# davelailai/DS-GCN

Hardware: AMD Instinct MI355X
Metric: clips/sec fwd+bwd, DS-STGCN NTU-60 3x64x25x2 (higher is better)
Workload: dtype f32; 1 GPU; DS-STGCN configs/dsstgcn/ntu60_xsub_3dkp/j.py (DSSTGCN_model.py kwargs), 64 clips/GPU of 3x64x25x2, 60 classes, train-mode BN, CE loss, fwd+bwd+grad all-reduce+SGD-nesterov per step; clips_per_gpu=64, global_batch=64, parallelism=dp1

## Files before the change

ds-gcn_amd/csrc/bwd64.hip:

```cpp
#include "common.h"

namespace {

constexpr int BF_NT = 256, BF_KC = 64, BF_LS = BF_KC + 2, BF_Q = BF_KC / 4, BF_J = 64 * BF_Q / BF_NT;
constexpr int BF_OOB = 0x7ffffff0;

struct BfArgs {
  const float* x1; const float* s1; const float* h1;
  const float* x2; const float* s2; const float* h2; int relu;
  const float* w;
  const float* z; const float* gz; const float* A0; const float* B0;
  float* dx; float* dx2; float* dwp; float* dbp; float* ipart;
  int pstride, n, Ci, Co, L, cpn, total_chunks, cps;
};

typedef float bf_f2 __attribute__((ext_vector_type(2)));

__device__ __forceinline__ __amdgpu_buffer_rsrc_t bf_rsrc(const void* p, int bytes) {
  return __builtin_amdgcn_make_buffer_rsrc(const_cast<void*>(p), (short)0, bytes, 0x00020000);
}
__device__ __forceinline__ f32x4 bf_load(__amdgpu_buffer_rsrc_t r, int voff) {
  return __builtin_bit_cast(f32x4, __builtin_amdgcn_raw_buffer_load_b128(r, voff, 0, 0));
}
__device__ __forceinline__ int bf_row32(int r, int half) { return (r & 3) + 8 * (r >> 2) + 4 * half; }

#ifdef DSGCN_LAB
__device__ long long g_bf_stamp[64];
#define BF_STAMP() do { if (blockIdx.x == 0 && threadIdx.x == 0 && nst < 62) g_bf_stamp[nst++] = wall_clock64(); } while (0)
#else
#define BF_STAMP() do {} while (0)
#endif

template <bool HASC, bool AFF, bool HAS2>
__global__ __launch_bounds__(BF_NT, 2) void k_bwd64(BfArgs a) {
  extern __shared__ __attribute__((aligned(16))) float lds[];
#ifdef DSGCN_LAB
  int nst = 0;
#endif
  BF_STAMP();
  float* Ds = lds;
  float* Xs = lds + 64 * BF_LS;
  float* Os = lds + 128 * BF_LS;
  float* Ws = lds + 192 * BF_LS;
  bf_f2* Cs = reinterpret_cast<bf_f2*>(Ws + 64 * 65);
  f32x4* Ps = reinterpret_cast<f32x4*>(Cs + 64);
  const int tid = threadIdx.x, lane = tid & 63;
  const int wave = __builtin_amdgcn_readfirstlane(tid >> 6);
  const int half = lane >> 5, l31 = lane & 31;
  const int Ci = a.Ci, Co = a.Co, L = a.L, L4 = L * 4;
  const int split = blockIdx.x;
  const int ch0 = split * a.cps, ch1 = min(a.total_chunks, ch0 + a.cps);

  for (int i = tid; i < 64 * 65; i += BF_NT) {
    const int co = i / 65, ci = i - co * 65;
    Ws[i] = (co < Co && ci < Ci) ? a.w[(size_t)co * Ci + ci] : 0.f;
  }
  if (tid < 64) {
    Cs[tid] = (HASC && tid < Co) ? bf_f2{a.A0[tid], a.B0[tid]} : bf_f2{0.f, 0.f};
    f32x4 p = {1.f, 0.f, 1.f, 0.f};
    if (AFF && tid < Ci) {
      if (a.s1) { p.x = a.s1[tid]; p.y = a.h1[tid]; }
      if (HAS2 && a.s2) { p.z = a.s2[tid]; p.w = a.h2[tid]; }
    }
    Ps[tid] = p;
  }
  const float lo = a.relu ? 0.f : -__builtin_inff();

  const int col = (tid % BF_Q) * 4, row0 = tid / BF_Q;
  f32x4 gr[BF_J], zr[HASC ? BF_J : 1], xr[BF_J], yr[HAS2 ? BF_J : 1];
  f32x4 xk[AFF ? BF_J : 1], yk[HAS2 ? BF_J : 1];
  float dsum[BF_J], r0[BF_J], r1[BF_J], r2[BF_J];
#pragma unroll
  for (int j = 0; j < BF_J; ++j) { dsum[j] = 0.f; r0[j] = 0.f; r1[j] = 0.f; r2[j] = 0.f; }
  auto issue = [&](int ch) {
    const int n = ch / a.cpn, c0 = (ch - n * a.cpn) * BF_KC;
    const bool pv = c0 + col < L;
    const __amdgpu_buffer_rsrc_t rg = bf_rsrc(a.gz + (size_t)n * Co * L, Co * L4);
    const __amdgpu_buffer_rsrc_t rz = bf_rsrc((HASC ? a.z : a.gz) + (size_t)n * Co * L, HASC ? Co * L4 : 0);
    const __amdgpu_buffer_rsrc_t rx = bf_rsrc(a.x1 + (size_t)n * Ci * L, Ci * L4);
    const __amdgpu_buffer_rsrc_t ry = bf_rsrc((HAS2 ? a.x2 : a.x1) + (size_t)n * Ci * L, HAS2 ? Ci * L4 : 0);
#pragma unroll
    for (int j = 0; j < BF_J; ++j) {
      const int row = row0 + 16 * j;
      const int vd = (pv && row < Co) ? (row * L + c0 + col) * 4 : BF_OOB;
      const int vx = (pv && row < Ci) ? (row * L + c0 + col) * 4 : BF_OOB;
      gr[j] = bf_load(rg, vd);
      if constexpr (HASC) zr[j] = bf_load(rz, vd);
      xr[j] = bf_load(rx, vx);
      if constexpr (HAS2) yr[j] = bf_load(ry, vx);
    }
  };
  auto commit = [&](int ch) {
    const int n = ch / a.cpn, c0 = (ch - n * a.cpn) * BF_KC;
    const bool pv = c0 + col < L;
#pragma unroll
    for (int j = 0; j < BF_J; ++j) {
      const int row = row0 + 16 * j;
      f32x4 d = gr[j];
      if constexpr (HASC) {
        const bf_f2 c = Cs[row];
#pragma unroll
        for (int e = 0; e < 4; ++e) d[e] += fmaf(c.y, zr[j][e], c.x);
      }
      if (!(pv && row < Co)) d = f32x4{0.f, 0.f, 0.f, 0.f};
      dsum[j] += (d.x + d.y) + (d.z + d.w);
      bf_f2* dd = reinterpret_cast<bf_f2*>(Ds + row * BF_LS + col);
      dd[0] = bf_f2{d.x, d.y};
      dd[1] = bf_f2{d.z, d.w};
      f32x4 v = xr[j];
      if constexpr (AFF) {
        const f32x4 p = Ps[row];
        xk[j] = xr[j];
        if constexpr (HAS2) yk[j] = yr[j];
#pragma unroll
        for (int e = 0; e < 4; ++e) {
          float t = fmaf(xr[j][e], p.x, p.y);
          if constexpr (HAS2) t += fmaf(yr[j][e], p.z, p.w);
          v[e] = fmaxf(t, lo);
        }
      }
      if (!(pv && row < Ci)) v = f32x4{0.f, 0.f, 0.f, 0.f};
      bf_f2* dxs = reinterpret_cast<bf_f2*>(Xs + row * BF_LS + col);
      dxs[0] = bf_f2{v.x, v.y};
      dxs[1] = bf_f2{v.z, v.w};
    }
  };

  f32x16 accw, accw2, accd, accd2;
#pragma unroll
  for (int i = 0; i < 16; ++i) { accw[i] = 0.f; accw2[i] = 0.f; }
  const bool narrow_i = Ci <= 32;
  const int mt = narrow_i ? (wave & 1) : (wave >> 1), nt = narrow_i ? 0 : (wave & 1);
  const int cit = narrow_i ? 0 : (wave >> 1), pt = wave & 1;
  const float* Ap = Ds + (32 * mt + l31) * BF_LS + 2 * half;
  const float* Bp = Xs + (32 * nt + l31) * BF_LS + 2 * half;
  const int KSd = (Co + 1) >> 1;
  const bool wg_on = 32 * mt < Co && 32 * nt < Ci && !(narrow_i && wave >= 2);
  const bool dg_on = 32 * cit < Ci && !(narrow_i && wave < 2);

  __syncthreads();
  BF_STAMP();
  if (ch0 < ch1) issue(ch0);
  for (int ch = ch0; ch < ch1; ++ch) {
    commit(ch);
    asm volatile("s_waitcnt lgkmcnt(0)" ::: "memory");
    __builtin_amdgcn_s_barrier();
    BF_STAMP();
    if (ch + 1 < ch1) issue(ch + 1);
    if (wg_on) {
      bf_f2 av0 = *reinterpret_cast<const bf_f2*>(Ap), bv0 = *reinterpret_cast<const bf_f2*>(Bp);
      bf_f2 av1 = *reinterpret_cast<const bf_f2*>(Ap + 4), bv1 = *reinterpret_cast<const bf_f2*>(Bp + 4);
#pragma unroll
      for (int w = 0; w < BF_Q; w += 2) {
        bf_f2 an0 = av0, bn0 = bv0, an1 = av1, bn1 = bv1;
        if (w + 2 < BF_Q) {
          an0 = *reinterpret_cast<const bf_f2*>(Ap + 4 * (w + 2)); bn0 = *reinterpret_cast<const bf_f2*>(Bp + 4 * (w + 2));
          an1 = *reinterpret_cast<const bf_f2*>(Ap + 4 * (w + 3)); bn1 = *reinterpret_cast<const bf_f2*>(Bp + 4 * (w + 3));
        }
        __builtin_amdgcn_sched_barrier(0);
        accw = __builtin_amdgcn_mfma_f32_32x32x2f32(av0.x, bv0.x, accw, 0, 0, 0);
        accw2 = __builtin_amdgcn_mfma_f32_32x32x2f32(av0.y, bv0.y, accw2, 0, 0, 0);
        accw = __builtin_amdgcn_mfma_f32_32x32x2f32(av1.x, bv1.x, accw, 0, 0, 0);
        accw2 = __builtin_amdgcn_mfma_f32_32x32x2f32(av1.y, bv1.y, accw2, 0, 0, 0);
        __builtin_amdgcn_sched_barrier(0);
        av0 = an0; bv0 = bn0; av1 = an1; bv1 = bn1;
      }
    }
    if (dg_on) {
#pragma unroll
      for (int i = 0; i < 16; ++i) { accd[i] = 0.f; accd2[i] = 0.f; }
      const float* Wa = Ws + half * 65 + 32 * cit + l31;
      const float* Db = Ds + half * BF_LS + 32 * pt + l31;
      const int KS4 = (KSd + 3) & ~3;
      float wa[4], db[4];
#pragma unroll
      for (int i = 0; i < 4; ++i) { wa[i] = Wa[2 * i * 65]; db[i] = Db[2 * i * BF_LS]; }
      for (int ks = 0; ks < KS4; ks += 4) {
        float wn[4], dn[4];
        const int kn = ks + 4 < 32 ? ks + 4 : 28;
#pragma unroll
        for (int i = 0; i < 4; ++i) { wn[i] = Wa[2 * (kn + i) * 65]; dn[i] = Db[2 * (kn + i) * BF_LS]; }
        __builtin_amdgcn_sched_barrier(0);
        accd = __builtin_amdgcn_mfma_f32_32x32x2f32(wa[0], db[0], accd, 0, 0, 0);
        accd2 = __builtin_amdgcn_mfma_f32_32x32x2f32(wa[1], db[1], accd2, 0, 0, 0);
        accd = __builtin_amdgcn_mfma_f32_32x32x2f32(wa[2], db[2], accd, 0, 0, 0);
        accd2 = __builtin_amdgcn_mfma_f32_32x32x2f32(wa[3], db[3], accd2, 0, 0, 0);
        __builtin_amdgcn_sched_barrier(0);
#pragma unroll
        for (int i = 0; i < 4; ++i) { wa[i] = wn[i]; db[i] = dn[i]; }
      }
#pragma unroll
      for (int r = 0; r < 16; ++r)
        Os[(32 * cit + bf_row32(r, half)) * BF_LS + 32 * pt + l31] = accd[r] + accd2[r];
    }
    asm volatile("s_waitcnt lgkmcnt(0)" ::: "memory");
    __builtin_amdgcn_s_barrier();
    BF_STAMP();
    {
      const int n = ch / a.cpn, c0 = (ch - n * a.cpn) * BF_KC;
      if (c0 + col < L) {
#pragma unroll
        for (int j = 0; j < BF_J; ++j) {
          const int row = row0 + 16 * j;
          if (row < Ci) {
            const bf_f2* o = reinterpret_cast<const bf_f2*>(Os + row * BF_LS + col);
            const bf_f2 lo2 = o[0], hi2 = o[1];
            f32x4 dv = {lo2.x, lo2.y, hi2.x, hi2.y};
            f32x4 p = {1.f, 0.f, 1.f, 0.f};
            if constexpr (AFF) {
              p = Ps[row];
#pragma unroll
              for (int e = 0; e < 4; ++e) {
                float t = fmaf(xk[j][e], p.x, p.y);
                if constexpr (HAS2) t += fmaf(yk[j][e], p.z, p.w);
                if (a.relu && !(t > 0.f)) dv[e] = 0.f;
                r0[j] = fmaf(dv[e], xk[j][e], r0[j]);
                r1[j] += dv[e];
                if constexpr (HAS2) r2[j] = fmaf(dv[e], yk[j][e], r2[j]);
              }
            }
            const size_t go = ((size_t)n * Ci + row) * L + c0 + col;
            __builtin_nontemporal_store(f32x4{dv.x * p.x, dv.y * p.x, dv.z * p.x, dv.w * p.x}, reinterpret_cast<f32x4*>(a.dx + go));
            if constexpr (HAS2) __builtin_nontemporal_store(f32x4{dv.x * p.z, dv.y * p.z, dv.z * p.z, dv.w * p.z}, reinterpret_cast<f32x4*>(a.dx2 + go));
          }
        }
      }
    }
  }

  BF_STAMP();
  float* dw = a.dwp + (size_t)split * a.pstride;
  {
    const int ci = 32 * nt + l31;
#pragma unroll
    for (int r = 0; r < 16; ++r) {
      const int co = 32 * mt + bf_row32(r, half);
      if (wg_on && co < Co && ci < Ci) dw[(size_t)co * Ci + ci] = accw[r] + accw2[r];
    }
  }
#pragma unroll
  for (int j = 0; j < BF_J; ++j) {
    float s = dsum[j], s0 = r0[j], s1 = r1[j], s2 = r2[j];
#pragma unroll
    for (int off = 1; off < BF_Q; off <<= 1) {
      s += __shfl_xor(s, off, 64);
      if (AFF) { s0 += __shfl_xor(s0, off, 64); s1 += __shfl_xor(s1, off, 64); }
      if (HAS2) s2 += __shfl_xor(s2, off, 64);
    }
    const int row = row0 + 16 * j;
    if ((tid % BF_Q) == 0) {
      if (row < Co) a.dbp[(size_t)split * a.pstride + row] = s;
      if (AFF && a.ipart && row < Ci) {
        float* o = a.ipart + ((size_t)split * Ci + row) * 3;
        o[0] = s0; o[1] = s1; o[2] = s2;
      }
    }
  }
#ifdef DSGCN_LAB
  BF_STAMP();
  if (blockIdx.x == 0 && threadIdx.x == 0) g_bf_stamp[63] = nst;
#endif
}

constexpr int BB_RB = 80, BB_RT = 144, BB_OS = 36;
constexpr int BB_DK = 0, BB_XK = 3 * 64 * BB_RB, BB_DT = 2 * 3 * 64 * BB_RB, BB_WT = BB_DT + 3 * 32 * BB_RT,
              BB_OSO = BB_WT + 3 * 64 * BB_RT, BB_LDS = BB_OSO + 64 * BB_OS * 4;

template <bool HASC, bool AFF>
__global__ __launch_bounds__(BF_NT, 2) void k_bwd64b(BfArgs a) {
  extern __shared__ __attribute__((aligned(16))) char ldsb[];
#ifdef DSGCN_LAB
  int nst = 0;
#endif
  BF_STAMP();
  char* Dk = ldsb + BB_DK;
  char* Xk = ldsb + BB_XK;
  char* Dt = ldsb + BB_DT;
  char* Wt = ldsb + BB_WT;
  float* Os = reinterpret_cast<float*>(ldsb + BB_OSO);
  const int tid = threadIdx.x, lane = tid & 63;
  const int wave = __builtin_amdgcn_readfirstlane(tid >> 6);
  const int half = lane >> 5, l31 = lane & 31;
  const int Ci = a.Ci, Co = a.Co, L = a.L, L4 = L * 4;
  const int split = blockIdx.x;
  const int ch0 = split * a.cps, ch1 = min(a.total_chunks, ch0 + a.cps);
  const int row = tid >> 2, q = tid & 3;
  const bool rd = row < Co, rx = row < Ci;
  const float A0v = (HASC && rd) ? a.A0[row] : 0.f, B0v = (HASC && rd) ? a.B0[row] : 0.f;
  float s1v = 1.f, h1v = 0.f;
  if (AFF && rx && a.s1) { s1v = a.s1[row]; h1v = a.h1[row]; }
  const float lo = a.relu ? 0.f : -__builtin_inff();
  for (int i = tid; i < 64 * 32; i += BF_NT) {
    const int ci = i >> 5, co = 2 * (i & 31);
    const float w0 = (ci < Ci && co < Co) ? a.w[(size_t)co * Ci + ci] : 0.f;
    const float w1 = (ci < Ci && co + 1 < Co) ? a.w[(size_t)(co + 1) * Ci + ci] : 0.f;
    unsigned p0, p1, p2;
    b3_split(w0, w1, p0, p1, p2);
    char* base = Wt + ci * BB_RT + co * 2;
    *reinterpret_cast<unsigned*>(base) = p0;
    *reinterpret_cast<unsigned*>(base + 64 * BB_RT) = p1;
    *reinterpret_cast<unsigned*>(base + 2 * 64 * BB_RT) = p2;
  }

  struct Raw { f32x4 g[2], z[HASC ? 2 : 1], x[2]; };
  Raw ra, rb;
  f32x4 xk[AFF ? 2 : 1];
  float dsum = 0.f, r0 = 0.f, r1 = 0.f;
  auto issue = [&](int ch, Raw& R) {
    const int n = ch / a.cpn, c0 = (ch - n * a.cpn) * 32;
    const __amdgpu_buffer_rsrc_t rg = bf_rsrc(a.gz + (size_t)n * Co * L, Co * L4);
    const __amdgpu_buffer_rsrc_t rz = bf_rsrc((HASC ? a.z : a.gz) + (size_t)n * Co * L, HASC ? Co * L4 : 0);
    const __amdgpu_buffer_rsrc_t r1_ = bf_rsrc(a.x1 + (size_t)n * Ci * L, Ci * L4);
#pragma unroll
    for (int h = 0; h < 2; ++h) {
      const int p = c0 + 8 * q + 4 * h;
      const int vd = (rd && p < L) ? (row * L + p) * 4 : BF_OOB;
      const int vx = (rx && p < L) ? (row * L + p) * 4 : BF_OOB;
      R.g[h] = bf_load(rg, vd);
      if constexpr (HASC) R.z[h] = bf_load(rz, vd);
      R.x[h] = bf_load(r1_, vx);
    }
  };
  auto commit = [&](int ch, const Raw& R) {
    const int n = ch / a.cpn, c0 = (ch - n * a.cpn) * 32;
    float d[8], v[8];
#pragma unroll
    for (int h = 0; h < 2; ++h) {
      const bool in = c0 + 8 * q + 4 * h < L;
#pragma unroll
      for (int e = 0; e < 4; ++e) {
        float x = R.g[h][e];
        if constexpr (HASC) x += fmaf(B0v, R.z[h][e], A0v);
        d[4 * h + e] = (rd && in) ? x : 0.f;
        float t = R.x[h][e];
        if constexpr (AFF) {
          t = fmaf(t, s1v, h1v);
          t = fmaxf(t, lo);
        }
        v[4 * h + e] = (rx && in) ? t : 0.f;
      }
      if constexpr (AFF) xk[h] = R.x[h];
    }
    dsum += ((d[0] + d[1]) + (d[2] + d[3])) + ((d[4] + d[5]) + (d[6] + d[7]));
    unsigned t0[4], t1[4], t2[4];
#pragma unroll
    for (int j = 0; j < 4; ++j) b3_split(d[2 * j], d[2 * j + 1], t0[j], t1[j], t2[j]);
    {
      char* base = Dk + row * BB_RB + q * 16;
      *reinterpret_cast<u32x4v*>(base) = u32x4v{t0[0], t0[1], t0[2], t0[3]};
      *reinterpret_cast<u32x4v*>(base + 64 * BB_RB) = u32x4v{t1[0], t1[1], t1[2], t1[3]};
      *reinterpret_cast<u32x4v*>(base + 2 * 64 * BB_RB) = u32x4v{t2[0], t2[1], t2[2], t2[3]};
    }
    {
      const int odd = row & 1;
      char* base = Dt + (8 * q + odd) * BB_RT + (row & ~1) * 2;
      const unsigned sel = odd ? 0x07060302u : 0x01000504u;
      unsigned o0[4], o1[4], o2[4];
#pragma unroll
      for (int j = 0; j < 4; ++j) {
        o0[j] = __shfl_xor(t0[j], 4, 64); o1[j] = __shfl_xor(t1[j], 4, 64); o2[j] = __shfl_xor(t2[j], 4, 64);
      }
#pragma unroll
      for (int j = 0; j < 4; ++j) {
        const unsigned w0 = __builtin_amdgcn_perm(t0[j], o0[j], sel);
        const unsigned w1 = __builtin_amdgcn_perm(t1[j], o1[j], sel);
        const unsigned w2 = __builtin_amdgcn_perm(t2[j], o2[j], sel);
        char* pj = base + 2 * j * BB_RT;
        *reinterpret_cast<unsigned*>(pj) = w0;
        *reinterpret_cast<unsigned*>(pj + 32 * BB_RT) = w1;
        *reinterpret_cast<unsigned*>(pj + 2 * 32 * BB_RT) = w2;
      }
    }
#pragma unroll
    for (int j = 0; j < 4; ++j) b3_split(v[2 * j], v[2 * j + 1], t0[j], t1[j], t2[j]);
    {
      char* base = Xk + row * BB_RB + q * 16;
      *reinterpret_cast<u32x4v*>(base) = u32x4v{t0[0], t0[1], t0[2], t0[3]};
      *reinterpret_cast<u32x4v*>(base + 64 * BB_RB) = u32x4v{t1[0], t1[1], t1[2], t1[3]};
      *reinterpret_cast<u32x4v*>(base + 2 * 64 * BB_RB) = u32x4v{t2[0], t2[1], t2[2], t2[3]};
    }
    (void)n;
  };

  const bool wgw = wave < 2;
  const int mt = wave & 1, cit = wave & 1;
  const bool wg0 = wgw && 32 * mt < Co, wg1 = wg0 && Ci > 32;
  const bool dg_on = !wgw && 32 * cit < Ci;
  const int KSD = (Co + 15) >> 4;
  f32x16 accw, accw1;
#pragma unroll
  for (int i = 0; i < 16; ++i) { accw[i] = 0.f; accw1[i] = 0.f; }
  const char* Af = Dk + (32 * mt + l31) * BB_RB + 16 * half;
  const char* Bf = Xk + l31 * BB_RB + 16 * half;
  const char* Wf = Wt + (32 * cit + l31) * BB_RT + 16 * half;
  const char* Df = Dt + l31 * BB_RT + 16 * half;
  auto six = [&](f32x16 c, const char* pa, int sa, const char* pb, int sb) {
    const bf16x8 a0 = __builtin_bit_cast(bf16x8, *reinterpret_cast<const u32x4v*>(pa)),
                 a1 = __builtin_bit_cast(bf16x8, *reinterpret_cast<const u32x4v*>(pa + sa)),
                 a2 = __builtin_bit_cast(bf16x8, *reinterpret_cast<const u32x4v*>(pa + 2 * sa));
    const bf16x8 b0 = __builtin_bit_cast(bf16x8, *reinterpret_cast<const u32x4v*>(pb)),
                 b1 = __builtin_bit_cast(bf16x8, *reinterpret_cast<const u32x4v*>(pb + sb)),
                 b2 = __builtin_bit_cast(bf16x8, *reinterpret_cast<const u32x4v*>(pb + 2 * sb));
    c = __builtin_amdgcn_mfma_f32_32x32x16_bf16(a2, b0, c, 0, 0, 0);
    c = __builtin_amdgcn_mfma_f32_32x32x16_bf16(a1, b1, c, 0, 0, 0);
    c = __builtin_amdgcn_mfma_f32_32x32x16_bf16(a0, b2, c, 0, 0, 0);
    c = __builtin_amdgcn_mfma_f32_32x32x16_bf16(a1, b0, c, 0, 0, 0);
    c = __builtin_amdgcn_mfma_f32_32x32x16_bf16(a0, b1, c, 0, 0, 0);
    c = __builtin_amdgcn_mfma_f32_32x32x16_bf16(a0, b0, c, 0, 0, 0);
    return c;
  };

  __syncthreads();
  BF_STAMP();
  auto unit = [&](int ch, Raw& R) {
    commit(ch, R);
    if (ch + 2 < ch1) issue(ch + 2, R);
    asm volatile("s_waitcnt lgkmcnt(0)" ::: "memory");
    __builtin_amdgcn_s_barrier();
    BF_STAMP();
    if (wg0) {
      accw = six(accw, Af, 64 * BB_RB, Bf, 64 * BB_RB);
      accw = six(accw, Af + 32, 64 * BB_RB, Bf + 32, 64 * BB_RB);
      if (wg1) {
        accw1 = six(accw1, Af, 64 * BB_RB, Bf + 32 * BB_RB, 64 * BB_RB);
        accw1 = six(accw1, Af + 32, 64 * BB_RB, Bf + 32 * BB_RB + 32, 64 * BB_RB);
      }
    }
    if (dg_on) {
      f32x16 accd;
#pragma unroll
      for (int i = 0; i < 16; ++i) accd[i] = 0.f;
#pragma unroll
      for (int ks = 0; ks < 4; ++ks)
        if (ks < KSD) accd = six(accd, Wf + 32 * ks, 64 * BB_RT, Df + 32 * ks, 32 * BB_RT);
#pragma unroll
      for (int r = 0; r < 16; ++r) Os[(32 * cit + bf_row32(r, half)) * BB_OS + l31] = accd[r];
    }
    asm volatile("s_waitcnt lgkmcnt(0)" ::: "memory");
    __builtin_amdgcn_s_barrier();
    BF_STAMP();
    {
      const int n = ch / a.cpn, c0 = (ch - n * a.cpn) * 32;
      f32x4* o = reinterpret_cast<f32x4*>(Os + row * BB_OS + 8 * q);
#pragma unroll
      for (int h = 0; h < 2; ++h) {
        f32x4 dv = o[h];
        if (rx && c0 + 8 * q + 4 * h < L) {
          float sx = 1.f;
          if constexpr (AFF) {
            sx = s1v;
#pragma unroll
            for (int e = 0; e < 4; ++e) {
              const float t = fmaf(xk[h][e], s1v, h1v);
              if (a.relu && !(t > 0.f)) dv[e] = 0.f;
              r0 = fmaf(dv[e], xk[h][e], r0);
              r1 += dv[e];
            }
          }
          const size_t go = ((size_t)n * Ci + row) * L + c0 + 8 * q + 4 * h;
          __builtin_nontemporal_store(f32x4{dv.x * sx, dv.y * sx, dv.z * sx, dv.w * sx}, reinterpret_cast<f32x4*>(a.dx + go));
        }
      }
    }
  };
  if (ch0 < ch1) issue(ch0, ra);
  if (ch0 + 1 < ch1) issue(ch0 + 1, rb);
  for (int ch = ch0; ch < ch1; ch += 2) {
    unit(ch, ra);
    if (ch + 1 < ch1) unit(ch + 1, rb);
  }

  BF_STAMP();
  float* dw = a.dwp + (size_t)split * a.pstride;
#pragma unroll
  for (int r = 0; r < 16; ++r) {
    const int co = 32 * mt + bf_row32(r, half);
    if (wg0 && co < Co && l31 < Ci) dw[(size_t)co * Ci + l31] = accw[r];
    if (wg1 && co < Co && 32 + l31 < Ci) dw[(size_t)co * Ci + 32 + l31] = accw1[r];
  }
  {
    float s = dsum, s0 = r0, s1 = r1;
#pragma unroll
    for (int off = 1; off < 4; off <<= 1) {
      s += __shfl_xor(s, off, 64);
      if (AFF) { s0 += __shfl_xor(s0, off, 64); s1 += __shfl_xor(s1, off, 64); }
    }
    if (q == 0) {
      if (rd) a.dbp[(size_t)split * a.pstride + row] = s;
      if (AFF && a.ipart && rx) {
        float* o = a.ipart + ((size_t)split * Ci + row) * 3;
        o[0] = s0; o[1] = s1; o[2] = 0.f;
      }
    }
  }
#ifdef DSGCN_LAB
  BF_STAMP();
  if (blockIdx.x == 0 && threadIdx.x == 0) g_bf_stamp[63] = nst;
#endif
}

struct BfPlan { int cpn, chunks, splits, cps; };

int g_bf_b3 = 1;

bool bf_plan(int n, int Ci, int Co, int L, BfPlan* p) {
  if (Ci <= 0 || Co <= 0 || Ci > 64 || Co > 64 || L % 4) return false;
  if ((long)64 * L * 4 >= (1L << 31) - 64) return false;
  p->cpn = (L + BF_KC - 1) / BF_KC;
  p->chunks = n * p->cpn;
  int target = 512;
  if (target > p->chunks) target = p->chunks;
  p->cps = (p->chunks + target - 1) / target;
  p->splits = (p->chunks + p->cps - 1) / p->cps;
  return true;
}

}

__attribute__((visibility("hidden"))) int dsgcn_bwd64_splits(int n, int Ci, int Co, int L) {
  BfPlan p;
  return bf_plan(n, Ci, Co, L, &p) ? p.splits : 0;
}

__attribute__((visibility("hidden"))) int dsgcn_bwd64(const float* x1, const float* s1, const float* h1, const float* x2,
                                                       const float* s2, const float* h2, int relu, const float* w,
                                                       const float* z, const float* gz, const float* A0, const float* B0,
                                                       float* dx, float* dx2, float* dwp, float* dbp, int pstride,
                                                       float* ipart, int n, int Ci, int Co, int L, hipStream_t st) {
  BfPlan p;
  if (!bf_plan(n, Ci, Co, L, &p)) return 0;
  BfArgs a = {};
  a.x1 = x1; a.s1 = s1; a.h1 = h1; a.x2 = x2; a.s2 = s2; a.h2 = h2; a.relu = relu; a.w = w; a.z = z; a.gz = gz;
  a.A0 = A0; a.B0 = B0; a.dx = dx; a.dx2 = dx2; a.dwp = dwp; a.dbp = dbp; a.ipart = ipart; a.pstride = pstride;
  a.n = n; a.Ci = Ci; a.Co = Co; a.L = L; a.cpn = p.cpn; a.total_chunks = p.chunks; a.cps = p.cps;
  const bool b3 = g_bf_b3 && x2 == nullptr && Ci >= 16;
  if (b3) {
    a.cpn = (L + 31) / 32;
    a.total_chunks = n * a.cpn;
    a.cps = (a.total_chunks + p.splits - 1) / p.splits;
  }
  const size_t lds = b3 ? (size_t)BB_LDS : (size_t)(192 * BF_LS + 64 * 65 + 2 * 64 + 4 * 64) * sizeof(float);
  const dim3 grid((unsigned)p.splits), blk(BF_NT);
  const bool hasc = A0 != nullptr, has2 = x2 != nullptr, aff = s1 != nullptr || s2 != nullptr || relu != 0 || has2;
  if (b3) {
#define BB_LAUNCH(HC, AF)                                                                                               \
  {                                                                                                                   \
    static bool raised = false;                                                                                       \
    if (!raised) {                                                                                                    \
      hipError_t e = hipFuncSetAttribute((const void*)k_bwd64b<HC, AF>, hipFuncAttributeMaxDynamicSharedMemorySize, \
                                         (int)lds);                                                                   \
      if (e != hipSuccess) return (int)e;                                                                             \
      raised = true;                                                                                                  \
    }                                                                                                                 \
    hipLaunchKernelGGL((k_bwd64b<HC, AF>), grid, blk, lds, st, a);                                                \
  }
    if (hasc) {
      if (aff) BB_LAUNCH(true, true) else BB_LAUNCH(true, false)
    } else {
      if (aff) BB_LAUNCH(false, true) else BB_LAUNCH(false, false)
    }
#undef BB_LAUNCH
    DSGCN_LAUNCH_CHECK();
    return 1;
  }
#define BF_LAUNCH(HC, AF, H2)                                                                                          \
  {                                                                                                                   \
    static bool raised = false;                                                                                       \
    if (!raised) {                                                                                                    \
      hipError_t e = hipFuncSetAttribute((const void*)k_bwd64<HC, AF, H2>, hipFuncAttributeMaxDynamicSharedMemorySize, \
                                         (int)lds);                                                                   \
      if (e != hipSuccess) return (int)e;                                                                             \
      raised = true;                                                                                                  \
    }                                                                                                                 \
    hipLaunchKernelGGL((k_bwd64<HC, AF, H2>), grid, blk, lds, st, a);                                                 \
  }
  if (has2) {
    if (hasc) BF_LAUNCH(true, true, true) else BF_LAUNCH(false, true, true)
  } else if (hasc) {
    if (aff) BF_LAUNCH(true, true, false) else BF_LAUNCH(true, false, false)
  } else {
    if (aff) BF_LAUNCH(false, true, false) else BF_LAUNCH(false, false, false)
  }
#undef BF_LAUNCH
  DSGCN_LAUNCH_CHECK();
  return 1;
}

__attribute__((visibility("hidden"))) int dsgcn_bwd64_tuning(int value) { g_bf_b3 = value; return 0; }

#ifdef DSGCN_LAB
extern "C" int dsgcn_bwd64_phases(long long* out) {
  return (int)hipMemcpyFromSymbol(out, HIP_SYMBOL(g_bf_stamp), sizeof(long long) * 64);
}
#endif
```

ds-gcn_amd/csrc/fuseout.hip:

```cpp
#include "common.h"
#include "dropout.h"
#include "dsgcn_jobs.h"

namespace {

__global__ __launch_bounds__(64) void k_fuse_out_fwd(const float* __restrict__ x1, const float* __restrict__ s1,
                                                     const float* __restrict__ h1, const float* __restrict__ x2,
                                                     const float* __restrict__ s2, const float* __restrict__ h2,
                                                     int relu, float* __restrict__ out, float* __restrict__ xbar, int C,
                                                     int T, int V, int vec, int ld, float* __restrict__ out_s2,
                                                     float* __restrict__ pmean, DropArgs dr) {
  extern __shared__ __attribute__((aligned(16))) float lds[];
  const int lane = threadIdx.x;
  const long plane = blockIdx.x;
  const int c = (int)(plane % C);
  const int L = T * V;
  const bool drop = dr.thresh != 0;
  const unsigned long long dstep = (drop && dr.step) ? (unsigned long long)*dr.step : 0ull;
  const float a1 = s1 ? s1[c] : 1.f, b1 = s1 ? h1[c] : 0.f;
  const float a2 = s2 ? s2[c] : 1.f, b2 = s2 ? h2[c] : 0.f;
  const float* p1 = x1 + (size_t)plane * L;
  const float* p2 = x2 ? x2 + (size_t)plane * L : nullptr;
  float* po = out ? out + (size_t)plane * L : nullptr;
  float psum = 0.f;
  if (vec) {
    const int L4 = L >> 2;
    const f32x4* q1 = reinterpret_cast<const f32x4*>(p1);
    const f32x4* q2 = reinterpret_cast<const f32x4*>(p2);
    f32x4* qo = reinterpret_cast<f32x4*>(po);
    f32x4* ql = reinterpret_cast<f32x4*>(lds);
#pragma unroll 4
    for (int i = lane; i < L4; i += 64) {
      f32x4 v = q1[i];
      v.x = fmaf(v.x, a1, b1); v.y = fmaf(v.y, a1, b1); v.z = fmaf(v.z, a1, b1); v.w = fmaf(v.w, a1, b1);
      if (relu & 2) { v.x = fmaxf(v.x, 0.f); v.y = fmaxf(v.y, 0.f); v.z = fmaxf(v.z, 0.f); v.w = fmaxf(v.w, 0.f); }
      if (drop) {
        unsigned rw[4];
        drop_words(dr, dstep, (unsigned long long)plane * L4 + i, rw);
        v.x *= rw[0] >= dr.thresh ? dr.inv : 0.f; v.y *= rw[1] >= dr.thresh ? dr.inv : 0.f;
        v.z *= rw[2] >= dr.thresh ? dr.inv : 0.f; v.w *= rw[3] >= dr.thresh ? dr.inv : 0.f;
      }
      if (p2) {
        const f32x4 r = q2[i];
        v.x += fmaf(r.x, a2, b2); v.y += fmaf(r.y, a2, b2); v.z += fmaf(r.z, a2, b2); v.w += fmaf(r.w, a2, b2);
      }
      if (relu & 1) { v.x = fmaxf(v.x, 0.f); v.y = fmaxf(v.y, 0.f); v.z = fmaxf(v.z, 0.f); v.w = fmaxf(v.w, 0.f); }
      if (po) qo[i] = v;
      psum += (v.x + v.y) + (v.z + v.w);
      if (xbar || out_s2) ql[i] = v;
    }
  } else {
    for (int i = lane; i < L; i += 64) {
      float v = fmaf(p1[i], a1, b1);
      if (relu & 2) v = fmaxf(v, 0.f);
      if (drop) v *= drop_mult(dr, dstep, (unsigned long long)plane * L + i);
      if (p2) v += fmaf(p2[i], a2, b2);
      if (relu & 1) v = fmaxf(v, 0.f);
      if (po) po[i] = v;
      psum += v;
      if (xbar || out_s2) lds[i] = v;
    }
  }
  if (pmean) {
    psum = wave_sum(psum);
    if (lane == 0) pmean[plane] = psum / (float)L;
  }
  if (xbar || out_s2) wave_lds_sync();
  if (out_s2) {
    const int T2 = (T + 1) >> 1, L2 = T2 * V;
    float* ps = out_s2 + (size_t)plane * L2;
    const float invV = 1.f / (float)V;
    if ((L2 & 3) == 0) {
      f32x4* q4 = reinterpret_cast<f32x4*>(ps);
      for (int i = lane; i < (L2 >> 2); i += 64) {
        int t, v;
        divmod_small(4 * i, V, invV, t, v);
        float r[4];
#pragma unroll
        for (int k = 0; k < 4; ++k) {
          r[k] = lds[2 * t * V + v];
          if (++v == V) { v = 0; ++t; }
        }
        q4[i] = f32x4{r[0], r[1], r[2], r[3]};
      }
    } else {
      for (int i = lane; i < L2; i += 64) {
        int t, v;
        divmod_small(i, V, invV, t, v);
        ps[i] = lds[2 * t * V + v];
      }
    }
  }
  if (xbar) {
    if (lane < ld) {
      float s = 0.f;
      if (lane < V)
        for (int t = 0; t < T; ++t) s += lds[t * V + lane];
      xbar[(size_t)plane * ld + lane] = s / (float)T;
    }
  }
}

__global__ __launch_bounds__(64) void k_fuse_out_bwd(const float* __restrict__ x1, const float* __restrict__ s1,
                                                     const float* __restrict__ h1, const float* __restrict__ x2,
                                                     const float* __restrict__ s2, const float* __restrict__ h2,
                                                     int relu, const float* __restrict__ dout,
                                                     const float* __restrict__ dout2, const float* __restrict__ dout3,
                                                     const float* __restrict__ dxbar, float* __restrict__ dx1,
                                                     float* __restrict__ dx2, float* __restrict__ part, int C, int T,
                                                     int V, int ld, int s3, DropArgs dr) {
  __shared__ float dxb[32];
  const int lane = threadIdx.x;
  const long plane = blockIdx.x;
  const int c = (int)(plane % C);
  const int L = T * V;
  const bool drop = dr.thresh != 0;
  const unsigned long long dstep = (drop && dr.step) ? (unsigned long long)*dr.step : 0ull;
  const float a1 = s1 ? s1[c] : 1.f, b1 = s1 ? h1[c] : 0.f;
  const float a2 = s2 ? s2[c] : 1.f, b2 = s2 ? h2[c] : 0.f;
  if (lane < V) dxb[lane] = dxbar ? dxbar[(size_t)plane * ld + lane] / (float)T : 0.f;
  wave_lds_sync();
  const float* __restrict__ p1 = x1 + (size_t)plane * L;
  const float* __restrict__ p2 = x2 ? x2 + (size_t)plane * L : nullptr;
  const float* __restrict__ pg = (dout && s3 != 3) ? dout + (size_t)plane * L : nullptr;
  const float gpl = s3 == 3 ? dout[plane] / (float)L : 0.f;
  const float* __restrict__ pg2 = dout2 ? dout2 + (size_t)plane * L : nullptr;
  const float* __restrict__ pg3 = dout3 ? dout3 + (size_t)plane * (s3 == 2 ? ((T + 1) >> 1) * V : L) : nullptr;
  float* __restrict__ o1 = dx1 + (size_t)plane * L;
  float* __restrict__ o2 = dx2 ? dx2 + (size_t)plane * L : nullptr;
  float u0 = 0.f, u1 = 0.f, u2 = 0.f, u3 = 0.f;
  int v = lane % V, t = lane / V;
  const int step = 64 % V, tstep = 64 / V;
#pragma unroll 5
  for (int i = lane; i < L; i += 64) {
    const float xa = p1[i];
    const float xb = p2 ? p2[i] : 0.f;
    const float pre1 = fmaf(xa, a1, b1);
    float pre = (relu & 2) ? fmaxf(pre1, 0.f) : pre1;
    const float dm = drop ? drop_mult(dr, dstep, (unsigned long long)plane * L + i) : 1.f;
    pre *= dm;
    if (p2) pre += fmaf(xb, a2, b2);
    float g = s3 == 3 ? gpl : (pg ? pg[i] : 0.f);
    if (pg2) g += pg2[i];
    if (pg3) {
      if (s3 == 2) { if (!(t & 1)) g += pg3[(t >> 1) * V + v]; }
      else g += pg3[i];
    }
    g += dxb[v];
    if ((relu & 1) && !(pre > 0.f)) g = 0.f;
    const float g1 = (((relu & 2) && !(pre1 > 0.f)) ? 0.f : g) * dm;
    o1[i] = g1 * a1;
    if (o2) o2[i] = g * a2;
    u0 = fmaf(g1, xa, u0);
    u1 += g;
    u2 = fmaf(g, xb, u2);
    u3 += g1;
    v += step;
    t += tstep;
    if (v >= V) { v -= V; ++t; }
  }
  if (part) {
    u0 = wave_sum(u0);
    u1 = wave_sum(u1);
    u2 = wave_sum(u2);
    u3 = wave_sum(u3);
    if (lane == 0) {
      part[(size_t)plane * 4 + 0] = u0;
      part[(size_t)plane * 4 + 1] = u1;
      part[(size_t)plane * 4 + 2] = u2;
      part[(size_t)plane * 4 + 3] = u3;
    }
  }
}

template <int NG, bool S3, bool X2>
__global__ __launch_bounds__(64) void k_fuse_out_bwd4(const float* __restrict__ x1, const float* __restrict__ s1,
                                                      const float* __restrict__ h1, const float* __restrict__ x2,
                                                      const float* __restrict__ s2, const float* __restrict__ h2,
                                                      int relu, const float* __restrict__ dout,
                                                      const float* __restrict__ dout2, const float* __restrict__ dout3,
                                                      const float* __restrict__ dxbar, float* __restrict__ dx1,
                                                      float* __restrict__ dx2, float* __restrict__ part, int C, int T,
                                                      int V, int ld, DropArgs dr) {
  __shared__ float dxb[32];
  const int lane = threadIdx.x;
  const long plane = blockIdx.x;
  const int c = (int)(plane % C);
  const int L = T * V, L4 = L >> 2;
  const bool drop = dr.thresh != 0;
  const unsigned long long dstep = (drop && dr.step) ? (unsigned long long)*dr.step : 0ull;
  const float a1 = s1 ? s1[c] : 1.f, b1 = s1 ? h1[c] : 0.f;
  const float a2 = s2 ? s2[c] : 1.f, b2 = s2 ? h2[c] : 0.f;
  if (lane < V) dxb[lane] = dxbar ? dxbar[(size_t)plane * ld + lane] / (float)T : 0.f;
  wave_lds_sync();
  const f32x4* __restrict__ p1 = reinterpret_cast<const f32x4*>(x1 + (size_t)plane * L);
  const f32x4* __restrict__ p2 = X2 ? reinterpret_cast<const f32x4*>(x2 + (size_t)plane * L) : nullptr;
  const f32x4* __restrict__ pg = NG >= 1 ? reinterpret_cast<const f32x4*>(dout + (size_t)plane * L) : nullptr;
  const float gplane = NG == 0 ? dout[plane] / (float)L : 0.f;
  const f32x4* __restrict__ pg2 = NG >= 2 ? reinterpret_cast<const f32x4*>(dout2 + (size_t)plane * L) : nullptr;
  const f32x4* __restrict__ pg3 = (NG >= 3 && !S3) ? reinterpret_cast<const f32x4*>(dout3 + (size_t)plane * L) : nullptr;
  const float* __restrict__ ps3 = S3 ? dout3 + (size_t)plane * (((T + 1) >> 1) * V) : nullptr;
  f32x4* __restrict__ o1 = reinterpret_cast<f32x4*>(dx1 + (size_t)plane * L);
  f32x4* __restrict__ o2 = X2 ? reinterpret_cast<f32x4*>(dx2 + (size_t)plane * L) : nullptr;
  const float invV = 1.f / (float)V;
  float u0 = 0.f, u1 = 0.f, u2 = 0.f, u3 = 0.f;
  for (int i = lane; i < L4; i += 64) {
    const f32x4 xa = p1[i];
    f32x4 xb = {0.f, 0.f, 0.f, 0.f}, g = {gplane, gplane, gplane, gplane};
    if constexpr (NG >= 1) g = pg[i];
    if constexpr (X2) xb = p2[i];
    if constexpr (NG >= 2) { const f32x4 w = pg2[i]; g.x += w.x; g.y += w.y; g.z += w.z; g.w += w.w; }
    if constexpr (NG >= 3 && !S3) { const f32x4 w = pg3[i]; g.x += w.x; g.y += w.y; g.z += w.z; g.w += w.w; }
    int t, v;
    divmod_small(4 * i, V, invV, t, v);
    f32x4 r1, r2;
    float dm[4] = {1.f, 1.f, 1.f, 1.f};
    if (drop) {
      unsigned rw[4];
      drop_words(dr, dstep, (unsigned long long)plane * L4 + i, rw);
#pragma unroll
      for (int k = 0; k < 4; ++k) dm[k] = rw[k] >= dr.thresh ? dr.inv : 0.f;
    }
#pragma unroll
    for (int k = 0; k < 4; ++k) {
      float gg = g[k];
      if constexpr (S3) { if (!(t & 1)) gg += ps3[(t >> 1) * V + v]; }
      gg += dxb[v];
      const float pre1 = fmaf(xa[k], a1, b1);
      float pre = ((relu & 2) ? fmaxf(pre1, 0.f) : pre1) * dm[k];
      if constexpr (X2) pre += fmaf(xb[k], a2, b2);
      if ((relu & 1) && !(pre > 0.f)) gg = 0.f;
      const float g1 = (((relu & 2) && !(pre1 > 0.f)) ? 0.f : gg) * dm[k];
      r1[k] = g1 * a1;
      r2[k] = gg * a2;
      u0 = fmaf(g1, xa[k], u0);
      u1 += gg;
      u2 = fmaf(gg, xb[k], u2);
      u3 += g1;
      if (++v == V) { v = 0; ++t; }
    }
    o1[i] = r1;
    if constexpr (X2) o2[i] = r2;
  }
  if (part) {
    u0 = wave_sum(u0);
    u1 = wave_sum(u1);
    u2 = wave_sum(u2);
    u3 = wave_sum(u3);
    if (lane == 0) {
      part[(size_t)plane * 4 + 0] = u0;
      part[(size_t)plane * 4 + 1] = u1;
      part[(size_t)plane * 4 + 2] = u2;
      part[(size_t)plane * 4 + 3] = u3;
    }
  }
}

int g_fo_vec = 1;

}

namespace {

DropArgs drop_args(const dsgcn_dropout* d) {
  DropArgs a = {};
  if (d && d->p > 0.f) {
    a.step = d->step; a.seed = d->seed; a.call = d->call;
    double t = (double)d->p * 4294967296.0;
    a.thresh = t >= 4294967295.0 ? 4294967295u : (t < 1.0 ? 1u : (unsigned)t);
    a.inv = 1.f / (1.f - d->p);
  }
  return a;
}

__global__ __launch_bounds__(256) void k_dropout_mask(float* __restrict__ mask, long numel, DropArgs dr) {
  const unsigned long long step = dr.step ? (unsigned long long)*dr.step : 0ull;
  for (long e = (long)blockIdx.x * 256 + threadIdx.x; e < numel; e += (long)gridDim.x * 256)
    mask[e] = dr.thresh ? drop_mult(dr, step, (unsigned long long)e) : 1.f;
}

}

extern "C" {

int dsgcn_fuse_out_fwd_drop(const float* x1, const float* s1, const float* h1, const float* x2, const float* s2,
                            const float* h2, int relu, float* out, float* out_s2, float* xbar, float* pmean, int n, int C,
                            int T, int V, int xbar_ld, const dsgcn_dropout* d, void* stream) {
  if (!x1 || (!out && !pmean) || n <= 0 || C <= 0 || T <= 0 || V <= 0 || V > 32 || (s1 && !h1) || (s2 && !h2)) return DSGCN_EINVAL;
  if ((out_s2 || xbar) && !out) return DSGCN_EINVAL;
  if (xbar && (xbar_ld < V || xbar_ld > 64)) return DSGCN_EINVAL;
  if (d && !(d->p >= 0.f && d->p < 1.f)) return DSGCN_EINVAL;
  const int vec = ((T * V) % 4 == 0) ? 1 : 0;
  const size_t lds = (xbar || out_s2) ? (size_t)T * V * sizeof(float) : 0;
  if (lds > 64 * 1024) return DSGCN_EUNSUPPORTED;
  hipLaunchKernelGGL(k_fuse_out_fwd, dim3((unsigned)((long)n * C)), dim3(64), lds, (hipStream_t)stream, x1, s1, h1, x2,
                     s2, h2, relu, out, xbar, C, T, V, vec, xbar ? xbar_ld : V, out_s2, pmean, drop_args(d));
  DSGCN_LAUNCH_CHECK();
  return 0;
}

int dsgcn_fuse_out_fwd(const float* x1, const float* s1, const float* h1, const float* x2, const float* s2,
                       const float* h2, int relu, float* out, float* xbar, int n, int C, int T, int V, int xbar_ld,
                       void* stream) {
  if (!out) return DSGCN_EINVAL;
  return dsgcn_fuse_out_fwd_drop(x1, s1, h1, x2, s2, h2, relu, out, nullptr, xbar, nullptr, n, C, T, V, xbar_ld, nullptr, stream);
}

int dsgcn_fuse_out_fwd2(const float* x1, const float* s1, const float* h1, const float* x2, const float* s2,
                        const float* h2, int relu, float* out, float* out_s2, float* xbar, int n, int C, int T, int V,
                        int xbar_ld, void* stream) {
  if (!out) return DSGCN_EINVAL;
  return dsgcn_fuse_out_fwd_drop(x1, s1, h1, x2, s2, h2, relu, out, out_s2, xbar, nullptr, n, C, T, V, xbar_ld, nullptr, stream);
}

int dsgcn_fuse_out_pool_fwd(const float* x1, const float* s1, const float* h1, const float* x2, const float* s2,
                            const float* h2, int relu, float* pmean, int n, int C, int T, int V, void* stream) {
  if (!pmean) return DSGCN_EINVAL;
  return dsgcn_fuse_out_fwd_drop(x1, s1, h1, x2, s2, h2, relu, nullptr, nullptr, nullptr, pmean, n, C, T, V, V, nullptr, stream);
}

int dsgcn_fuse_out_bwd_drop(const float* x1, const float* s1, const float* h1, const float* x2, const float* s2,
                            const float* h2, int relu, const float* dout, const float* dout2, const float* dout3,
                            int stride3, const float* dxbar, float* dx1, float* dx2, float* part, int n, int C, int T, int V,
                            int xbar_ld, const dsgcn_dropout* d, void* stream) {
  if (!x1 || !dx1 || n <= 0 || C <= 0 || T <= 0 || V <= 0 || V > 32 || (x2 && !dx2)) return DSGCN_EINVAL;
  if (dxbar && xbar_ld < V) return DSGCN_EINVAL;
  if ((dout2 || dout3) && !dout) return DSGCN_EINVAL;
  if (stride3 < 1 || stride3 > 3 || (stride3 == 3 && (!dout || dout2 || dout3 || dxbar))) return DSGCN_EINVAL;
  if (d && !(d->p >= 0.f && d->p < 1.f)) return DSGCN_EINVAL;
  const DropArgs dr = drop_args(d);
  const dim3 grid((unsigned)((long)n * C)), blk(64);
  hipStream_t st = (hipStream_t)stream;
  if (stride3 == 3) {
    if ((T * V) % 4 == 0) {
      if (x2)
        hipLaunchKernelGGL((k_fuse_out_bwd4<0, false, true>), grid, blk, 0, st, x1, s1, h1, x2, s2, h2, relu, dout,
                           (const float*)nullptr, (const float*)nullptr, (const float*)nullptr, dx1, dx2, part, C, T, V, V, dr);
      else
        hipLaunchKernelGGL((k_fuse_out_bwd4<0, false, false>), grid, blk, 0, st, x1, s1, h1, x2, s2, h2, relu, dout,
                           (const float*)nullptr, (const float*)nullptr, (const float*)nullptr, dx1, dx2, part, C, T, V, V, dr);
    } else {
      hipLaunchKernelGGL(k_fuse_out_bwd, grid, blk, 0, st, x1, s1, h1, x2, s2, h2, relu, dout, (const float*)nullptr,
                         (const float*)nullptr, (const float*)nullptr, dx1, dx2, part, C, T, V, V, 3, dr);
    }
    DSGCN_LAUNCH_CHECK();
    return 0;
  }
  if (g_fo_vec && dout && (T * V) % 4 == 0 && !(dout3 && !dout2 && stride3 == 1)) {
    const int ng = dout3 && stride3 == 1 ? 3 : (dout2 ? 2 : 1);
    const bool s3 = dout3 && stride3 == 2;
#define FO4(NGV, S3V, X2V) hipLaunchKernelGGL((k_fuse_out_bwd4<NGV, S3V, X2V>), grid, blk, 0, st, x1, s1, h1, x2, s2, h2, relu, \
                                              dout, dout2, dout3, dxbar, dx1, dx2, part, C, T, V, xbar_ld, dr)
    if (x2) {
      if (s3) { if (ng == 2) FO4(2, true, true); else FO4(1, true, true); }
      else if (ng == 3) FO4(3, false, true);
      else if (ng == 2) FO4(2, false, true);
      else FO4(1, false, true);
    } else {
      if (s3) { if (ng == 2) FO4(2, true, false); else FO4(1, true, false); }
      else if (ng == 3) FO4(3, false, false);
      else if (ng == 2) FO4(2, false, false);
      else FO4(1, false, false);
    }
#undef FO4
    DSGCN_LAUNCH_CHECK();
    return 0;
  }
  hipLaunchKernelGGL(k_fuse_out_bwd, grid, blk, 0, st, x1, s1, h1, x2, s2, h2, relu, dout, dout2, dout3, dxbar, dx1, dx2,
                     part, C, T, V, xbar_ld, stride3, dr);
  DSGCN_LAUNCH_CHECK();
  return 0;
}

int dsgcn_fuse_out_pool_bwd(const float* x1, const float* s1, const float* h1, const float* x2, const float* s2,
                            const float* h2, int relu, const float* dpmean, float* dx1, float* dx2, float* part, int n,
                            int C, int T, int V, void* stream) {
  if (!dpmean) return DSGCN_EINVAL;
  return dsgcn_fuse_out_bwd_drop(x1, s1, h1, x2, s2, h2, relu, dpmean, nullptr, nullptr, 3, nullptr, dx1, dx2, part, n, C, T, V,
                                 V, nullptr, stream);
}

int dsgcn_fuse_out_bwd3(const float* x1, const float* s1, const float* h1, const float* x2, const float* s2,
                        const float* h2, int relu, const float* dout, const float* dout2, const float* dout3,
                        const float* dxbar, float* dx1, float* dx2, float* part, int n, int C, int T, int V, int xbar_ld,
                        void* stream) {
  return dsgcn_fuse_out_bwd_drop(x1, s1, h1, x2, s2, h2, relu, dout, dout2, dout3, 1, dxbar, dx1, dx2, part, n, C, T, V,
                                 xbar_ld, nullptr, stream);
}

int dsgcn_fuse_out_bwd3s(const float* x1, const float* s1, const float* h1, const float* x2, const float* s2,
                         const float* h2, int relu, const float* dout, const float* dout2, const float* dout3, int stride3,
                         const float* dxbar, float* dx1, float* dx2, float* part, int n, int C, int T, int V, int xbar_ld,
                         void* stream) {
  if (stride3 != 1 && stride3 != 2) return DSGCN_EINVAL;
  return dsgcn_fuse_out_bwd_drop(x1, s1, h1, x2, s2, h2, relu, dout, dout2, dout3, stride3, dxbar, dx1, dx2, part, n, C, T, V,
                                 xbar_ld, nullptr, stream);
}

int dsgcn_dropout_mask(float* mask, long numel, const dsgcn_dropout* d, void* stream) {
  if (!mask || numel <= 0 || (d && !(d->p >= 0.f && d->p < 1.f))) return DSGCN_EINVAL;
  const long blocks = (numel + 255) / 256;
  hipLaunchKernelGGL(k_dropout_mask, dim3((unsigned)(blocks > 4096 ? 4096 : blocks)), dim3(256), 0, (hipStream_t)stream, mask,
                     numel, drop_args(d));
  DSGCN_LAUNCH_CHECK();
  return 0;
}

#ifdef DSGCN_LAB
int dsgcn_fuse_out_tuning(int key, int value) {
  if (key != 0) return DSGCN_EINVAL;
  g_fo_vec = value;
  return 0;
}
#endif

int dsgcn_fuse_out_bwd(const float* x1, const float* s1, const float* h1, const float* x2, const float* s2,
                       const float* h2, int relu, const float* dout, const float* dxbar, float* dx1, float* dx2,
                       float* part, int n, int C, int T, int V, int xbar_ld, void* stream) {
  return dsgcn_fuse_out_bwd3(x1, s1, h1, x2, s2, h2, relu, dout, nullptr, nullptr, dxbar, dx1, dx2, part, n, C, T, V,
                             xbar_ld, stream);
}

}

namespace {
__global__ __launch_bounds__(256) void k_pack(const float* const* __restrict__ src, const long* __restrict__ off,
                                              const int* __restrict__ numel, float* __restrict__ dst) {
  const int i = blockIdx.x;
  const float* __restrict__ s = src[i];
  float* __restrict__ d = dst + off[i];
  const int n = numel[i];
  for (int j = blockIdx.y * 256 + threadIdx.x; j < n; j += gridDim.y * 256) d[j] = s[j];
}
}

namespace {
__global__ __launch_bounds__(256) void k_pack_fill(const float* const* __restrict__ src, const long* __restrict__ off,
                                                   const long* __restrict__ numel, float* __restrict__ dst) {
  const int i = blockIdx.x;
  const float* __restrict__ s = src[i];
  float* __restrict__ d = dst + off[i];
  const long n = numel[i];
  if (s) {
    for (long j = blockIdx.y * 256 + threadIdx.x; j < n; j += gridDim.y * 256) d[j] = s[j];
  } else {
    for (long j = blockIdx.y * 256 + threadIdx.x; j < n; j += gridDim.y * 256) d[j] = 0.f;
  }
}
}

extern "C" int dsgcn_pack_fill(const float* const* src_table, const long* dst_offsets, const long* numels, int count,
                               float* dst, void* stream) {
  if (!src_table || !dst_offsets || !numels || !dst || count <= 0) return DSGCN_EINVAL;
  hipLaunchKernelGGL(k_pack_fill, dim3((unsigned)count, 8), dim3(256), 0, (hipStream_t)stream, src_table, dst_offsets,
                     numels, dst);
  DSGCN_LAUNCH_CHECK();
  return 0;
}

extern "C" int dsgcn_pack(const float* const* src_table, const long* dst_offsets, const int* numels, int count,
                          float* dst, void* stream) {
  if (!src_table || !dst_offsets || !numels || !dst || count <= 0) return DSGCN_EINVAL;
  hipLaunchKernelGGL(k_pack, dim3((unsigned)count, 8), dim3(256), 0, (hipStream_t)stream, src_table, dst_offsets, numels,
                     dst);
  DSGCN_LAUNCH_CHECK();
  return 0;
}

namespace {
__global__ __launch_bounds__(256) void k_add3(const f32x4* __restrict__ a, const f32x4* __restrict__ b,
                                              const f32x4* __restrict__ c, f32x4* __restrict__ out, long n4,
                                              const float* as, const float* bs, const float* cs, float* os, long n) {
  const long i = (long)blockIdx.x * 256 + threadIdx.x;
  if (i < n4) {
    f32x4 v = a[i];
    const f32x4 w = b[i];
    v.x += w.x; v.y += w.y; v.z += w.z; v.w += w.w;
    if (c) { const f32x4 u = c[i]; v.x += u.x; v.y += u.y; v.z += u.z; v.w += u.w; }
    out[i] = v;
  }
  if (blockIdx.x == 0) {
    const long j = n4 * 4 + threadIdx.x;
    if (j < n) os[j] = as[j] + bs[j] + (cs ? cs[j] : 0.f);
  }
}
}

extern "C" int dsgcn_add3(const float* a, const float* b, const float* c, float* out, long n, void* stream) {
  if (!a || !b || !out || n <= 0) return DSGCN_EINVAL;
  const long n4 = n / 4;
  const unsigned blocks = (unsigned)((n4 + 255) / 256);
  hipLaunchKernelGGL(k_add3, dim3(blocks ? blocks : 1), dim3(256), 0, (hipStream_t)stream,
                     reinterpret_cast<const f32x4*>(a), reinterpret_cast<const f32x4*>(b),
                     reinterpret_cast<const f32x4*>(c), reinterpret_cast<f32x4*>(out), n4, a, b, c, out, n);
  DSGCN_LAUNCH_CHECK();
  return 0;
}
```

ds-gcn_amd/csrc/pwconv.hip:

```cpp
#include "common.h"
#include "bn_jobs.h"

namespace {

constexpr int KCH = 16;
constexpr int WSTR = KCH + 1;
constexpr int NTW = 2;
constexpr int PW_NT = 256;
constexpr int XCH = KCH / 4;

struct PwArgs {
  const float* x1; const float* s1; const float* h1;
  const float* x2; const float* s2; const float* h2;
  int relu;
  const float* w; const float* bias;
  float* z; float* zaug; float* partial;
  int n, Ci, Co, T, V, Tout, stride, aug, TR, NPpad, vec, stats, roll, nbx, cc;
};

__device__ __forceinline__ int mfma_row32(int r, int half) { return (r & 3) + 8 * (r >> 2) + 4 * half; }

__device__ __forceinline__ float virt1(float a, float b, bool has2, float s1, float h1, float s2, float h2,
                                       int relu) {
  float v = fmaf(a, s1, h1);
// ... 920 lines not shown
          }
        }
      } else {
#pragma unroll
        for (int e = 0; e < 4; ++e) {
          const int pe = p + e;
          if (pe < nvalid) {
            if (co < Co) {
              if (has_g) gr[j][e] = a.gz[gzb + pe];
              if (has_c) zr[j][e] = a.z[gzb + pe];
            }
            if (ci < Ci) {
              const int rl = (int)(((float)pe + 0.5f) * invV);
              const size_t g = gxb + (size_t)rl * a.stride * V + (pe - rl * V);
              xr[j][e] = a.x1[g];
              if (HAS2) yr[HAS2 ? j : 0][e] = a.x2[g];
            }
          }
        }
      }
    }
  };

  auto commit = [&](int ch) {
    const int n = ch / a.nb_per_sample;
    const int r0 = (ch - n * a.nb_per_sample) * TR;
    const int nvalid = min(TR, a.Tout - r0) * V;
    float dsum = 0.f;
#pragma unroll
    for (int j = 0; j < WG_J; ++j) {
#pragma unroll
      for (int e = 0; e < 4; ++e) {
        const int pe = 16 * j + 4 * quarter + e;
        if (pe < KP) {
          float d = 0.f, x = 0.f;
          if (pe < nvalid) {
            if (co < Co) {
              d = has_g ? gr[j][e] : 0.f;
              if (has_c) d += fmaf(B0c, zr[j][e], A0c);
              if (a.aug) {
                const int rl = (int)(((float)pe + 0.5f) * invV);
                const size_t ga = (size_t)(n * Co + co) * a.Tout + r0 + rl;
                float ea = a.gzaug ? a.gzaug[ga] : 0.f;
                if (has_c) ea += fmaf(B0c, a.zaug[ga], A0c);
                d = fmaf(ea, invV, d);
              }
            }
            if (ci < Ci) x = virt1(xr[j][e], HAS2 ? yr[HAS2 ? j : 0][e] : 0.f, has2, s1, h1, s2, h2, a.relu);
          }
          Ds[row * LS + pe] = d;
          Xs[row * LS + pe] = x;
          dsum += d;
        }
      }
    }
    dsum += __shfl_xor(dsum, 1, 64);
    dsum += __shfl_xor(dsum, 2, 64);
    dbacc += dsum;
  };

  if (ch0 < ch1) issue(ch0);
  for (int ch = ch0; ch < ch1; ++ch) {
    commit(ch);
    __syncthreads();
    if (ch + 1 < ch1) issue(ch + 1);
    for (int kk = 0; kk < KP; kk += 2) {
      const float av = Ds[(32 * mt + l31) * LS + kk + half];
      const float bv = Xs[(32 * ntile + l31) * LS + kk + half];
      acc = __builtin_amdgcn_mfma_f32_32x32x2f32(av, bv, acc, 0, 0, 0);
    }
    __syncthreads();
  }
  const int cio = ciBase + 32 * ntile + l31;
  if (cio < Ci) {
#pragma unroll
    for (int r = 0; r < 16; ++r) {
      const int coo = coBase + 32 * mt + mfma_row32(r, half);
      if (coo < Co) a.dwp[(size_t)split * a.pstride + (size_t)coo * Ci + cio] = acc[r];
    }
  }
  if (byy == 0 && quarter == 0 && co < Co) a.dbp[(size_t)split * a.pstride + co] = dbacc;
}

__global__ __launch_bounds__(64) void k_bn_bwd_coef(const float* __restrict__ g_scale,
                                                    const float* __restrict__ g_shift,
                                                    const float* __restrict__ mean, const float* __restrict__ var,
                                                    const float* __restrict__ gamma, float eps, double count, int C,
                                                    int c_affine, float* __restrict__ dgamma,
                                                    float* __restrict__ dbeta, float* __restrict__ A0,
                                                    float* __restrict__ B0) {
  const int c = blockIdx.x * 64 + threadIdx.x;
  if (c >= C) return;
  if (c >= c_affine) { dgamma[c] = 0.f; dbeta[c] = 0.f; A0[c] = 0.f; B0[c] = 0.f; return; }
  const double gs = g_scale ? (double)g_scale[c] : 0.0, gh = g_shift ? (double)g_shift[c] : 0.0;
  const double mu = mean[c], r = 1.0 / sqrt((double)var[c] + (double)eps);
  const double g = gamma ? (double)gamma[c] : 1.0;
  const double t = gs - mu * gh;
  dgamma[c] = (float)(r * t);
  dbeta[c] = (float)gh;
  const double dmean = -gh * g * r;
  const double dvar = -0.5 * r * r * r * g * t;
  A0[c] = (float)((dmean - 2.0 * dvar * mu) / count);
  B0[c] = (float)(2.0 * dvar / count);
}

__global__ __launch_bounds__(1024) void k_bn_coef_rows(const float* __restrict__ part, int R, int C, int k, int ids, int idh,
                                                       const float* __restrict__ mean, const float* __restrict__ var,
                                                       const float* __restrict__ gamma, float eps, double count,
                                                       int c_affine, float* __restrict__ coef, int accumulate) {
  __shared__ double red[16][8][2];
  const BnCoefJob J = {part, mean, var, gamma, coef, count, eps, R, C, k, ids, idh, c_affine, accumulate};
  bn_coef_rows_block(J, blockIdx.x, red);
}

}

int g_pw_maxmt = 2;
int g_pw4 = 15;

__attribute__((visibility("hidden"))) int dsgcn_p4_tuning(int key, int value);
__attribute__((visibility("hidden"))) int dsgcn_p4_groups(int n, int K, int M, int L, int epi);
__attribute__((visibility("hidden"))) int dsgcn_wg2_tuning(int key, int value);
__attribute__((visibility("hidden"))) int dsgcn_p4_fwd(const float* x1, const float* s1, const float* h1,
                                                        const float* x2, const float* s2, const float* h2, int relu,
                                                        const float* w, const float* bias, float* z, float* partial,
                                                        int n, int Ci, int Co, int L, hipStream_t st, const void* ws);
__attribute__((visibility("hidden"))) size_t dsgcn_p4_ws_bytes(int n, int Ci, int Co, int L);
__attribute__((visibility("hidden"))) int dsgcn_bwd64_tuning(int value);
__attribute__((visibility("hidden"))) int dsgcn_p4_wsplit(const float* w, int Ci, int Co, void* out, hipStream_t st);
__attribute__((visibility("hidden"))) int dsgcn_p4_wsplit_multi(const float* const* w, void* const* out, const int* Ci,
                                                                const int* Co, int njobs, hipStream_t st);
__attribute__((visibility("hidden"))) int dsgcn_p4_dgrad(const float* x1, const float* s1, const float* h1,
                                                          const float* x2, const float* s2, const float* h2, int relu,
                                                          const float* w, const float* z, const float* gz,
                                                          const float* A0, const float* B0, float* dx1, float* dx2,
                                                          float* ipart, int n, int Ci, int Co, int L, hipStream_t st,
                                                          const void* ws);

__attribute__((visibility("hidden"))) int dsgcn_p4_group_ok(int n, int Ci, int Co, int L);
__attribute__((visibility("hidden"))) int dsgcn_p4_fwd_group(const float* const* x1, const float* const* s1,
                                                              const float* const* h1, int relu, const float* const* w,
                                                              float* const* z, int ng, int n, int Ci, int Co, int L,
                                                              hipStream_t st);
__attribute__((visibility("hidden"))) int dsgcn_p4_dgrad_group(const float* const* x1, const float* const* s1,
                                                                const float* const* h1, int relu, const float* const* w,
                                                                const float* const* gz, float* const* dx1, float* const* ipart,
                                                                int ng, int n, int Ci, int Co, int L, hipStream_t st);

__attribute__((visibility("hidden"))) int dsgcn_bwd64_splits(int n, int Ci, int Co, int L);
__attribute__((visibility("hidden"))) int dsgcn_bwd64(const float* x1, const float* s1, const float* h1, const float* x2,
                                                       const float* s2, const float* h2, int relu, const float* w,
                                                       const float* z, const float* gz, const float* A0, const float* B0,
                                                       float* dx, float* dx2, float* dwp, float* dbp, int pstride,
                                                       float* ipart, int n, int Ci, int Co, int L, hipStream_t st);

__attribute__((visibility("hidden"))) int dsgcn_wg2_splits(int n, int Ci, int Co, int L);
__attribute__((visibility("hidden"))) int dsgcn_wg2(const float* x1, const float* s1, const float* h1, const float* x2,
                                                     const float* s2, const float* h2, int relu, const float* z,
                                                     const float* gz, const float* A0, const float* B0, float* dwp,
                                                     float* dbp, int pstride, int n, int Ci, int Co, int L,
                                                     hipStream_t st, const BnCoefTable* jobs, int ngroup = 0,
                                                     const float* const* gx1 = nullptr, const float* const* gs1 = nullptr,
                                                     const float* const* gh1 = nullptr, const float* const* ggz = nullptr,
                                                     float* const* gdwp = nullptr, float* const* gdbp = nullptr);

static int pw_conv_rows(int n, int K, int M, int T, int V, int stride, int which) {
  const int Tout = (T + stride - 1) / stride;
  const int L = Tout * V;
  if (stride == 1 && (g_pw4 & which)) {
    const int g = dsgcn_p4_groups(n, K, M, L, which == 2 ? 1 : 0);
    if (g > 0) return g;
  }
  return n * ((L + 4 * 32 - 1) / (4 * 32));
}

extern "C" {

#ifdef DSGCN_LAB
int dsgcn_pwconv_tuning(int key, int value) {
  if (key == 1) { g_pw_maxmt = value; return 0; }
  if (key == 2) { g_pw_roll = value; return 0; }
  if (key == 3) { g_pw4 = value; return 0; }
  if (key >= 4 && key <= 6) return dsgcn_p4_tuning(key - 4, value);
  if (key >= 7 && key <= 9) return dsgcn_wg2_tuning(key - 7, value);
  if (key >= 10 && key <= 12) return dsgcn_p4_tuning(key - 7, value);
  if (key == 13) return dsgcn_wg2_tuning(3, value);
  if (key == 14) return dsgcn_p4_tuning(6, value);
  if (key >= 15 && key <= 17) return dsgcn_wg2_tuning(key - 11, value);
  if (key == 18) return dsgcn_bwd64_tuning(value);
  if (key == 19) return dsgcn_p4_tuning(7, value);
  if (key == 22) return dsgcn_p4_tuning(9, value);
  if (key == 20) return dsgcn_p4_tuning(8, value);
  return DSGCN_EINVAL;
}
#endif

int dsgcn_pwconv_plan(int Tout, int V, int aug, int* TR, int* NPpad, int* nblk_per_sample) {
  int tr = Tout >= 32 ? 8 : 4;
  if (tr > Tout) tr = Tout;
  int np = tr * (V + (aug ? 1 : 0));
  while (np > 256 && tr > 1) { tr >>= 1; np = tr * (V + (aug ? 1 : 0)); }
  if (np > 256) return DSGCN_EUNSUPPORTED;
  *TR = tr;
  *NPpad = (np + 31) & ~31;
  *nblk_per_sample = (Tout + tr - 1) / tr;
  return 0;
}

int dsgcn_pwconv_partial_rows(int n, int Ci, int Co, int T, int V, int stride, int aug) {
  int rows = pw_conv_rows(n, Ci, Co, T, V, stride, 1);
  if (aug) rows += n;
  return rows;
}

int dsgcn_pwconv_fwd_ws(const float* x1, const float* s1, const float* h1, const float* x2, const float* s2,
                        const float* h2, int relu, const float* w, const float* bias, float* z, float* zaug,
                        float* partial, int n, int Ci, int Co, int T, int V, int stride, int aug, int stats,
                        const void* ws, void* stream) {
  if (!x1 || !w || !z || n <= 0 || Ci <= 0 || Co <= 0 || T <= 0 || V <= 0 || stride <= 0) return DSGCN_EINVAL;
  if ((aug && !zaug) || (stats && !partial) || (s1 && !h1) || (s2 && !h2)) return DSGCN_EINVAL;
  const int Tout = (T + stride - 1) / stride;
  PwArgs a = {};
  a.x1 = x1; a.s1 = s1; a.h1 = h1; a.x2 = x2; a.s2 = s2; a.h2 = h2; a.relu = relu;
  a.w = w; a.bias = bias; a.z = z; a.zaug = zaug; a.partial = partial;
  a.n = n; a.Ci = Ci; a.Co = Co; a.T = T; a.V = V; a.Tout = Tout; a.stride = stride; a.aug = aug;
  a.stats = stats;
  a.roll = ((g_pw_roll & 1) && Ci % KW == 0) ? 1 : 0;
  hipStream_t st = (hipStream_t)stream;
  const int L = Tout * V;
  const int conv_rows = pw_conv_rows(n, Ci, Co, T, V, stride, 1);
  int fast = 0;
  if (stride == 1 && (g_pw4 & 1)) {
    fast = dsgcn_p4_fwd(x1, s1, h1, x2, s2, h2, relu, w, bias, z, stats ? partial : nullptr, n, Ci, Co, L, st, ws);
    if (fast != 0 && fast != 1) return fast;
  }
  if (!fast) {
  if ((long)n * Ci * T * V * 4 >= (1L << 31) - 64 || (long)n * Co * T * V * 4 >= (1L << 31) - 64) return DSGCN_EUNSUPPORTED;
  const int mtiles = (Co + 31) / 32;
  const int MT = mtiles >= g_pw_maxmt ? g_pw_maxmt : mtiles;
  const int NW = 1;
  const int nbx = (L + 4 * NW * 32 - 1) / (4 * NW * 32);
  a.nbx = nbx;
  a.cc = (mtiles + MT - 1) / MT;
  dim3 grid((unsigned)(((long)nbx * n + 7) / 8 * 8 * a.cc));
  size_t ldsf = (size_t)32 * MT * KWS + 4 + (size_t)4 * Ci;
  if (ldsf < (size_t)4 * 32 * 36 + 512) ldsf = (size_t)4 * 32 * 36 + 512;
  const size_t lds = ldsf * sizeof(float);
#define PW_FWD2(MTV)                                                                                  \
  if (a.roll) hipLaunchKernelGGL((k_pwconv_fwd2<MTV, 1, true>), grid, dim3(PW_NT), lds, st, a);       \
  else hipLaunchKernelGGL((k_pwconv_fwd2<MTV, 1, false>), grid, dim3(PW_NT), lds, st, a)
  switch (MT) {
    case 1: PW_FWD2(1); break;
    case 2: PW_FWD2(2); break;
    case 3: PW_FWD2(3); break;
    default: PW_FWD2(4); break;
  }
#undef PW_FWD2
  DSGCN_LAUNCH_CHECK();
  }
  if (aug) {
    const size_t l2 = (size_t)Tout * V * sizeof(float);
    if (l2 > 64 * 1024) return DSGCN_EUNSUPPORTED;
    hipLaunchKernelGGL(k_rowmean_stats, dim3((unsigned)((long)n * Co)), dim3(64), l2, st, z, zaug,
                       stats ? partial + (size_t)conv_rows * Co * 2 : (float*)nullptr, Co, Tout, V);
    DSGCN_LAUNCH_CHECK();
  }
  return 0;
}

int dsgcn_pwconv_fwd(const float* x1, const float* s1, const float* h1, const float* x2, const float* s2,
                     const float* h2, int relu, const float* w, const float* bias, float* z, float* zaug,
                     float* partial, int n, int Ci, int Co, int T, int V, int stride, int aug, int stats,
                     void* stream) {
  return dsgcn_pwconv_fwd_ws(x1, s1, h1, x2, s2, h2, relu, w, bias, z, zaug, partial, n, Ci, Co, T, V, stride, aug, stats,
                             nullptr, stream);
}

size_t dsgcn_pwconv_wsplit_bytes(int n, int Ci, int Co, int T, int V, int stride) {
  if (n <= 0 || Ci <= 0 || Co <= 0 || T <= 0 || V <= 0 || stride != 1 || (g_pw4 & 3) != 3) return 0;
  return dsgcn_p4_ws_bytes(n, Ci, Co, T * V);
}

int dsgcn_pwconv_wsplit(const float* w, int Ci, int Co, void* ws, void* stream) {
  if (!w || !ws || Ci <= 0 || Co <= 0) return DSGCN_EINVAL;
  return dsgcn_p4_wsplit(w, Ci, Co, ws, (hipStream_t)stream);
}

int dsgcn_pwconv_wsplit_multi(const float* const* w, void* const* ws, const int* Ci, const int* Co, int njobs,
                              void* stream) {
  if (!w || !ws || !Ci || !Co || njobs <= 0) return DSGCN_EINVAL;
  for (int j = 0; j < njobs; ++j)
    if (!w[j] || !ws[j] || Ci[j] <= 0 || Co[j] <= 0) return DSGCN_EINVAL;
  return dsgcn_p4_wsplit_multi(w, ws, Ci, Co, njobs, (hipStream_t)stream);
}

int dsgcn_bn_finalize(const float* partial, int nblk, int C, double count, const float* gamma, const float* beta,
                      float eps, float* mean_out, float* var_out, float* scale_out, float* shift_out, int c_affine,
                      void* stream) {
  if (!partial || !mean_out || !var_out || !scale_out || !shift_out || nblk <= 0 || C <= 0) return DSGCN_EINVAL;
  hipLaunchKernelGGL(k_bn_finalize, dim3((unsigned)((C + 7) / 8)), dim3(1024), 0, (hipStream_t)stream, partial, nblk,
                     C, count, gamma, beta, eps, mean_out, var_out, scale_out, shift_out, c_affine);
  DSGCN_LAUNCH_CHECK();
  return 0;
}

int dsgcn_pwconv_group_ok(int n, int Ci, int Co, int T, int V) {
  if (n <= 0 || Ci <= 0 || Co <= 0 || T <= 0 || V <= 0) return 0;
// ... 194 lines not shown
    case 1: DSGCN_DGRAD(1, 1); break;
    case 2: DSGCN_DGRAD(2, 1); break;
    case 3: DSGCN_DGRAD(3, 1); break;
    default: DSGCN_DGRAD(4, 1); break;
  }
#undef DSGCN_DGRAD
  DSGCN_LAUNCH_CHECK();
  return 0;
}

int dsgcn_pwconv_wgrad_splits(int n, int Ci, int Co, int T, int V, int stride) {
  const int Tout = (T + stride - 1) / stride;
  if (stride == 1 && (g_pw4 & 4)) {
    const int s = dsgcn_wg2_splits(n, Ci, Co, T * V);
    if (s > 0) return s;
  }
  const int TR = Tout >= WG_TR ? WG_TR : Tout;
  const int chunks = n * ((Tout + TR - 1) / TR);
  const int tiles = ((Co + 63) / 64) * ((Ci + 63) / 64);
  int splits = 512 / tiles;
  if (splits < 1) splits = 1;
  if (splits > chunks) splits = chunks;
  const int per = (chunks + splits - 1) / splits;
  return (chunks + per - 1) / per;
}

int dsgcn_pwconv_wgrad_jobs(const float* x1, const float* s1, const float* h1, const float* x2, const float* s2,
                            const float* h2, int relu, const float* z, const float* zaug, const float* gz,
                            const float* gzaug, const float* A0, const float* B0, float* dwp, float* dbp, int pstride, int n,
                            int Ci, int Co, int T, int V, int stride, int aug, const dsgcn_bn_coef_job* jobs, int njobs,
                            void* stream) {
  if (!x1 || !dwp || !dbp || n <= 0 || Ci <= 0 || Co <= 0 || T <= 0 || V <= 0 || stride <= 0) return DSGCN_EINVAL;
  if ((A0 && (!B0 || !z)) || (aug && A0 && !zaug)) return DSGCN_EINVAL;
  if (njobs < 0 || njobs > BNJ_MAX || (njobs > 0 && !jobs)) return DSGCN_EINVAL;
  BnCoefTable jt = {};
  jt.n = njobs;
  for (int i = 0; i < njobs; ++i) {
    const dsgcn_bn_coef_job& q = jobs[i];
    jt.j[i] = BnCoefJob{q.part, q.mean, q.var, q.gamma, q.coef, q.count, q.eps, q.R, q.C, q.k, q.i_ds, q.i_dh, q.c_affine,
                        q.accumulate};
  }
  if (!bnj_coef_ok(jt)) return DSGCN_EINVAL;
  if (stride == 1 && !aug && (g_pw4 & 4)) {
    if (pstride < Co * Ci) return DSGCN_EINVAL;
    const int fast = dsgcn_wg2(x1, s1, h1, x2, s2, h2, relu, z, gz, A0, B0, dwp, dbp, pstride, n, Ci, Co, T * V,
                               (hipStream_t)stream, &jt);
    if (fast == 1) return 0;
    if (fast != 0) return fast;
  }
  if (njobs) {
    hipLaunchKernelGGL(k_bn_coef_rows_multi, dim3((unsigned)bnj_total_blocks(jt)), dim3(BNJ_NT), 0, (hipStream_t)stream, jt);
    DSGCN_LAUNCH_CHECK();
  }
  if ((long)n * Ci * T * V * 4 >= (1L << 31) - 64 || (long)n * Co * T * V * 4 >= (1L << 31) - 64) return DSGCN_EUNSUPPORTED;
  const int Tout = (T + stride - 1) / stride;
  const int TR = Tout >= WG_TR ? WG_TR : Tout;
  if (TR * V > 16 * WG_J) return DSGCN_EUNSUPPORTED;
  PwBwdArgs a = {};
  a.x1 = x1; a.s1 = s1; a.h1 = h1; a.x2 = x2; a.s2 = s2; a.h2 = h2; a.relu = relu;
  a.z = z; a.zaug = zaug; a.gz = gz; a.gzaug = gzaug; a.A0 = A0; a.B0 = B0; a.dwp = dwp; a.dbp = dbp;
  a.pstride = pstride;
  if (pstride < Co * Ci) return DSGCN_EINVAL;
  a.n = n; a.Ci = Ci; a.Co = Co; a.T = T; a.V = V; a.Tout = Tout; a.stride = stride; a.aug = aug; a.TR = TR;
  a.nb_per_sample = (Tout + TR - 1) / TR;
  a.total_chunks = n * a.nb_per_sample;
  a.vec = (stride == 1 && (T * V) % 4 == 0 && (Tout * V) % 4 == 0 && (TR * V) % 4 == 0 &&
           ((Tout % TR) * V) % 4 == 0) ? 1 : 0;
  const int splits = dsgcn_pwconv_wgrad_splits(n, Ci, Co, T, V, stride);
  a.chunks_per_split = (a.total_chunks + splits - 1) / splits;
  const int KP = (TR * V + 1) & ~1;
  const int LS = KP | 1;
  const size_t lds = (size_t)2 * 64 * LS * sizeof(float);
  dim3 grid((unsigned)((Co + 63) / 64), (unsigned)((Ci + 63) / 64), (unsigned)splits);
  a.nbx = a.cc = 0;
  if (grid.x * grid.y > 1 && splits % 8 == 0 && (g_pw_roll & 8)) {
    a.nbx = (int)grid.x; a.cc = (int)grid.y;
    grid = dim3(grid.x * grid.y * (unsigned)splits);
  }
  hipStream_t st = (hipStream_t)stream;
  if (a.vec && x2) hipLaunchKernelGGL((k_pwconv_wgrad<true, true>), grid, dim3(PW_NT), lds, st, a);
  else if (a.vec) hipLaunchKernelGGL((k_pwconv_wgrad<true, false>), grid, dim3(PW_NT), lds, st, a);
  else if (x2) hipLaunchKernelGGL((k_pwconv_wgrad<false, true>), grid, dim3(PW_NT), lds, st, a);
  else hipLaunchKernelGGL((k_pwconv_wgrad<false, false>), grid, dim3(PW_NT), lds, st, a);
  DSGCN_LAUNCH_CHECK();
  return 0;
}

int dsgcn_pwconv_wgrad(const float* x1, const float* s1, const float* h1, const float* x2, const float* s2,
                       const float* h2, int relu, const float* z, const float* zaug, const float* gz,
                       const float* gzaug, const float* A0, const float* B0, float* dwp, float* dbp, int pstride, int n,
                       int Ci, int Co, int T, int V, int stride, int aug, void* stream) {
  return dsgcn_pwconv_wgrad_jobs(x1, s1, h1, x2, s2, h2, relu, z, zaug, gz, gzaug, A0, B0, dwp, dbp, pstride, n, Ci, Co, T, V,
                                 stride, aug, nullptr, 0, stream);
}

int dsgcn_dz_eff_aug(const float* gz, const float* z, const float* gzaug, const float* zaug, const float* A0,
                     const float* B0, float* out, int n, int C, int T, int V, void* stream) {
  if (!z || !zaug || !out || n <= 0 || C <= 0 || T <= 0 || V <= 0) return DSGCN_EINVAL;
  if ((T * V) % 4 == 0 && T <= 8192) {
    hipLaunchKernelGGL(k_dz_eff_aug4, dim3((unsigned)((long)n * C)), dim3(64), (size_t)T * 4, (hipStream_t)stream, gz, z,
                       gzaug, zaug, A0, B0, out, C, T, V);
    DSGCN_LAUNCH_CHECK();
    return 0;
  }
  hipLaunchKernelGGL(k_dz_eff_aug, dim3((unsigned)((long)n * C)), dim3(64), 0, (hipStream_t)stream, gz, z, gzaug, zaug,
                     A0, B0, out, C, T, V);
  DSGCN_LAUNCH_CHECK();
  return 0;
}

int dsgcn_bn_bwd_coef(const float* g_scale, const float* g_shift, const float* mean, const float* var,
                      const float* gamma, float eps, double count, int C, int c_affine, float* dgamma, float* dbeta,
                      float* A0, float* B0, void* stream) {
  if (!mean || !var || !dgamma || !dbeta || !A0 || !B0 || C <= 0) return DSGCN_EINVAL;
  hipLaunchKernelGGL(k_bn_bwd_coef, dim3((unsigned)((C + 63) / 64)), dim3(64), 0, (hipStream_t)stream, g_scale,
                     g_shift, mean, var, gamma, eps, count, C, c_affine, dgamma, dbeta, A0, B0);
  DSGCN_LAUNCH_CHECK();
  return 0;
}

int dsgcn_bn_coef_rows(const float* part, int R, int C, int k, int i_ds, int i_dh, const float* mean, const float* var,
                       const float* gamma, float eps, double count, int c_affine, float* coef, int accumulate,
                       void* stream) {
  if (!part || !mean || !var || !coef || R <= 0 || C <= 0 || k <= 0 || i_ds < 0 || i_ds >= k || i_dh < 0 || i_dh >= k)
    return DSGCN_EINVAL;
  hipLaunchKernelGGL(k_bn_coef_rows, dim3((unsigned)((C + 7) / 8)), dim3(1024), 0, (hipStream_t)stream, part, R, C, k, i_ds,
                     i_dh, mean, var, gamma, eps, count, c_affine, coef, accumulate);
  DSGCN_LAUNCH_CHECK();
  return 0;
}

}


extern "C" {

int dsgcn_pwconv_bwd_rows(int n, int Ci, int Co, int T, int V, int stride) {
  if (stride != 1 || !(g_pw4 & 8) || n <= 0 || T <= 0 || V <= 0) return 0;
  return dsgcn_bwd64_splits(n, Ci, Co, T * V);
}

int dsgcn_pwconv_bwd(const float* x1, const float* s1, const float* h1, const float* x2, const float* s2, const float* h2,
                     int relu, const float* w, const float* z, const float* gz, const float* A0, const float* B0,
                     float* dx1, float* dx2, float* ipart, float* dwp, float* dbp, int pstride, int n, int Ci, int Co,
                     int T, int V, void* stream) {
  if (!x1 || !w || !gz || !dx1 || !dwp || !dbp || n <= 0 || Ci <= 0 || Co <= 0 || T <= 0 || V <= 0) return DSGCN_EINVAL;
  if ((A0 && (!B0 || !z)) || (s1 && !h1) || (s2 && !h2) || (x2 && !dx2) || pstride < Co * Ci) return DSGCN_EINVAL;
  const int rc = dsgcn_bwd64(x1, s1, h1, x2, s2, h2, relu, w, z, gz, A0, B0, dx1, dx2, dwp, dbp, pstride, ipart, n, Ci, Co,
                             T * V, (hipStream_t)stream);
  if (rc == 1) return 0;
  return rc == 0 ? DSGCN_EUNSUPPORTED : rc;
}

}
```

ds-gcn_amd/kernels.py:

```python
import contextlib
import sys

_active = None


def ops():
    return _active if _active is not None else sys.modules[__name__]


@contextlib.contextmanager
def use_ops(namespace):
    global _active
    prev = _active
    _active = namespace
    try:
        yield namespace
    finally:
        _active = prev


NAME = 'hip'

import torch

# ... 254 lines not shown
        job = jobs.get(key)
        if job is None:
            if len(jobs) > self.limit:
                for k in [k for k, j in jobs.items() if not j['pinned']]:
                    del jobs[k]
            job = jobs[key] = dict(stamp=None, used=0, pinned=False, **alloc())
        job['src'] = src
        if capturing:
            job['pinned'] = True
        stamp = (ws['epoch'], self._versions(src))
        job['used'] = ws['epoch']
        if job['stamp'] == stamp:
            return job
        if self.batched != ws['epoch'] and job['stamp'] is not None:
            self.batched = ws['epoch']
            for k in [k for k, j in jobs.items() if j['used'] < ws['epoch'] - 1 and j is not job and not j['pinned']]:
                del jobs[k]
            todo = [j for k, j in jobs.items() if k[2] == dev and j['stamp'] is not None]
            self.launch(todo)
            for j in todo:
                j['stamp'] = (ws['epoch'], self._versions(j['src']))
                if capturing:
                    j['pinned'] = True
            if job['stamp'] == stamp:
                return job
        self.launch([job])
        job['stamp'] = stamp
        return job


class deferred_param_sums:

    def __init__(self, flat=None):
        self.flat = flat

    def __enter__(self):
        global _deferred
        if self.flat is not None:
            if not self.flat.gather:
                raise RuntimeError('deferred_param_sums needs FlatParams(gather=True): with gradient views autograd '
                                   'accumulates in place, before the deferred sums are filled')
            if any(p.grad is not None for p in self.flat.params):
                raise RuntimeError('deferred_param_sums: a parameter already holds a .grad — call zero_grad() first '
                                   '(gradient accumulation over several backward passes is not supported here)')
        self.prev = _deferred
        _deferred = []
        return self

    def __exit__(self, *exc):
        global _deferred
        try:
            if exc[0] is None:
                flush_param_sums()
        finally:
            _deferred = self.prev
            _leaf_uses.clear()
            _post_flush.clear()
            _ctr_fin_queue.clear()
        return False


_post_flush = []


def flush_param_sums():
    global _deferred
    queued = _deferred
    if queued:
        _deferred = [] if _deferred is not None else None
        for level in sorted({j[4] for j in queued}):
            _flush_jobs([j[:4] for j in queued if j[4] == level])
    hooks = list(_post_flush)
    _post_flush.clear()
    for h in hooks:
        h()


def _flush_jobs(jobs):
    import numpy as _np
    k = len(jobs)
    tab = _np.empty((k, 4), dtype=_np.int64)
    blk = 0
    nblocks = native.lib().dsgcn_colsum_blocks
    for i, (src, R, C, out) in enumerate(jobs):
        tab[i] = (src.data_ptr(), out.data_ptr(), (R << 32) | C, blk)
        blk += nblocks(src.data_ptr(), C)
    native.check(native.lib().dsgcn_colsum_multi_host(tab.ctypes.data, k, _stream()), 'dsgcn_colsum_multi_host')


def param_colsum(t, defer_ok=True, level=0):
    if _deferred is None or not defer_ok or not t.is_cuda:
        return colsum(t)
    R = t.shape[0]
    shape = t.shape[1:]
    C = t.numel() // max(R, 1)
    g = _fold(R, C)
    out = torch.empty(C, device=t.device, dtype=torch.float32)
    if g > 1:
        mid = torch.empty(g * C, device=t.device, dtype=torch.float32)
        _deferred.append((t, R // g, g * C, mid, level))
        _deferred.append((mid, g, C, out, level + 1))
    else:
        _deferred.append((t, R, C, out, level))
    return out.view(shape)


class _CatRows(torch.autograd.Function):

    @staticmethod
    def forward(ctx, *ts):
        ctx.rows = [t.shape[0] for t in ts]
        t0 = ts[0]
        adjacent = all(t.is_contiguous() and t.dtype == t0.dtype and t.device == t0.device and
                       t.shape[1:] == t0.shape[1:] for t in ts)
        if adjacent:
            esz = t0.element_size()
            base = t0.untyped_storage().data_ptr()
            for a, b in zip(ts[:-1], ts[1:]):
                if b.untyped_storage().data_ptr() != base or a.data_ptr() + a.numel() * esz != b.data_ptr():
                    adjacent = False
                    break
        if not adjacent:
            return torch.cat(ts, 0)
        size = (sum(ctx.rows),) + tuple(t0.shape[1:])
        stride = []
        acc = 1
        for d in reversed(size):
            stride.append(acc)
            acc *= d
        return torch.as_strided(t0.detach(), size, tuple(reversed(stride)))

    @staticmethod
    def backward(ctx, g):
        return tuple(g.split(ctx.rows, 0))


def cat_rows(tensors):
    tensors = list(tensors)
    return tensors[0] if len(tensors) == 1 else _CatRows.apply(*tensors)


def _f32c(t):
    if t is None:
        return None
    if t.dtype != torch.float32:
        raise TypeError(f'dsgcn kernels compute in fp32, got {t.dtype}')
    return t if t.is_contiguous() else t.contiguous()


BN_FEED = _os.environ.get('DSGCN_BN_FEED', '1') != '0'


class BNCtx:
    __slots__ = ('mean', 'var', 'gamma', 'eps', 'count', 'C', 'n_affine', 'coef', 'host', 'queued')

    def __init__(self):
        self.coef = None
        self.host = False
        self.queued = None


def _bn_attach(scale, bn, mean, var, gamma, eps, count, n_affine):
    if bn is None or scale is None or not BN_FEED:
        return
    bn.mean, bn.var, bn.gamma, bn.eps, bn.count = mean, var, gamma, float(eps), float(count)
    bn.C, bn.n_affine = int(scale.numel()), int(n_affine)
    scale._dsgcn_bn = bn


def _bn_of(scale):
    return getattr(scale, '_dsgcn_bn', None) if (scale is not None and BN_FEED) else None


BN_BATCH = _os.environ.get('DSGCN_BN_BATCH', '1') == '1'
_fin_queue = None
_coef_wait = []


def _fin_job(partial, rows, Co, count, gamma, beta, eps, mean, var, scale, shift, n_affine):
    j = native.BnFinJob(_ptr(partial), _ptr(gamma), _ptr(beta), _ptr(mean), _ptr(var), _ptr(scale), _ptr(shift), float(count),
                        float(eps), int(rows), int(Co), int(n_affine))
    j._keep = (partial, gamma, beta, mean, var, scale, shift)
    return j


def _launch_fin(jobs):
    lib = native.lib()
    for i in range(0, len(jobs), native.BN_JOBS_MAX):
        chunk = jobs[i:i + native.BN_JOBS_MAX]
        arr = (native.BnFinJob * len(chunk))(*chunk)
        native.check(lib.dsgcn_bn_finalize_multi(arr, len(chunk), _stream()), 'dsgcn_bn_finalize_multi')


def bn_finalize(partial, rows, Co, count, gamma, beta, eps, mean, var, scale, shift, n_affine):
    if _fin_queue is not None:
        _fin_queue.append(_fin_job(partial, rows, Co, count, gamma, beta, eps, mean, var, scale, shift, n_affine))
        return
    rc = native.lib().dsgcn_bn_finalize(_ptr(partial), rows, Co, count, _ptr(gamma), _ptr(beta), float(eps), _ptr(mean),
                                        _ptr(var), _ptr(scale), _ptr(shift), int(n_affine), _stream())
    native.check(rc, 'dsgcn_bn_finalize')


class bn_batch:

    def __init__(self):
        self.jobs = []
        self._stack = []

    def _enter(self, flush):
        global _fin_queue
        self._stack.append((_fin_queue, flush))
        if BN_BATCH:
            _fin_queue = self.jobs
        return self

    def __enter__(self):
        return self._enter(True)

    def hold(self):
        outer = self

        class _Hold:
            def __enter__(self):
                return outer._enter(False)

            def __exit__(self, *exc):
                return outer.__exit__(*exc)
        return _Hold()

    def take(self):
        jobs, self.jobs[:] = list(self.jobs), []
        return jobs

    def flush(self):
        jobs = self.take()
        if jobs:
            _launch_fin(jobs)

    def __exit__(self, *exc):
        global _fin_queue
        _fin_queue, flush = self._stack.pop()
        if exc[0] is not None:
            self.jobs[:] = []
        elif flush:
            self.flush()
        return False


def _coef_job(bn, part, k, i_ds, i_dh):
    C = bn.C
    R = part.numel() // (C * k)
    acc = bn.coef is not None
    if not acc:
        bn.coef = torch.empty((4, C), device=part.device, dtype=torch.float32)
    j = native.BnCoefJob(_ptr(part), _ptr(bn.mean), _ptr(bn.var), _ptr(bn.gamma), _ptr(bn.coef), float(bn.count),
                         float(bn.eps), int(R), int(C), int(k), int(i_ds), int(i_dh), int(bn.n_affine), int(acc))
    j._keep = (part, bn.mean, bn.var, bn.gamma, bn.coef)
    return j


def _launch_coef(jobs):
    lib = native.lib()
    for i in range(0, len(jobs), native.BN_JOBS_MAX):
        chunk = jobs[i:i + native.BN_JOBS_MAX]
        arr = (native.BnCoefJob * len(chunk))(*chunk)
        native.check(lib.dsgcn_bn_coef_rows_multi(arr, len(chunk), _stream()), 'dsgcn_bn_coef_rows_multi')


def _flush_coef_wait():
    if _coef_wait:
        jobs = [j for _, j in _coef_wait]
        for bn, _ in _coef_wait:
            bn.queued = None
        _coef_wait.clear()
        _launch_coef(jobs)


def _bn_feed(bn, part, k, i_ds, i_dh):
    _bn_feed_multi([(bn, part, k, i_ds, i_dh)])


def _job_array(jobs):
    return ((native.BnCoefJob * len(jobs))(*jobs) if jobs else None), len(jobs)


def _bn_feed_multi(feeds, launch=True):
    if not BN_BATCH:
        for bn, part, k, i_ds, i_dh in feeds:
            C = bn.C
            R = part.numel() // (C * k)
            acc = bn.coef is not None
            if not acc:
                bn.coef = torch.empty((4, C), device=part.device, dtype=torch.float32)
            rc = native.lib().dsgcn_bn_coef_rows(_ptr(part), R, C, k, i_ds, i_dh, _ptr(bn.mean), _ptr(bn.var), _ptr(bn.gamma),
                                                 bn.eps, bn.count, bn.n_affine, _ptr(bn.coef), int(acc), _stream())
            native.check(rc, 'dsgcn_bn_coef_rows')
        return []
    now = []
    for bn, part, k, i_ds, i_dh in feeds:
        if bn.queued is not None:
            _flush_coef_wait()
        job = _coef_job(bn, part, k, i_ds, i_dh)
        if bn.host:
            bn.queued = job
            _coef_wait.append((bn, job))
        else:
            now.append(job)
    if not launch and len(now) <= native.BN_JOBS_MAX:
        return now
    if now:
        _launch_coef(now)
    return []


def _bn_coef(bn, gscale, gshift, mean, var, gamma, eps, count, C, n_affine):
    coef = None
    if bn is not None:
        if bn.queued is not None:
            _flush_coef_wait()
        coef, bn.coef = bn.coef, None
    if gscale is not None or gshift is not None:
        c2 = torch.empty((4, C), device=mean.device, dtype=torch.float32)
        rc = native.lib().dsgcn_bn_bwd_coef(_ptr(gscale), _ptr(gshift), _ptr(mean), _ptr(var), _ptr(gamma), eps, count, C,
                                            n_affine, _ptr(c2[0]), _ptr(c2[1]), _ptr(c2[2]), _ptr(c2[3]), _stream())
# ... 97 lines not shown
                                       _ptr(edge_type), _ptr(dahat), _ptr(dd), _ptr(dproj), _ptr(ppar), pstride, n, mid, V,
                                       ld, P, E, arr, len(jobs), _stream())
        native.check(rc, 'dsgcn_dynadj_bwd_jobs')
        red = param_colsum(ppar, ctx.defer_ok)
        o = 3 * V * V
        dA, dalpha, dbeta = red[:o].view(3, V, V), red[o:o + 3], red[o + 3:o + 6]
        dwe = red[o + 6:o + 6 + E * mid * mid].view(E * mid, mid)
        dbe = red[o + 6 + E * mid * mid:o + 6 + E * mid * mid + E * mid]
        return dproj, dA, dalpha, dbeta, dwe, dbe, None, None, None, None


def _kb_projections(xbar, V, weights, biases):
    w_all = cat_rows(weights)
    b_all = cat_rows(biases)
    xpad = torch.nn.functional.pad(xbar, (0, 32 - V)) if xbar.shape[-1] < 32 else xbar
    proj = pwconv(xpad.unsqueeze(2), None, None, None, False, w_all, b_all, 1, False)[0]
    return proj.view(xbar.shape[0], w_all.shape[0], xpad.shape[-1])


def dynadj(xbar, A, alpha, beta, w1, b1, w2, b2, wse, bse, we, be, node_type, edge_type, single_use=True, host=None):
    proj = _kb_projections(xbar, A.shape[-1], [w1, w2, wse], [b1, b2, bse])
    return _DynAdj.apply(proj, A, alpha, beta, we, be, node_type, edge_type, bool(single_use), host)


class _TypedSelect(torch.autograd.Function):

    @staticmethod
    def forward(ctx, proj, node_type, KM, P, V):
        _require_cuda(proj)
        proj = _f32c(proj)
        n, _, ld = proj.shape
        x12 = torch.empty((n, KM, 2, 32), device=proj.device, dtype=torch.float32)
        native.check(native.lib().dsgcn_dyntyped_select_fwd(_ptr(proj), _ptr(node_type), _ptr(x12), n, KM, P, V, ld,
                                                            _stream()), 'dsgcn_dyntyped_select_fwd')
        ctx.save_for_backward(node_type)
        ctx.dims = (tuple(proj.shape), KM, P, V)
        return x12

    @staticmethod
    def backward(ctx, dx12):
        node_type, = ctx.saved_tensors
        shape, KM, P, V = ctx.dims
        dx12 = _f32c(dx12)
        dproj = torch.empty(shape, device=dx12.device, dtype=torch.float32)
        native.check(native.lib().dsgcn_dyntyped_select_bwd(_ptr(dx12), _ptr(node_type), _ptr(dproj), shape[0], KM, P, V,
                                                            shape[2], _stream()), 'dsgcn_dyntyped_select_bwd')
        return dproj, None, None, None, None


class _TypedAdj(torch.autograd.Function):

    @staticmethod
    def forward(ctx, x12, pq, be, A, alpha, beta, edge_type, flags, defer_ok):
        _require_cuda(x12, A)
        x12, pq, be, A, alpha, beta = [_f32c(t) for t in (x12, pq, be, A, alpha, beta)]
        n, KM = x12.shape[:2]
        mid, V = KM // 3, A.shape[-1]
        E = pq.shape[1] // KM if pq is not None else 0
        ahat = torch.empty((n, KM, V, V), device=x12.device, dtype=torch.float32)
        rc = native.lib().dsgcn_dyntyped_fwd(_ptr(x12), _ptr(pq), _ptr(be), _ptr(A), _ptr(alpha), _ptr(beta),
                                             _ptr(edge_type), _ptr(ahat), n, mid, V, E, flags, _stream())
        native.check(rc, 'dsgcn_dyntyped_fwd')
        ctx.save_for_backward(x12, pq, be, alpha, beta, edge_type)
        ctx.dims = (n, mid, V, E, flags)
        ctx.defer_ok = defer_ok
        return ahat

    @staticmethod
    def backward(ctx, dahat):
        x12, pq, be, alpha, beta, edge_type = ctx.saved_tensors
        n, mid, V, E, flags = ctx.dims
        dahat = _f32c(dahat)
        lib = native.lib()
        dd = torch.empty_like(dahat)
        dx12 = torch.empty_like(x12)
        dpq = torch.empty_like(pq) if pq is not None else None
        pstride = lib.dsgcn_dyntyped_partial_stride(mid, V, E, flags)
        ppar = torch.empty((n, pstride), device=x12.device, dtype=torch.float32)
        rc = lib.dsgcn_dyntyped_bwd(_ptr(x12), _ptr(pq), _ptr(be), _ptr(alpha), _ptr(beta), _ptr(edge_type), _ptr(dahat),
                                    _ptr(dd), _ptr(dx12), _ptr(dpq), _ptr(ppar), pstride, n, mid, V, E, flags, _stream())
        native.check(rc, 'dsgcn_dyntyped_bwd')
        red = param_colsum(ppar, bool(ctx.defer_ok))
        o = 3 * V * V
        dA, dalpha, dbeta = red[:o].view(3, V, V), red[o:o + 3], red[o + 3:o + 6]
        dbe = red[o + 6:o + 6 + E * 3 * mid] if pq is not None else None
        return dx12, dpq, dbe, dA, dalpha, dbeta, None, None, None


def dynadj_typed(xbar, A, alpha, beta, w1, b1, w2, b2, we, be, node_type, edge_type, P, add_type, single_use=True):
    V = A.shape[-1]
    proj = _kb_projections(xbar, V, [w1, w2], [b1, b2])
    x12 = _TypedSelect.apply(proj, node_type, w1.shape[0] // P, P, V)
    pq, flags = None, 0
    if we is not None:
        pq = pwconv(x12, None, None, None, False, we, None, 1, False)[0]
        flags = 1 | (2 if add_type else 0)
    defer_ok = bool(single_use) and _leafish(A, alpha, beta, be)
    return _TypedAdj.apply(x12, pq, be if we is not None else None, A, alpha, beta, edge_type, flags, defer_ok)



import ctypes as _ct


def _pw_plan(Tout, V, aug):
    tr, npad, nb = _ct.c_int(), _ct.c_int(), _ct.c_int()
    native.check(native.lib().dsgcn_pwconv_plan(Tout, V, int(aug), _ct.byref(tr), _ct.byref(npad), _ct.byref(nb)),
                 'dsgcn_pwconv_plan')
    return tr.value, npad.value, nb.value


class _PwConv(torch.autograd.Function):

    @staticmethod
    def forward(ctx, x1, s1, h1, x2, s2, h2, relu, weight, bias, stride, aug, gamma, beta, eps, n_affine, want_bn,
                bn=None, out=None):
        _require_cuda(x1, weight)
        ctx.bn, ctx.bn1, ctx.bn2 = bn, _bn_of(s1), _bn_of(s2)
        x1, s1, h1, x2, s2, h2, bias, gamma, beta = [_f32c(t) for t in (x1, s1, h1, x2, s2, h2, bias, gamma, beta)]
        w2 = _f32c(weight.reshape(weight.shape[0], -1))
        n, Ci, T, V = x1.shape
        Co = w2.shape[0]
        assert w2.shape[1] == Ci, (w2.shape, x1.shape)
        Tout = (T + stride - 1) // stride
        dev = x1.device
        if out is not None:
            z = out.t
            if (tuple(z.shape) != (n, Co, Tout, V) or z.dtype != torch.float32 or not z.is_contiguous() or z.device != dev
                    or z.requires_grad):
                raise ValueError(f'pwconv(out=): expected a contiguous fp32 {(n, Co, Tout, V)} slice without history')
        else:
            z = torch.empty((n, Co, Tout, V), device=dev, dtype=torch.float32)
        zaug = torch.empty((n, Co, Tout), device=dev, dtype=torch.float32) if aug else None
        lib = native.lib()
        partial = None
        if want_bn:
            rows = lib.dsgcn_pwconv_partial_rows(n, Ci, Co, T, V, stride, int(aug))
            partial = torch.empty((rows, Co, 2), device=dev, dtype=torch.float32)
        ws = None
        wsb = lib.dsgcn_pwconv_wsplit_bytes(n, Ci, Co, T, V, stride)
        if wsb:
            ws = _wsplit_image(w2, Ci, Co, wsb)
        rc = lib.dsgcn_pwconv_fwd_ws(_ptr(x1), _ptr(s1), _ptr(h1), _ptr(x2), _ptr(s2), _ptr(h2), int(relu), _ptr(w2),
                                     _ptr(bias), _ptr(z), _ptr(zaug), _ptr(partial), n, Ci, Co, T, V, stride, int(aug),
                                     int(want_bn), _ptr(ws), _stream())
        native.check(rc, 'dsgcn_pwconv_fwd_ws')
        scale = shift = mean = var = None
        count = float(n * Tout * (V + (1 if aug else 0)))
        if want_bn:
            stats = torch.empty((4, Co), device=dev, dtype=torch.float32)
            mean, var, scale, shift = stats[0], stats[1], stats[2], stats[3]
            bn_finalize(partial, partial.shape[0], Co, count, gamma, beta, eps, mean, var, scale, shift, n_affine)
            ctx.mark_non_differentiable(mean, var)
        ctx.set_materialize_grads(False)
        ctx.save_for_backward(x1, s1, h1, x2, s2, h2, w2, z, zaug, gamma, mean, var, ws)
        ctx.cfg = (int(relu), stride, int(aug), float(eps), int(n_affine), bool(want_bn), count, tuple(weight.shape),
                   bias is not None, beta is not None)
        ctx.defer_ok = _leafish(weight, bias)
        sink = getattr(weight, '_dsgcn_sink', None)
        if sink is not None and not (bias is None and s2 is None and (s1 is None or getattr(s1, '_dsgcn_sink', None) is sink)):
            sink = None
        ctx.sink = sink
        return z, zaug, scale, shift, mean, var

    @staticmethod
    def backward(ctx, gz, gzaug, gscale, gshift, _gm, _gv):
        x1, s1, h1, x2, s2, h2, w2, z, zaug, gamma, mean, var, ws = ctx.saved_tensors
        relu, stride, aug, eps, n_affine, want_bn, count, wshape, has_bias, has_beta = ctx.cfg
        n, Ci, T, V = x1.shape
        Co = w2.shape[0]
        dev = x1.device
        lib = native.lib()
        st = _stream()
        gz, gzaug, gscale, gshift = _f32c(gz), _f32c(gzaug), _f32c(gscale), _f32c(gshift)
        A0 = B0 = dgamma = dbeta = None
        if want_bn:
            dgamma, dbeta, A0, B0 = _bn_coef(ctx.bn, gscale, gshift, mean, var, gamma, eps, count, Co, n_affine)
        Tout = z.shape[2]
        if gz is None:
            gz = torch.zeros_like(z)
        if aug:
            dzeff = torch.empty_like(z)
            rc = lib.dsgcn_dz_eff_aug(_ptr(gz), _ptr(z), _ptr(gzaug), _ptr(zaug), _ptr(A0), _ptr(B0), _ptr(dzeff), n,
                                      Co, Tout, V, st)
            native.check(rc, 'dsgcn_dz_eff_aug')
            gz, gzaug, A0, B0, aug = dzeff, None, None, None, 0
        dx1 = torch.empty_like(x1)
        dx2 = torch.empty_like(x2) if x2 is not None else None
        pstride = Co * Ci + Co
        rows = lib.dsgcn_pwconv_bwd_rows(n, Ci, Co, T, V, stride) if (not aug and gz is not None) else 0
        if rows > 0:
            wpart = torch.empty((rows, pstride), device=dev, dtype=torch.float32)
            ipart = (torch.empty((rows, Ci, 3), device=dev, dtype=torch.float32)
                     if (s1 is not None or s2 is not None) else None)
            rc = lib.dsgcn_pwconv_bwd(_ptr(x1), _ptr(s1), _ptr(h1), _ptr(x2), _ptr(s2), _ptr(h2), relu, _ptr(w2), _ptr(z),
                                      _ptr(gz), _ptr(A0), _ptr(B0), _ptr(dx1), _ptr(dx2), _ptr(ipart), wpart.data_ptr(),
                                      wpart.data_ptr() + 4 * Co * Ci, pstride, n, Ci, Co, T, V, st)
            native.check(rc, 'dsgcn_pwconv_bwd')
            return _PwConv._finish(wpart, ipart, dx1, dx2, s1, s2, Co, Ci, wshape, has_bias, dgamma, dbeta, gamma,
                                   has_beta, n_affine, ctx.defer_ok, ctx.bn1, ctx.bn2, ctx.sink is not None and bool(ctx.sink))
        ipart = None
        if s1 is not None or s2 is not None:
            rows = lib.dsgcn_pwconv_ipart_rows(n, Ci, Co, T, V, stride)
            ipart = torch.empty((rows, Ci, 3), device=dev, dtype=torch.float32)
        rc = lib.dsgcn_pwconv_dgrad_ws(_ptr(x1), _ptr(s1), _ptr(h1), _ptr(x2), _ptr(s2), _ptr(h2), relu, _ptr(w2),
                                       _ptr(z), _ptr(zaug), _ptr(gz), _ptr(gzaug), _ptr(A0), _ptr(B0), _ptr(dx1),
                                       _ptr(dx2), _ptr(ipart), n, Ci, Co, T, V, stride, aug, _ptr(ws), st)
        native.check(rc, 'dsgcn_pwconv_dgrad_ws')
        splits = lib.dsgcn_pwconv_wgrad_splits(n, Ci, Co, T, V, stride)
        pstride = Co * Ci + Co
        wpart = torch.empty((splits, pstride), device=dev, dtype=torch.float32)
        sink = ctx.sink is not None and bool(ctx.sink)
        hosted, fed = [], False
        if (ipart is not None and not (sink and _deferred is not None) and (s1 is None or ctx.bn1 is not None) and
                (s2 is None or ctx.bn2 is not None)):
            hosted = _bn_feed_multi(([(ctx.bn1, ipart, 3, 0, 1)] if s1 is not None else []) +
                                    ([(ctx.bn2, ipart, 3, 2, 1)] if s2 is not None else []), launch=False)
            fed = True
        rc = lib.dsgcn_pwconv_wgrad_jobs(_ptr(x1), _ptr(s1), _ptr(h1), _ptr(x2), _ptr(s2), _ptr(h2), relu, _ptr(z),
                                         _ptr(zaug), _ptr(gz), _ptr(gzaug), _ptr(A0), _ptr(B0), wpart.data_ptr(),
                                         wpart.data_ptr() + 4 * Co * Ci, pstride, n, Ci, Co, T, V, stride, aug,
                                         *_job_array(hosted), st)
        native.check(rc, 'dsgcn_pwconv_wgrad_jobs')
        return _PwConv._finish(wpart, ipart, dx1, dx2, s1, s2, Co, Ci, wshape, has_bias, dgamma, dbeta, gamma, has_beta,
                               n_affine, ctx.defer_ok, ctx.bn1, ctx.bn2, sink, fed)

    @staticmethod
    def _finish(wpart, ipart, dx1, dx2, s1, s2, Co, Ci, wshape, has_bias, dgamma, dbeta, gamma, has_beta, n_affine,
                defer_ok=False, bn1=None, bn2=None, sink=False, already_fed=False):
        if sink and _deferred is not None:
            wsum = param_colsum(wpart, True)
            ds1 = dh1 = None
            if ipart is not None:
                red = param_colsum(ipart.view(ipart.shape[0], -1), True).view(Ci, 3)
                ds1, dh1 = red[:, 0], red[:, 1]
            return (dx1, ds1, dh1, dx2, None, None, None, wsum[:Co * Ci].view(wshape), None, None, None, None, None, None,
                    None, None, None, None)
        fed = ipart is not None and (s1 is None or bn1 is not None) and (s2 is None or bn2 is not None)
        if fed and already_fed:
            ipart = None
        elif fed:
            _bn_feed_multi(([(bn1, ipart, 3, 0, 1)] if s1 is not None else []) + ([(bn2, ipart, 3, 2, 1)] if s2 is not None else []))
            ipart = None
        if ipart is not None and (_deferred is None or not defer_ok):
            wsum, red = colsum_pair(wpart, ipart, split_last_b=True)
        elif ipart is not None:
            red = colsum(ipart, split_last=True)
            wsum = param_colsum(wpart, True)
        else:
            wsum = param_colsum(wpart, defer_ok)
        dw = wsum[:Co * Ci].view(wshape)
        db = wsum[Co * Ci:] if has_bias else None
        ds1 = dh1 = ds2 = dh2 = None
        if ipart is not None:
            if s1 is not None:
                ds1, dh1 = red[0], red[1]
            if s2 is not None:
                ds2, dh2 = red[2], red[1]
        if dgamma is not None:
            dgamma = dgamma[:n_affine] if gamma is not None else None
            dbeta = dbeta[:n_affine] if has_beta else None
        return (dx1, ds1, dh1, dx2, ds2, dh2, None, dw, db, None, None, dgamma, dbeta, None, None, None, None, None)


class _PwConvGroup(torch.autograd.Function):

    @staticmethod
    def forward(ctx, K, slots, *ts):
        xs, ss, hs, ws = ts[:K], ts[K:2 * K], ts[2 * K:3 * K], ts[3 * K:4 * K]
        _require_cuda(*xs, *ws)
        xs = [_f32c(t) for t in xs]
        ss = [_f32c(t) for t in ss]
        hs = [_f32c(t) for t in hs]
        w2 = [_f32c(w.reshape(w.shape[0], -1)) for w in ws]
        n, Ci, T, V = xs[0].shape
        Co = w2[0].shape[0]
        zs = [sl.t for sl in slots]
        for z in zs:
            if tuple(z.shape) != (n, Co, T, V) or z.dtype != torch.float32 or not z.is_contiguous() or z.requires_grad:
                raise ValueError(f'pwconv_group(out=): expected contiguous fp32 {(n, Co, T, V)} slices without history')
        rc = native.lib().dsgcn_pwconv_fwd_group(_ptr_array(xs), _ptr_array(ss), _ptr_array(hs), 0, _ptr_array(w2),
                                                 _ptr_array(zs), K, n, Ci, Co, T, V, _stream())
        native.check(rc, 'dsgcn_pwconv_fwd_group')
        ctx.save_for_backward(*xs, *ss, *hs, *w2)
        ctx.K = K
        ctx.wshapes = [tuple(w.shape) for w in ws]
        ctx.defer_ok = [_leafish(w) for w in ws]
        sinks = []
        for w, s1 in zip(ws, ss):
            sink = getattr(w, '_dsgcn_sink', None)
            if sink is not None and not (s1 is None or getattr(s1, '_dsgcn_sink', None) is sink):
                sink = None
            sinks.append(sink)
        ctx.sinks = sinks
        ctx.set_materialize_grads(False)
        return tuple(zs)

    @staticmethod
    def backward(ctx, *gzs):
        K = ctx.K
        sv = ctx.saved_tensors
        xs, ss, hs, w2 = sv[:K], sv[K:2 * K], sv[2 * K:3 * K], sv[3 * K:4 * K]
        n, Ci, T, V = xs[0].shape
        Co = w2[0].shape[0]
        dev = xs[0].device
        lib = native.lib()
        st = _stream()
        gzs = [_f32c(g) if g is not None else torch.zeros((n, Co, T, V), device=dev, dtype=torch.float32) for g in gzs]
        dxs = [torch.empty_like(x) for x in xs]
        has_s = ss[0] is not None
        rows = lib.dsgcn_pwconv_ipart_rows(n, Ci, Co, T, V, 1) if has_s else 0
        iparts = [torch.empty((rows, Ci, 3), device=dev, dtype=torch.float32) if has_s else None for _ in range(K)]
        rc = lib.dsgcn_pwconv_dgrad_group(_ptr_array(xs), _ptr_array(ss), _ptr_array(hs), 0, _ptr_array(w2), _ptr_array(gzs),
                                          _ptr_array(dxs), _ptr_array(iparts), K, n, Ci, Co, T, V, st)
        native.check(rc, 'dsgcn_pwconv_dgrad_group')
        splits = lib.dsgcn_pwconv_wgrad_splits(n, Ci, Co, T, V, 1)
        pstride = Co * Ci + Co
        out_x, out_s, out_h, out_w = [], [], [], []
        wparts = [torch.empty((splits, pstride), device=dev, dtype=torch.float32) for _ in range(K)]
        dwp = (_ct.c_void_p * K)(*[w.data_ptr() for w in wparts])
        dbp = (_ct.c_void_p * K)(*[w.data_ptr() + 4 * Co * Ci for w in wparts])
        rc = -2
        if GROUP_WGRAD:
            rc = lib.dsgcn_pwconv_wgrad_group(_ptr_array(xs), _ptr_array(ss), _ptr_array(hs), 0, _ptr_array(gzs), dwp, dbp,
                                              pstride, K, n, Ci, Co, T, V, st)
        if rc == -2:
            for k in range(K):
                rc = lib.dsgcn_pwconv_wgrad(_ptr(xs[k]), _ptr(ss[k]), _ptr(hs[k]), None, None, None, 0, None, None,
                                            _ptr(gzs[k]), None, None, None, wparts[k].data_ptr(),
                                            wparts[k].data_ptr() + 4 * Co * Ci, pstride, n, Ci, Co, T, V, 1, 0, st)
                native.check(rc, 'dsgcn_pwconv_wgrad')
        else:
            native.check(rc, 'dsgcn_pwconv_wgrad_group')
        for k in range(K):
            wpart = wparts[k]
            sink = ctx.sinks[k] is not None and bool(ctx.sinks[k])
            r = _PwConv._finish(wpart, iparts[k], dxs[k], None, ss[k], None, Co, Ci, ctx.wshapes[k], False, None, None, None,
                                False, 0, ctx.defer_ok[k], None, None, sink)
            out_x.append(r[0]); out_s.append(r[1]); out_h.append(r[2]); out_w.append(r[7])
        return (None, None, *out_x, *out_s, *out_h, *out_w)


def pwconv_group(xs, affs, ws, slots):
    K = len(xs)
    n, Ci, T, V = xs[0].shape
    Co = ws[0].shape[0]
    same = all(x.shape == xs[0].shape for x in xs) and all(w.shape == ws[0].shape for w in ws)
    if (GROUP_CONVS and 2 <= K <= 3 and same and xs[0].is_cuda and
            native.lib().dsgcn_pwconv_group_ok(n, Ci, Co, T, V) == 1):
        ss = [a[0] if a is not None else None for a in affs]
        hs = [a[1] if a is not None else None for a in affs]
        return list(_PwConvGroup.apply(K, list(slots), *xs, *ss, *hs, *ws))
    return [pwconv(x, a, None, None, False, w, None, 1, False, out=sl)[0] for x, a, w, sl in zip(xs, affs, ws, slots)]


GROUP_CONVS = _os.environ.get('DSGCN_GROUP_CONVS', '1') == '1'
GROUP_WGRAD = _os.environ.get('DSGCN_GROUP_WGRAD', '1') == '1'


class OutSlot:
    __slots__ = ('t',)

    def __init__(self, t):
        self.t = t


def pwconv(x1, a1, x2, a2, relu, weight, bias, stride=1, aug=False, gamma=None, beta=None, eps=1e-5, n_affine=None,
           want_bn=False, out=None):
    s1, h1 = a1 if a1 is not None else (None, None)
    s2, h2 = a2 if a2 is not None else (None, None)
    if n_affine is None:
        n_affine = weight.shape[0] if gamma is not None else 0
    bn = BNCtx() if want_bn else None
    out = _PwConv.apply(x1, s1, h1, x2, s2, h2, bool(relu), weight, bias, int(stride), bool(aug), gamma, beta,
                        float(eps), int(n_affine), bool(want_bn), bn, out)
    if want_bn:
        Tout = out[0].shape[2]
        count = float(x1.shape[0] * Tout * (x1.shape[3] + (1 if aug else 0)))
        _bn_attach(out[2], bn, out[4], out[5], gamma, eps, count, n_affine)
    return out



def tmean(x, ld=True):
    _require_cuda(x)
    return fuse_out(x, None, None, None, 0, ld)[1]


class _BranchAct(torch.autograd.Function):

    @staticmethod
    def forward(ctx, z, zaug, scale, shift, n_act):
        _require_cuda(z)
        z, zaug, scale, shift = [_f32c(t) for t in (z, zaug, scale, shift)]
        n, C, T, V = z.shape
        h = torch.empty((n, C, T, V + (1 if zaug is not None else 0)), device=z.device, dtype=torch.float32)
        rc = native.lib().dsgcn_branch_act_fwd(_ptr(z), _ptr(zaug), _ptr(scale), _ptr(shift), int(n_act), _ptr(h), n, C,
                                               T, V, _stream())
        native.check(rc, 'dsgcn_branch_act_fwd')
        ctx.save_for_backward(z, zaug, scale, shift)
        ctx.n_act = int(n_act)
        ctx.bn = _bn_of(scale)
        return h

    @staticmethod
    def backward(ctx, dh):
        z, zaug, scale, shift = ctx.saved_tensors
        n, C, T, V = z.shape
        dh = _f32c(dh)
        dz = torch.empty_like(z)
        dzaug = torch.empty_like(zaug) if zaug is not None else None
        part = torch.empty((n, C, 2), device=z.device, dtype=torch.float32)
        rc = native.lib().dsgcn_branch_act_bwd(_ptr(z), _ptr(zaug), _ptr(scale), _ptr(shift), ctx.n_act, _ptr(dh),
                                               _ptr(dz), _ptr(dzaug), _ptr(part), n, C, T, V, _stream())
        native.check(rc, 'dsgcn_branch_act_bwd')
        if ctx.bn is not None:
            _bn_feed(ctx.bn, part, 2, 0, 1)
            return dz, dzaug, None, None, None
        red = colsum(part, split_last=True)
        return dz, dzaug, red[0], red[1], None


class _TmsCombine(torch.autograd.Function):

    @staticmethod
    def forward(ctx, o, coeff, gamma, beta, eps, want_bn, bn=None):
        _require_cuda(o)
        ctx.bn = bn
        o, coeff, gamma, beta = [_f32c(t) for t in (o, coeff, gamma, beta)]
        n, C, T, V1 = o.shape
        V = V1 - 1
        dev = o.device
        f = torch.empty((n, C, T, V), device=dev, dtype=torch.float32)
        partial = torch.empty((n, C, 2), device=dev, dtype=torch.float32) if want_bn else None
        lib = native.lib()
        rc = lib.dsgcn_tms_combine_fwd(_ptr(o), _ptr(coeff), _ptr(f), _ptr(partial), n, C, T, V, _stream())
        native.check(rc, 'dsgcn_tms_combine_fwd')
        scale = shift = mean = var = None
        count = float(n * T * V)
        if want_bn:
            stats = torch.empty((4, C), device=dev, dtype=torch.float32)
            mean, var, scale, shift = stats[0], stats[1], stats[2], stats[3]
            rc = lib.dsgcn_bn_finalize(_ptr(partial), n, C, count, _ptr(gamma), _ptr(beta), float(eps), _ptr(mean),
                                       _ptr(var), _ptr(scale), _ptr(shift), C, _stream())
            native.check(rc, 'dsgcn_bn_finalize')
            ctx.mark_non_differentiable(mean, var)
        ctx.set_materialize_grads(False)
        ctx.save_for_backward(o, coeff, gamma, mean, var)
        ctx.cfg = (float(eps), bool(want_bn), count, beta is not None)
        ctx.defer_ok = _leafish(coeff)
        return f, scale, shift, mean, var

    @staticmethod
    def backward(ctx, gf, gscale, gshift, _gm, _gv):
        o, coeff, gamma, mean, var = ctx.saved_tensors
        eps, want_bn, count, has_beta = ctx.cfg
        n, C, T, V1 = o.shape
        V = V1 - 1
        dev = o.device
        lib = native.lib()
        gf, gscale, gshift = _f32c(gf), _f32c(gscale), _f32c(gshift)
        A0 = B0 = dgamma = dbeta = None
        if want_bn:
            dgamma, dbeta, A0, B0 = _bn_coef(ctx.bn, gscale, gshift, mean, var, gamma, eps, count, C, C)
        do = torch.empty_like(o)
        pcoef = torch.empty((n * C, V), device=dev, dtype=torch.float32)
        rc = lib.dsgcn_tms_combine_bwd(_ptr(o), _ptr(coeff), _ptr(gf), _ptr(A0), _ptr(B0), _ptr(do), _ptr(pcoef), n, C,
                                       T, V, _stream())
        native.check(rc, 'dsgcn_tms_combine_bwd')
        dcoeff = param_colsum(pcoef, ctx.defer_ok)
        if dgamma is not None:
            dgamma = dgamma if gamma is not None else None
            dbeta = dbeta if has_beta else None
        return do, dcoeff, dgamma, dbeta, None, None, None


def _int_array(vals):
    return (_ct.c_int * len(vals))(*vals)


def _ptr_array(tensors):
    return (_ct.c_void_p * len(tensors))(*[None if t is None else t.data_ptr() for t in tensors])


class _TapBranches(torch.autograd.Function):

    @staticmethod
    def forward(ctx, h, stride, KT, Cout, types, ci0s, co0s, cins, couts, dils, *wb):
        _require_cuda(h)
        h = _f32c(h)
        n, Cin, T, V1 = h.shape
        nbr = len(types)
        ws = [_f32c(t) for t in wb[:nbr]]
        bs = [_f32c(t) for t in wb[nbr:]]
        Tout = (T + stride - 1) // stride
        o = torch.empty((n, Cout, Tout, V1), device=h.device, dtype=torch.float32)
        rc = native.lib().dsgcn_tapconv_fwd(_ptr(h), _ptr(o), n, Cin, Cout, T, V1, stride, KT, nbr, _int_array(types),
                                            _int_array(ci0s), _int_array(co0s), _int_array(cins), _int_array(couts),
                                            _int_array(dils), _ptr_array(ws), _ptr_array(bs), _stream())
        native.check(rc, 'dsgcn_tapconv_fwd')
        ctx.save_for_backward(h, *[w for w in ws if w is not None])
        ctx.cfg = (stride, KT, Cout, tuple(types), tuple(ci0s), tuple(co0s), tuple(cins), tuple(couts), tuple(dils),
                   tuple(b is not None for b in bs))
        ctx.defer_ok = _leafish(*wb)
        return o

    @staticmethod
    def backward(ctx, go):
        h, *wsaved = ctx.saved_tensors
        stride, KT, Cout, types, ci0s, co0s, cins, couts, dils, has_b = ctx.cfg
        n, Cin, T, V1 = h.shape
        nbr = len(types)
        go = _f32c(go)
        lib = native.lib()
        it = iter(wsaved)
        ws = [next(it) if t == 0 else None for t in types]
        tabs = (_int_array(types), _int_array(ci0s), _int_array(co0s), _int_array(cins), _int_array(couts),
                _int_array(dils))
        dh = torch.empty_like(h)
        rc = lib.dsgcn_tapconv_dgrad(_ptr(h), _ptr(go), _ptr(dh), n, Cin, Cout, T, V1, stride, KT, nbr, *tabs,
                                     _ptr_array(ws), _stream())
        native.check(rc, 'dsgcn_tapconv_dgrad')
        Tout = go.shape[2]
        if 0 not in types:
            return (dh, None, None, None, None, None, None, None, None, None, *([None] * (2 * nbr)))
        offs, off = [], 0
# ... 1008 lines not shown

def ctr_topology(xbar, w1, b1, w2, b2, w4, b4, alpha, A, beta=None, edge=None, subset_major=False):
    n, Ci, V = xbar.shape
    K = A.shape[0]
    R = w1.shape[0] // K
    proj = pwconv(xbar.unsqueeze(2), None, None, None, False, cat_rows([w1, w2]), cat_rows([b1, b2]), 1,
                  False)[0].view(n, 2 * K * R, V)
    if subset_major and CTR_ONE_CONV and beta is None and not edge and alpha.numel() == 1 and K <= 4:
        d = _TanhDiffAug.apply(proj, A, K, R)
        use = _leafish(alpha, *w4, *b4)
        prep = _CtrWPrep.apply(use, alpha, *w4, *b4)
        for t in prep[:2 * K]:
            t._dsgcn_sink = use
        Co = w4[0].shape[0]
        buf = torch.empty((K, n, Co, V, V), device=xbar.device, dtype=torch.float32)
        parts = pwconv_group([d[k] for k in range(K)], [(prep[K + k], prep[2 * K + k]) for k in range(K)],
                             [prep[k] for k in range(K)], [OutSlot(buf[k]) for k in range(K)])
        return _JoinSlices.apply(OutSlot(buf), *parts)
    d = _TanhDiff.apply(proj, K, R)
    S = []
    for k in range(K):
        dk = d[k]
        if edge and k in edge:
            we, be, et = edge[k]
            dk = _EdgeSelect.apply(pwconv(dk, None, None, None, False, we, be, 1, False)[0], et, R)
        S.append(pwconv(dk, None, None, None, False, w4[k], b4[k], 1, False)[0])
    G = None
    if beta is not None:
        x1 = proj[:, :K * R].reshape(n * K, R, 1, V)
        x2 = proj[:, K * R:].reshape(n * K, R, 1, V)
        G = ops().gram(x1, x2).view(n, K, V, V)
    return _CtrAffine.apply(alpha, A, beta, G, *S)


class _Tee3(torch.autograd.Function):

    @staticmethod
    def forward(ctx, x):
        ctx.set_materialize_grads(False)
        return x.view_as(x), x.view_as(x), x.view_as(x)

    @staticmethod
    def backward(ctx, ga, gb, gc):
        gs = [_f32c(g) for g in (ga, gb, gc) if g is not None]
        if not gs:
            return None
        if len(gs) == 1:
            return gs[0]
        out = torch.empty_like(gs[0])
        rc = native.lib().dsgcn_add3(_ptr(gs[0]), _ptr(gs[1]), _ptr(gs[2]) if len(gs) > 2 else None, _ptr(out),
                                     out.numel(), _stream())
        native.check(rc, 'dsgcn_add3')
        return out


def tee3(x):
    _require_cuda(x)
    if not x.requires_grad:
        return x, x, x
    return _Tee3.apply(x)


class Prestrided:
    __slots__ = ('x', 'stride', 'frames')

    def __init__(self, x, stride, frames):
        if x.shape[2] != (frames + stride - 1) // stride:
            raise ValueError(f'Prestrided: {x.shape[2]} frames are not every {stride}-th of {frames}')
        self.x, self.stride, self.frames = x, int(stride), int(frames)


FUSE_OUT_LDS_BYTES = 64 * 1024


def prestrided_fits(T, V):
    return T * V * 4 <= FUSE_OUT_LDS_BYTES


_drop_state = {'call': 0, 'step': {}, 'used': False}


def _dropout_record(p, device):
    st = _drop_state
    if device not in st['step']:
        st['step'][device] = torch.zeros((), dtype=torch.int64, device=device)
    st['call'] = (st['call'] + 1) & 0x7fffffff
    st['used'] = True
    step = st['step'][device]
    return native.Dropout(step.data_ptr(), int(torch.initial_seed()) & 0xffffffffffffffff, st['call'], float(p)), step


def dropout_step_advance():
    if _drop_state['used']:
        for step in _drop_state['step'].values():
            step.add_(1)


def dropout_mask(numel, rec):
    dev = next(iter(_drop_state['step']))
    out = torch.empty(numel, device=dev, dtype=torch.float32)
    native.check(native.lib().dsgcn_dropout_mask(_ptr(out), numel, _ct.byref(rec), _stream()), 'dsgcn_dropout_mask')
    return out


class _FuseOut(torch.autograd.Function):

    @staticmethod
    def forward(ctx, x1, s1, h1, x2, s2, h2, relu, xbar_ld, tee, dropout=0.0):
        _require_cuda(x1)
        x1, s1, h1, x2, s2, h2 = [_f32c(t) for t in (x1, s1, h1, x2, s2, h2)]
        n, C, T, V = x1.shape
        if x2 is not None and x2.shape != x1.shape:
            raise ValueError(f'fuse_out: the two terms differ in shape: {tuple(x1.shape)} vs {tuple(x2.shape)}')
        out = torch.empty_like(x1)
        out_s2 = torch.empty((n, C, (T + 1) // 2, V), device=x1.device, dtype=torch.float32) if tee == 2 else None
        xbar = torch.empty((n, C, xbar_ld), device=x1.device, dtype=torch.float32) if xbar_ld else None
        ctx.drop = _dropout_record(dropout, x1.device) if dropout > 0 else None
        rc = native.lib().dsgcn_fuse_out_fwd_drop(_ptr(x1), _ptr(s1), _ptr(h1), _ptr(x2), _ptr(s2), _ptr(h2), int(relu),
                                                  _ptr(out), _ptr(out_s2), _ptr(xbar), None, n, C, T, V, int(xbar_ld),
                                                  _ct.byref(ctx.drop[0]) if ctx.drop else None, _stream())
        native.check(rc, 'dsgcn_fuse_out_fwd_drop')
        ctx.save_for_backward(x1, s1, h1, x2, s2, h2)
        ctx.relu = int(relu)
        ctx.xbar_ld = int(xbar_ld)
        ctx.tee = int(tee)
        ctx.bn1, ctx.bn2 = _bn_of(s1), _bn_of(s2)
        ctx.set_materialize_grads(False)
        if tee == 2:
            return out, out.view_as(out), out_s2, xbar
        if tee:
            return out, out.view_as(out), out.view_as(out), xbar
        return out, None, None, xbar

    @staticmethod
    def backward(ctx, dout, dout2, dout3, dxbar):
        x1, s1, h1, x2, s2, h2 = ctx.saved_tensors
        n, C, T, V = x1.shape
        stride3 = 1
        for g, frames in ((dout, T), (dout2, T), (dout3, (T + 1) // 2 if ctx.tee == 2 else T)):
            if g is not None and tuple(g.shape) != (n, C, frames, V):
                raise ValueError(f'fuse_out backward: gradient of shape {tuple(g.shape)}, expected {(n, C, frames, V)}')
        if ctx.tee == 2:
            d3 = _f32c(dout3)
            full = [_f32c(g) for g in (dout, dout2) if g is not None]
            if d3 is not None and not full:
                full = [torch.zeros_like(x1)]
            douts = full + [None] * (2 - len(full)) + [d3]
            stride3 = 2 if d3 is not None else 1
        else:
            douts = [_f32c(g) for g in (dout, dout2, dout3) if g is not None]
            douts += [None] * (3 - len(douts))
        dxbar = _f32c(dxbar)
        dx1 = torch.empty_like(x1)
        dx2 = torch.empty_like(x2) if x2 is not None else None
        need_part = s1 is not None or s2 is not None
        part = torch.empty((n, C, 4), device=x1.device, dtype=torch.float32) if need_part else None
        rc = native.lib().dsgcn_fuse_out_bwd_drop(_ptr(x1), _ptr(s1), _ptr(h1), _ptr(x2), _ptr(s2), _ptr(h2), ctx.relu,
                                                  _ptr(douts[0]), _ptr(douts[1]), _ptr(douts[2]), stride3, _ptr(dxbar),
                                                  _ptr(dx1), _ptr(dx2), _ptr(part), n, C, T, V, ctx.xbar_ld or V,
                                                  _ct.byref(ctx.drop[0]) if ctx.drop else None, _stream())
        native.check(rc, 'dsgcn_fuse_out_bwd_drop')
        ds1 = dh1 = ds2 = dh2 = None
        if need_part and (s1 is None or ctx.bn1 is not None) and (s2 is None or ctx.bn2 is not None):
            _bn_feed_multi(([(ctx.bn1, part, 4, 0, 3)] if s1 is not None else []) +
                           ([(ctx.bn2, part, 4, 2, 1)] if s2 is not None else []))
        elif need_part:
            red = colsum(part, split_last=True)
            if s1 is not None:
                ds1, dh1 = red[0], red[3]
            if s2 is not None:
                ds2, dh2 = red[2], red[1]
        return dx1, ds1, dh1, dx2, ds2, dh2, None, None, None, None


class _FuseOutPool(torch.autograd.Function):

    @staticmethod
    def forward(ctx, x1, s1, h1, x2, s2, h2, relu, dropout=0.0):
        _require_cuda(x1)
        x1, s1, h1, x2, s2, h2 = [_f32c(t) for t in (x1, s1, h1, x2, s2, h2)]
        n, C, T, V = x1.shape
        if x2 is not None and x2.shape != x1.shape:
            raise ValueError(f'fuse_out_pool: the two terms differ in shape: {tuple(x1.shape)} vs {tuple(x2.shape)}')
        pm = torch.empty((n, C), device=x1.device, dtype=torch.float32)
        ctx.drop = _dropout_record(dropout, x1.device) if dropout > 0 else None
        rc = native.lib().dsgcn_fuse_out_fwd_drop(_ptr(x1), _ptr(s1), _ptr(h1), _ptr(x2), _ptr(s2), _ptr(h2), int(relu),
                                                  None, None, None, _ptr(pm), n, C, T, V, V,
                                                  _ct.byref(ctx.drop[0]) if ctx.drop else None, _stream())
        native.check(rc, 'dsgcn_fuse_out_fwd_drop')
        ctx.save_for_backward(x1, s1, h1, x2, s2, h2)
        ctx.relu = int(relu)
        ctx.bn1, ctx.bn2 = _bn_of(s1), _bn_of(s2)
        return pm

    @staticmethod
    def backward(ctx, dpm):
        x1, s1, h1, x2, s2, h2 = ctx.saved_tensors
        n, C, T, V = x1.shape
        dpm = _f32c(dpm)
        dx1 = torch.empty_like(x1)
        dx2 = torch.empty_like(x2) if x2 is not None else None
        need_part = s1 is not None or s2 is not None
        part = torch.empty((n, C, 4), device=x1.device, dtype=torch.float32) if need_part else None
        rc = native.lib().dsgcn_fuse_out_bwd_drop(_ptr(x1), _ptr(s1), _ptr(h1), _ptr(x2), _ptr(s2), _ptr(h2), ctx.relu,
                                                  _ptr(dpm), None, None, 3, None, _ptr(dx1), _ptr(dx2), _ptr(part), n, C, T, V,
                                                  V, _ct.byref(ctx.drop[0]) if ctx.drop else None, _stream())
        native.check(rc, 'dsgcn_fuse_out_bwd_drop')
        ds1 = dh1 = ds2 = dh2 = None
        if need_part and (s1 is None or ctx.bn1 is not None) and (s2 is None or ctx.bn2 is not None):
            _bn_feed_multi(([(ctx.bn1, part, 4, 0, 3)] if s1 is not None else []) +
                           ([(ctx.bn2, part, 4, 2, 1)] if s2 is not None else []))
        elif need_part:
            red = colsum(part, split_last=True)
            if s1 is not None:
                ds1, dh1 = red[0], red[3]
            if s2 is not None:
                ds2, dh2 = red[2], red[1]
        return dx1, ds1, dh1, dx2, ds2, dh2, None, None


DROPOUT_FUSED = _os.environ.get('DSGCN_DROPOUT_FUSED', '1') != '0'


def fuse_out_pool(x1, a1, x2, a2, relu, dropout=0.0):
    s1, h1 = a1 if a1 is not None else (None, None)
    s2, h2 = a2 if a2 is not None else (None, None)
    return _FuseOutPool.apply(x1, s1, h1, x2, s2, h2, int(relu), float(dropout))


def fuse_out(x1, a1, x2, a2, relu, want_tmean=False, tee=False, dropout=0.0):
    s1, h1 = a1 if a1 is not None else (None, None)
    s2, h2 = a2 if a2 is not None else (None, None)
    ld = 0 if not want_tmean else (x1.shape[-1] if want_tmean is True else int(want_tmean))
    o1, o2, o3, xbar = _FuseOut.apply(x1, s1, h1, x2, s2, h2, int(relu), ld, int(tee), float(dropout))
    if int(tee) == 2:
        o3 = Prestrided(o3, 2, x1.shape[2])
    return ((o1, o2, o3) if tee else o1), xbar


class _HeadLoss(torch.autograd.Function):

    @staticmethod
    def forward(ctx, feat, weight, bias, label, M, loss_weight):
        _require_cuda(feat, weight, label)
        feat, weight, bias = _f32c(feat), _f32c(weight), _f32c(bias)
        if label.dtype != torch.int64 or not label.is_contiguous():
            label = label.to(torch.int64).contiguous()
        R, C = feat.shape
        K = weight.shape[0]
        if R % M or weight.shape[1] != C or label.numel() * M != R:
            raise ValueError(f'head_loss: feat {tuple(feat.shape)}, weight {tuple(weight.shape)}, {label.numel()} labels, '
                             f'{M} persons do not fit together')
        N = R // M
        dev = feat.device
        pooled = torch.empty((N, C), device=dev, dtype=torch.float32)
        score = torch.empty((N, K), device=dev, dtype=torch.float32)
        prob = torch.empty((N, K), device=dev, dtype=torch.float32)
        clip = torch.empty((N, 3), device=dev, dtype=torch.float32)
        loss = torch.empty((), device=dev, dtype=torch.float32)
        acc = torch.empty(2, device=dev, dtype=torch.float64)
        rc = native.lib().dsgcn_head_loss_fwd(_ptr(feat), _ptr(weight), _ptr(bias), _ptr(label), N, M, C, K,
                                              float(loss_weight), _ptr(pooled), _ptr(score), _ptr(prob), _ptr(clip),
                                              _ptr(loss), _ptr(acc), _stream())
        native.check(rc, 'dsgcn_head_loss_fwd')
        ctx.save_for_backward(prob, pooled, weight, label)
        ctx.dims = (N, M, C, K, float(loss_weight), bias is not None)
        ctx.mark_non_differentiable(acc, score)
        ctx.set_materialize_grads(False)
        return loss, acc, score

    @staticmethod
    def backward(ctx, gloss, _gacc, _gscore):
        if gloss is None:
            return None, None, None, None, None, None
        prob, pooled, weight, label = ctx.saved_tensors
        N, M, C, K, lw, has_bias = ctx.dims
        dev = prob.device
        gloss = _f32c(gloss)
        dfeat = torch.empty((N * M, C), device=dev, dtype=torch.float32)
        dw = torch.empty((K, C), device=dev, dtype=torch.float32)
        db = torch.empty(K, device=dev, dtype=torch.float32)
        rc = native.lib().dsgcn_head_loss_bwd(_ptr(prob), _ptr(pooled), _ptr(weight), _ptr(label), _ptr(gloss), N, M, C, K,
                                              lw, _ptr(dfeat), _ptr(dw), _ptr(db), _stream())
        native.check(rc, 'dsgcn_head_loss_bwd')
        return dfeat, dw, (db if has_bias else None), None, None, None


def head_loss(feat, weight, bias, label, persons, loss_weight=1.0):
    return _HeadLoss.apply(feat, weight, bias, label, int(persons), float(loss_weight))


def bn_running_update(items):
    import ctypes as _c
    k = len(items)
    ptrs = lambda ts: (_c.c_void_p * k)(*[None if t is None else t.data_ptr() for t in ts])
    for bn, mean, var, _ in items:
        _require_cuda(bn.running_mean, mean, var)
        for t in (bn.running_mean, bn.running_var, mean, var):
            if t.dtype != torch.float32 or not t.is_contiguous() or t.numel() != bn.num_features:
                raise ValueError('bn_running_update: fp32 contiguous per-channel vectors expected')
    nbt = [bn.num_batches_tracked for bn, _, _, _ in items]
    rc = native.lib().dsgcn_bn_running_multi(
        ptrs([bn.running_mean for bn, _, _, _ in items]), ptrs([bn.running_var for bn, _, _, _ in items]),
        ptrs([m for _, m, _, _ in items]), ptrs([v for _, _, v, _ in items]), ptrs(nbt),
        _int_array([bn.num_features for bn, _, _, _ in items]),
        (_c.c_float * k)(*[c / max(c - 1.0, 1.0) for _, _, _, c in items]),
        (_c.c_float * k)(*[float(bn.momentum) for bn, _, _, _ in items]), k, _stream())
    native.check(rc, 'dsgcn_bn_running_multi')


class _DataBN(torch.autograd.Function):

    @staticmethod
    def forward(ctx, x, gamma, beta, bn, mvc, training):
# ... 57 lines not shown
```

ds-gcn_amd/native.py:

```python
import ctypes
import glob
import os
import subprocess

_HERE = os.path.dirname(os.path.abspath(__file__))
CSRC = os.path.join(_HERE, 'csrc')
LIB_DIR = os.path.join(_HERE, 'lib')
LIB_PATH = os.path.join(LIB_DIR, 'libdsgcn.so')
LAB_LIB_PATH = os.path.join(LIB_DIR, 'libdsgcn_lab.so')
INCLUDE = os.path.join(os.path.dirname(_HERE), 'include')

_lib = None
_lab = None

c_f = ctypes.c_void_p
c_i = ctypes.c_void_p
c_int = ctypes.c_int
c_st = ctypes.c_void_p

SIGNATURES = {
    'dsgcn_version': [],
    'dsgcn_aggregate_fwd': [c_f, c_f, c_f, c_int, c_f, c_f, c_int, c_int, c_int, c_int, c_st],
    'dsgcn_aggregate_bwd_partial_rows': [c_int, c_int, c_int],
    'dsgcn_aggregate_bwd': [c_f, c_f, c_f, c_int, c_f, c_f, c_f, c_f, c_f, c_int, c_int, c_int, c_int, c_st],
    'dsgcn_pwconv_plan': [c_int, c_int, c_int, ctypes.POINTER(ctypes.c_int), ctypes.POINTER(ctypes.c_int),
                          ctypes.POINTER(ctypes.c_int)],
    'dsgcn_pwconv_fwd': [c_f] * 6 + [c_int] + [c_f] * 5 + [c_int] * 8 + [c_st],
    'dsgcn_bn_coef_rows': [c_f, c_int, c_int, c_int, c_int, c_int, c_f, c_f, c_f, ctypes.c_float, ctypes.c_double, c_int, c_f, c_int, c_st],
    'dsgcn_pwconv_fwd_ws': [c_f] * 6 + [c_int] + [c_f] * 5 + [c_int] * 8 + [c_f, c_st],
    'dsgcn_pwconv_wsplit': [c_f, c_int, c_int, c_f, c_st],
    'dsgcn_pwconv_wsplit_multi': [ctypes.c_void_p, ctypes.c_void_p, ctypes.POINTER(ctypes.c_int),
                                  ctypes.POINTER(ctypes.c_int), c_int, c_st],
    'dsgcn_pwconv_wsplit_bytes': [c_int] * 6,
    'dsgcn_tconv_ws_bytes': [c_int] * 7,
    'dsgcn_tconv_wsplit': [c_f, c_int, c_int, c_int, c_f, c_st],
    'dsgcn_tconv_wsplit_multi': [ctypes.c_void_p, c_int, c_st],
    'dsgcn_tconv_rows': [c_int] * 8,
    'dsgcn_tconv_fwd': [c_f] * 6 + [c_int] + [c_f] * 4 + [c_int] * 7 + [c_st],
    'dsgcn_tconv_dgrad': [c_f] * 6 + [c_int] + [c_f] * 8 + [c_int] * 7 + [c_st],
    'dsgcn_tconv_wgrad_splits': [c_int] * 7,
    'dsgcn_tconv_wgrad': [c_f] * 6 + [c_int] + [c_f] * 4 + [ctypes.c_void_p] * 2 + [c_int] * 8 + [c_st],
    'dsgcn_bn_finalize': [c_f, c_int, c_int, ctypes.c_double, c_f, c_f, ctypes.c_float, c_f, c_f, c_f, c_f, c_int,
                          c_st],
    'dsgcn_pwconv_partial_rows': [c_int] * 7,
    'dsgcn_pwconv_ipart_rows': [c_int] * 6,
    'dsgcn_dz_eff_aug': [c_f] * 7 + [c_int] * 4 + [c_st],
    'dsgcn_colsum': [c_f, c_int, c_int, c_f, c_st],
    'dsgcn_colsum_t': [c_f, c_int, c_int, c_int, c_f, c_st],
    'dsgcn_colsum_blocks': [c_f, c_int],
    'dsgcn_colsum_multi': [c_f, c_int, c_int, c_st],
    'dsgcn_colsum2': [c_f, c_int, c_int, c_int, c_f, c_f, c_int, c_int, c_int, c_f, c_st],
    'dsgcn_pwconv_dgrad': [c_f] * 6 + [c_int] + [c_f] * 10 + [c_int] * 7 + [c_st],
    'dsgcn_pwconv_dgrad_ws': [c_f] * 6 + [c_int] + [c_f] * 10 + [c_int] * 7 + [c_f, c_st],
    'dsgcn_pwconv_wgrad_splits': [c_int] * 6,
    'dsgcn_pwconv_bwd_rows': [c_int] * 6,
    'dsgcn_pwconv_bwd': [c_f] * 6 + [c_int] + [c_f] * 10 + [c_int] * 6 + [c_st],
    'dsgcn_pwconv_wgrad': [c_f] * 6 + [c_int] + [c_f] * 8 + [c_int] * 8 + [c_st],
    'dsgcn_bn_bwd_coef': [c_f] * 5 + [ctypes.c_float, ctypes.c_double, c_int, c_int] + [c_f] * 4 + [c_st],
    'dsgcn_branch_act_fwd': [c_f] * 4 + [c_int] + [c_f] + [c_int] * 4 + [c_st],
    'dsgcn_branch_act_bwd': [c_f] * 4 + [c_int] + [c_f] * 4 + [c_int] * 4 + [c_st],
    'dsgcn_tms_combine_fwd': [c_f] * 4 + [c_int] * 4 + [c_st],
    'dsgcn_tms_combine_bwd': [c_f] * 7 + [c_int] * 4 + [c_st],
    'dsgcn_tapconv_fwd': [c_f, c_f] + [c_int] * 8 + [c_i] * 6 + [ctypes.c_void_p, ctypes.c_void_p, c_st],
    'dsgcn_tapconv_dgrad': [c_f, c_f, c_f] + [c_int] * 8 + [c_i] * 6 + [ctypes.c_void_p, c_st],
    'dsgcn_tapconv_wgrad_splits': [c_int] * 8 + [c_i] * 4,
    'dsgcn_tapconv_wgrad': [c_f, c_f] + [c_int] * 8 + [c_i] * 6 + [ctypes.c_void_p, ctypes.c_void_p, c_int, c_int, c_st],
    'dsgcn_tms_rows': [c_int] * 8 + [c_i] * 3 + [c_int],
    'dsgcn_tms_fwd': [c_f] * 4 + [c_int] + [c_f] * 4 + [c_int] * 7 + [c_i] * 4 + [ctypes.c_void_p, ctypes.c_void_p, c_st],
    'dsgcn_tms_dgrad': [c_f] * 4 + [c_int] + [c_f] * 10 + [c_int] * 7 + [c_i] * 4 + [ctypes.c_void_p, c_st],
    'dsgcn_tms_wgrad': [c_f] * 4 + [c_int] + [c_f] * 5 + [c_int] * 7 + [c_i] * 4 + [ctypes.c_void_p, ctypes.c_void_p, c_int, c_st],
    'dsgcn_tms_split_rows': [c_int] * 8 + [c_i] * 4,
    'dsgcn_tms_split_fwd': [c_f] * 4 + [c_int] + [c_f] * 4 + [c_int] * 6 + [c_i] * 4 + [ctypes.c_void_p, ctypes.c_void_p, c_st],
    'dsgcn_tms_split_prep': [c_f] * 9 + [c_int] * 4 + [c_st],
    'dsgcn_tms_split_dgrad': [c_f] * 4 + [c_int] + [c_f] * 5 + [c_int] * 6 + [c_i] * 4 + [ctypes.c_void_p, c_st],
    'dsgcn_tms_split_wgrad': [c_f] * 4 + [c_int] + [c_f] * 2 + [c_int] * 6 + [c_i] * 4 + [ctypes.c_void_p, ctypes.c_void_p, c_int, c_int, c_st],
    'dsgcn_aggsum_partial_rows': [c_int, c_int, c_int],
    'dsgcn_aggsum_bwd_piece_rows': [c_int] * 5,
    'dsgcn_aggsum_fwd': [c_f, c_f] + [ctypes.c_long] * 3 + [c_f, c_f] + [c_int] * 5 + [c_st],
    'dsgcn_aggsum_bwd': [c_f, c_f] + [ctypes.c_long] * 3 + [c_f] * 6 + [ctypes.c_long] * 3 + [c_int] * 5 + [c_st],
    'dsgcn_tanhdiff_fwd': [c_f, c_f] + [c_int] * 4 + [c_st],
    'dsgcn_tanhdiff_bwd': [c_f, c_f, c_f] + [c_int] * 4 + [c_st],
    'dsgcn_tanhdiff_bwd_k': [c_f, ctypes.c_void_p, c_f] + [c_int] * 4 + [c_st],
    'dsgcn_tanhdiff_aug_fwd': [c_f, c_f, c_f] + [c_int] * 4 + [c_st],
    'dsgcn_tanhdiff_aug_bwd': [c_f, ctypes.c_void_p, c_f, c_f] + [c_int] * 4 + [c_st],
    'dsgcn_ctr_wprep': [ctypes.c_void_p, ctypes.c_void_p, c_f, c_f, c_f] + [c_int] * 3 + [c_st],
    'dsgcn_ctr_wprep_multi': [ctypes.c_void_p, c_int, c_st],
    'dsgcn_ctr_wfin_multi': [ctypes.c_void_p, c_int, c_st],
    'dsgcn_ctr_wfin': [ctypes.c_void_p, ctypes.c_void_p, c_int, ctypes.c_void_p, c_f] + [c_int] * 3 + [c_st],
    'dsgcn_ctr_affine_fwd': [ctypes.c_void_p, c_f, c_int, c_f, c_f, c_f, c_f] + [c_int] * 4 + [c_st],
    'dsgcn_ctr_affine_bwd': [ctypes.c_void_p, c_f, c_int, c_f, ctypes.c_void_p, c_f] + [c_int] * 4 + [c_st],
    'dsgcn_edge_select_fwd': [c_f, c_i, c_f] + [c_int] * 4 + [c_st],
    'dsgcn_edge_select_bwd': [c_f, c_i, c_f] + [c_int] * 4 + [c_st],
    'dsgcn_plane_stats': [c_f, c_f, ctypes.c_long, c_int, c_st],
    'dsgcn_add3': [c_f, c_f, c_f, c_f, ctypes.c_long, c_st],
    'dsgcn_pack': [c_f, c_f, c_f, c_int, c_f, c_st],
    'dsgcn_pack_fill': [c_f, c_f, c_f, c_int, c_f, c_st],
    'dsgcn_colsum_multi_host': [ctypes.c_void_p, c_int, c_st],
    'dsgcn_fuse_out_fwd': [c_f] * 6 + [c_int] + [c_f] * 2 + [c_int] * 5 + [c_st],
    'dsgcn_fuse_out_bwd': [c_f] * 6 + [c_int] + [c_f] * 5 + [c_int] * 5 + [c_st],
    'dsgcn_fuse_out_bwd3': [c_f] * 6 + [c_int] + [c_f] * 7 + [c_int] * 5 + [c_st],
    'dsgcn_fuse_out_fwd2': [c_f] * 6 + [c_int] + [c_f] * 3 + [c_int] * 5 + [c_st],
    'dsgcn_fuse_out_bwd3s': [c_f] * 6 + [c_int] + [c_f] * 3 + [c_int] + [c_f] * 4 + [c_int] * 5 + [c_st],
    'dsgcn_fuse_out_pool_fwd': [c_f] * 6 + [c_int] + [c_f] + [c_int] * 4 + [c_st],
    'dsgcn_fuse_out_pool_bwd': [c_f] * 6 + [c_int] + [c_f] * 4 + [c_int] * 4 + [c_st],
    'dsgcn_dwcausal_fwd': [c_f, c_f, c_f, c_i, c_f] + [c_int] * 6 + [c_st],
    'dsgcn_dwcausal_bwd': [c_f, c_f, c_i, c_f, c_f, c_f] + [c_int] * 6 + [c_st],
    'dsgcn_gate_fwd': [c_f, c_f, c_int, c_f, c_f] + [c_int] * 5 + [c_st],
    'dsgcn_gate_bwd': [c_f, c_f, c_int, c_f, c_f, c_int, c_f, c_f] + [c_int] * 4 + [c_st],
    'dsgcn_skeleton_prep': [ctypes.c_void_p] * 11 + [c_int] * 10 + [c_st],
    'dsgcn_dynadj_partial_stride': [c_int, c_int, c_int],
    'dsgcn_dynadj_fwd': [c_f] * 6 + [c_i, c_i, c_f] + [c_int] * 6 + [c_st],
    'dsgcn_dynadj_bwd': [c_f] * 5 + [c_i, c_i] + [c_f] * 4 + [c_int] * 7 + [c_st],
    'dsgcn_pwconv_group_ok': [c_int] * 5,
    'dsgcn_pwconv_fwd_group': [ctypes.c_void_p] * 3 + [c_int] + [ctypes.c_void_p] * 2 + [c_int] * 6 + [c_st],
    'dsgcn_pwconv_dgrad_group': [ctypes.c_void_p] * 3 + [c_int] + [ctypes.c_void_p] * 4 + [c_int] * 6 + [c_st],
    'dsgcn_pwconv_wgrad_group': [ctypes.c_void_p] * 3 + [c_int] + [ctypes.c_void_p] * 3 + [c_int] * 7 + [c_st],
    'dsgcn_pwconv_wgrad_jobs': [c_f] * 6 + [c_int] + [c_f] * 8 + [c_int] * 8 + [ctypes.c_void_p, c_int, c_st],
    'dsgcn_tms_split_wgrad_jobs': [c_f] * 4 + [c_int] + [c_f] * 2 + [c_int] * 6 + [c_i] * 4 + [ctypes.c_void_p, ctypes.c_void_p, c_int, c_int, ctypes.c_void_p, c_int, c_st],
    'dsgcn_fuse_out_fwd_drop': [c_f] * 6 + [c_int] + [c_f] * 4 + [c_int] * 5 + [ctypes.c_void_p, c_st],
    'dsgcn_fuse_out_bwd_drop': [c_f] * 6 + [c_int] + [c_f] * 3 + [c_int] + [c_f] * 4 + [c_int] * 5 + [ctypes.c_void_p, c_st],
    'dsgcn_dropout_mask': [c_f, ctypes.c_long, ctypes.c_void_p, c_st],
    'dsgcn_bn_finalize_multi': [ctypes.c_void_p, c_int, c_st],
    'dsgcn_bn_coef_rows_multi': [ctypes.c_void_p, c_int, c_st],
    'dsgcn_dyntyped_select_fwd': [c_f, c_i, c_f] + [c_int] * 5 + [c_st],
    'dsgcn_dyntyped_select_bwd': [c_f, c_i, c_f] + [c_int] * 5 + [c_st],
    'dsgcn_dyntyped_partial_stride': [c_int] * 4,
    'dsgcn_dyntyped_fwd': [c_f] * 6 + [c_i, c_f] + [c_int] * 5 + [c_st],
    'dsgcn_dyntyped_bwd': [c_f] * 5 + [c_i] + [c_f] * 5 + [c_int] * 6 + [c_st],
    'dsgcn_dynflag_partial_stride': [c_int] * 4,
    'dsgcn_dynflag_fwd': [c_f] * 8 + [c_i, c_i, c_f] + [c_int] * 7 + [c_st],
    'dsgcn_dynflag_bwd': [c_f] * 7 + [c_i, c_i] + [c_f] * 5 + [c_int] * 8 + [c_st],
    'dsgcn_dynplain_partial_stride': [c_int] * 2,
    'dsgcn_dynplain_fwd': [c_f] * 5 + [c_int] * 5 + [c_st],
    'dsgcn_dynplain_bwd': [c_f] * 6 + [c_int] * 6 + [c_st],
    'dsgcn_dynadj_fwd_jobs': [c_f] * 6 + [c_i, c_i, c_f] + [c_int] * 6 + [ctypes.c_void_p, c_int, c_st],
    'dsgcn_dynadj_bwd_jobs': [c_f] * 5 + [c_i, c_i] + [c_f] * 4 + [c_int] * 7 + [ctypes.c_void_p, c_int, c_st],
    'dsgcn_head_loss_fwd': [c_f, c_f, c_f, c_i] + [c_int] * 4 + [ctypes.c_float] + [c_f] * 6 + [c_st],
    'dsgcn_head_loss_bwd': [c_f, c_f, c_f, c_i, c_f] + [c_int] * 4 + [ctypes.c_float] + [c_f] * 3 + [c_st],
    'dsgcn_head_test_fwd': [c_f, c_f, c_f] + [c_int] * 6 + [c_f, c_f, c_st],
    'dsgcn_data_bn_fwd': [c_f] * 10 + [c_int] * 7 + [ctypes.c_float, ctypes.c_float, c_st],
    'dsgcn_data_bn_bwd': [c_f] * 6 + [c_int] * 6 + [c_st],
    'dsgcn_sgd_step': [c_f, c_f, c_f, c_f, ctypes.c_float, ctypes.c_float, c_int, ctypes.c_longlong, c_st],
    'dsgcn_grad_norm_rows': [ctypes.c_longlong],
    'dsgcn_grad_norm_partials': [c_f, ctypes.c_longlong, c_int, ctypes.c_void_p, c_st],
    'dsgcn_sgd_step_clip': [c_f, c_f, c_f, c_f, ctypes.c_void_p, c_int, c_int, ctypes.c_float, c_f, ctypes.c_float,
                            ctypes.c_float, c_int, ctypes.c_longlong, c_st],
    'dsgcn_bn_running_multi': [ctypes.c_void_p] * 5 + [ctypes.POINTER(ctypes.c_int), ctypes.POINTER(ctypes.c_float),
                               ctypes.POINTER(ctypes.c_float), c_int, c_st],
}




class BnFinJob(ctypes.Structure):
    _fields_ = [('partial', ctypes.c_void_p), ('gamma', ctypes.c_void_p), ('beta', ctypes.c_void_p),
                ('mean', ctypes.c_void_p), ('var', ctypes.c_void_p), ('scale', ctypes.c_void_p), ('shift', ctypes.c_void_p),
                ('count', ctypes.c_double), ('eps', ctypes.c_float), ('nblk', ctypes.c_int), ('C', ctypes.c_int),
                ('c_affine', ctypes.c_int)]


class BnCoefJob(ctypes.Structure):
    _fields_ = [('part', ctypes.c_void_p), ('mean', ctypes.c_void_p), ('var', ctypes.c_void_p), ('gamma', ctypes.c_void_p),
                ('coef', ctypes.c_void_p), ('count', ctypes.c_double), ('eps', ctypes.c_float), ('R', ctypes.c_int),
                ('C', ctypes.c_int), ('k', ctypes.c_int), ('i_ds', ctypes.c_int), ('i_dh', ctypes.c_int),
                ('c_affine', ctypes.c_int), ('accumulate', ctypes.c_int)]


BN_JOBS_MAX = 4


class Dropout(ctypes.Structure):
    _fields_ = [('step', ctypes.c_void_p), ('seed', ctypes.c_ulonglong), ('call', ctypes.c_uint), ('p', ctypes.c_float)]


class CtrPrepJob(ctypes.Structure):
    _fields_ = [('w', ctypes.c_void_p * 4), ('b', ctypes.c_void_p * 4), ('alpha', ctypes.c_void_p), ('wout', ctypes.c_void_p),
                ('sh', ctypes.c_void_p), ('K', ctypes.c_int), ('Co', ctypes.c_int), ('R', ctypes.c_int),
                ('reserved', ctypes.c_int)]


class CtrFinJob(ctypes.Structure):
    _fields_ = [('dwp', ctypes.c_void_p * 4), ('ds', ctypes.c_void_p * 4), ('out', ctypes.c_void_p * 4),
                ('dalpha', ctypes.c_void_p), ('K', ctypes.c_int), ('Co', ctypes.c_int), ('R', ctypes.c_int),
                ('ds_stride', ctypes.c_int)]


class TsplitJob(ctypes.Structure):
    _fields_ = [('w', ctypes.c_void_p), ('ws', ctypes.c_void_p), ('Ci', ctypes.c_int), ('Co', ctypes.c_int),
                ('KT', ctypes.c_int), ('reserved', ctypes.c_int)]


SIZE_T_RESULTS = {'dsgcn_pwconv_wsplit_bytes', 'dsgcn_tconv_ws_bytes'}

LAB_SIGNATURES = {
    'dsgcn_aggregate_fwd_valu': [c_f, c_f, c_f, c_int, c_f, c_f, c_int, c_int, c_int, c_int, c_st],
    'dsgcn_aggregate_fwd_variant': [c_f, c_f, c_f, c_int, c_f, c_f, c_int, c_int, c_int, c_int, c_int, c_st],
    'dsgcn_set_tuning': [c_int, c_int],
    'dsgcn_pwconv_tuning': [c_int, c_int],
    'dsgcn_diag_mfma_probe': [c_f, c_int, c_int, c_int, c_st],
    'dsgcn_aggsum_tuning': [c_int, c_int],
    'dsgcn_tms_tuning': [c_int, c_int],
    'dsgcn_dynadj_phases': [ctypes.c_void_p],
    'dsgcn_pwg2_phases': [ctypes.c_void_p],
    'dsgcn_pwg2_phases_block': [c_int],
    'dsgcn_bwd64_phases': [ctypes.c_void_p],
    'dsgcn_tcw_phases': [ctypes.c_void_p],
    'dsgcn_tconv_tuning': [c_int, c_int],
    'dsgcn_tms_split_tuning': [c_int, c_int],
    'dsgcn_fuse_out_tuning': [c_int, c_int],
    'dsgcn_tms_split_phases': [c_int, ctypes.c_void_p],
}


def sources(lab=False):
    srcs = sorted(glob.glob(os.path.join(CSRC, '*.hip')))
    if lab:
        srcs += sorted(glob.glob(os.path.join(CSRC, 'lab', '*.hip')))
    return srcs


def _source_hash(lab=False):
    import hashlib
    h = hashlib.sha256()
    extra = sorted(glob.glob(os.path.join(CSRC, 'lab', '*.h'))) if lab else []
    for path in (sources(lab) + sorted(glob.glob(os.path.join(CSRC, '*.h'))) + extra +
                 sorted(glob.glob(os.path.join(INCLUDE, '*.h')))):
        with open(path, 'rb') as f:
            h.update(os.path.basename(path).encode())
            h.update(f.read())
    return h.hexdigest()


def _file_hash(paths):
    import hashlib
    h = hashlib.sha256()
    for path in paths:
        with open(path, 'rb') as f:
            h.update(os.path.basename(path).encode())
            h.update(f.read())
    return h.hexdigest()


def build(force=False, verbose=False, lab=False):
    from concurrent.futures import ThreadPoolExecutor
    srcs = sources(lab)
    lib_path = LAB_LIB_PATH if lab else LIB_PATH
    stamp = lib_path + '.srchash'
    digest = _source_hash(lab)
    if not force and os.path.exists(lib_path) and os.path.exists(stamp):
        with open(stamp) as f:
            if f.read().strip() == digest:
                return lib_path
    obj_dir = os.path.join(LIB_DIR, 'obj_lab' if lab else 'obj')
    os.makedirs(obj_dir, exist_ok=True)
    hipcc = os.environ.get('HIPCC', '/opt/rocm/bin/hipcc')
    headers = sorted(glob.glob(os.path.join(CSRC, '*.h'))) + sorted(glob.glob(os.path.join(INCLUDE, '*.h')))
    if lab:
        headers += sorted(glob.glob(os.path.join(CSRC, 'lab', '*.h')))
    flags = ['--offload-arch=gfx950', '-O3', '-std=c++17', '-fPIC', '-I', INCLUDE, '-I', CSRC]
    if lab:
        flags.append('-DDSGCN_LAB')
        flags += [f for f in os.environ.get('DSGCN_LAB_FLAGS', '').split() if f]
    jobs, objs = [], []
    for src in srcs:
        base = os.path.splitext(os.path.basename(src))[0]
        obj = os.path.join(obj_dir, f'{base}.{_file_hash([src] + headers)[:16]}.o')
        objs.append(obj)
        if force or not os.path.exists(obj):
            for old in glob.glob(os.path.join(obj_dir, base + '.*.o')):
                os.remove(old)
            jobs.append([hipcc] + flags + ['-c', src, '-o', obj])

# ... 53 lines not shown
```

include/dsgcn.h:

```cpp
#ifndef DSGCN_H_
#define DSGCN_H_

#include <stddef.h>
#include "dsgcn_jobs.h"
#ifdef __cplusplus
extern "C" {
#endif

#define DSGCN_EINVAL (-1)
#define DSGCN_EUNSUPPORTED (-2)

int dsgcn_version(void);

int dsgcn_aggregate_fwd(const float* zp, const float* scale, const float* shift, int relu, const float* ahat,
                        float* y, int n, int KC, int T, int V, void* stream);

int dsgcn_aggregate_bwd_partial_rows(int n, int T, int V);
int dsgcn_aggregate_bwd(const float* zp, const float* scale, const float* shift, int relu, const float* ahat,
                        const float* dy, float* dzp, float* dahat, float* partial, int n, int KC, int T, int V,
                        void* stream);

int dsgcn_dynadj_partial_stride(int mid, int V, int E);
int dsgcn_dynadj_fwd(const float* proj, const float* A, const float* alpha, const float* beta, const float* we,
                     const float* be, const int* node_type, const int* edge_type, float* ahat, int n, int mid, int V,
                     int ld, int P, int E, void* stream);
int dsgcn_dynadj_bwd(const float* proj, const float* alpha, const float* beta, const float* we, const float* be,
                     const int* node_type, const int* edge_type, const float* dahat, float* dd_ws, float* dproj,
                     float* ppar, int pstride, int n, int mid, int V, int ld, int P, int E, void* stream);
int dsgcn_dynadj_fwd_jobs(const float* proj, const float* A, const float* alpha, const float* beta, const float* we,
                          const float* be, const int* node_type, const int* edge_type, float* ahat, int n, int mid, int V,
                          int ld, int P, int E, const dsgcn_bn_fin_job* jobs, int njobs, void* stream);
int dsgcn_dynadj_bwd_jobs(const float* proj, const float* alpha, const float* beta, const float* we, const float* be,
                          const int* node_type, const int* edge_type, const float* dahat, float* dd_ws, float* dproj,
                          float* ppar, int pstride, int n, int mid, int V, int ld, int P, int E,
                          const dsgcn_bn_coef_job* jobs, int njobs, void* stream);

int dsgcn_dyntyped_select_fwd(const float* proj, const int* node_type, float* x12, int n, int KM, int P, int V, int ld,
                              void* stream);
int dsgcn_dyntyped_select_bwd(const float* dx12, const int* node_type, float* dproj, int n, int KM, int P, int V, int ld,
                              void* stream);
int dsgcn_dyntyped_partial_stride(int mid, int V, int E, int flags);
int dsgcn_dyntyped_fwd(const float* x12, const float* pq, const float* be, const float* A, const float* alpha,
                       const float* beta, const int* edge_type, float* ahat, int n, int mid, int V, int E, int flags,
                       void* stream);
int dsgcn_dyntyped_bwd(const float* x12, const float* pq, const float* be, const float* alpha, const float* beta,
                       const int* edge_type, const float* dahat, float* dd_ws, float* dx12, float* dpq, float* ppar,
                       int pstride, int n, int mid, int V, int E, int flags, void* stream);

int dsgcn_dynflag_partial_stride(int mid, int V, int E, int flags);
int dsgcn_dynflag_fwd(const float* proj, const float* pq, const float* be, const float* wa, const float* ba,
                      const float* A, const float* alpha, const float* beta, const int* node_type, const int* edge_type,
                      float* ahat, int n, int mid, int V, int ld, int P, int E, int flags, void* stream);
int dsgcn_dynflag_bwd(const float* proj, const float* pq, const float* be, const float* wa, const float* ba,
                      const float* alpha, const float* beta, const int* node_type, const int* edge_type,
                      const float* dahat, float* dd_ws, float* dproj, float* dpq, float* ppar, int pstride, int n,
                      int mid, int V, int ld, int P, int E, int flags, void* stream);

int dsgcn_dynplain_partial_stride(int K, int V);
int dsgcn_dynplain_fwd(const float* proj, const float* A, const float* alpha, const float* beta, float* ahat, int n, int K,
                       int mid, int V, int ld, void* stream);
int dsgcn_dynplain_bwd(const float* proj, const float* alpha, const float* beta, const float* dahat, float* dproj,
                       float* ppar, int pstride, int n, int K, int mid, int V, int ld, void* stream);

int dsgcn_fuse_out_fwd(const float* x1, const float* s1, const float* h1, const float* x2, const float* s2,
                       const float* h2, int relu, float* out, float* xbar, int n, int C, int T, int V, int xbar_ld,
                       void* stream);
int dsgcn_fuse_out_bwd(const float* x1, const float* s1, const float* h1, const float* x2, const float* s2,
                       const float* h2, int relu, const float* dout, const float* dxbar, float* dx1, float* dx2,
                       float* part, int n, int C, int T, int V, int xbar_ld, void* stream);
int dsgcn_fuse_out_bwd3(const float* x1, const float* s1, const float* h1, const float* x2, const float* s2,
                        const float* h2, int relu, const float* dout, const float* dout2, const float* dout3,
                        const float* dxbar, float* dx1, float* dx2, float* part, int n, int C, int T, int V, int xbar_ld,
                        void* stream);
int dsgcn_fuse_out_fwd2(const float* x1, const float* s1, const float* h1, const float* x2, const float* s2,
                        const float* h2, int relu, float* out, float* out_s2, float* xbar, int n, int C, int T, int V,
                        int xbar_ld, void* stream);
int dsgcn_fuse_out_bwd3s(const float* x1, const float* s1, const float* h1, const float* x2, const float* s2,
                         const float* h2, int relu, const float* dout, const float* dout2, const float* dout3, int stride3,
                         const float* dxbar, float* dx1, float* dx2, float* part, int n, int C, int T, int V, int xbar_ld,
                         void* stream);

int dsgcn_fuse_out_pool_fwd(const float* x1, const float* s1, const float* h1, const float* x2, const float* s2,
                            const float* h2, int relu, float* pmean, int n, int C, int T, int V, void* stream);
int dsgcn_fuse_out_pool_bwd(const float* x1, const float* s1, const float* h1, const float* x2, const float* s2,
                            const float* h2, int relu, const float* dpmean, float* dx1, float* dx2, float* part, int n,
                            int C, int T, int V, void* stream);
int dsgcn_fuse_out_fwd_drop(const float* x1, const float* s1, const float* h1, const float* x2, const float* s2,
                            const float* h2, int relu, float* out, float* out_s2, float* xbar, float* pmean, int n, int C,
                            int T, int V, int xbar_ld, const dsgcn_dropout* d, void* stream);
int dsgcn_fuse_out_bwd_drop(const float* x1, const float* s1, const float* h1, const float* x2, const float* s2,
                            const float* h2, int relu, const float* dout, const float* dout2, const float* dout3,
                            int stride3, const float* dxbar, float* dx1, float* dx2, float* part, int n, int C, int T, int V,
                            int xbar_ld, const dsgcn_dropout* d, void* stream);
int dsgcn_dropout_mask(float* mask, long numel, const dsgcn_dropout* d, void* stream);

size_t dsgcn_tconv_ws_bytes(int n, int Ci, int Co, int T, int V, int KT, int stride);
int dsgcn_tconv_wsplit(const float* w, int Ci, int Co, int KT, void* ws, void* stream);
int dsgcn_tconv_wsplit_multi(const dsgcn_tsplit_job* jobs, int njobs, void* stream);
int dsgcn_tconv_rows(int which, int n, int Ci, int Co, int T, int V, int KT, int stride);
int dsgcn_tconv_fwd(const float* x1, const float* s1, const float* h1, const float* x2, const float* s2, const float* h2,
                    int relu, const void* ws, const float* bias, float* z, float* partial, int n, int Ci, int Co, int T,
                    int V, int KT, int stride, void* stream);
int dsgcn_tconv_dgrad(const float* x1, const float* s1, const float* h1, const float* x2, const float* s2,
                      const float* h2, int relu, const void* ws, const float* z, const float* gz, const float* A0,
                      const float* B0, float* dx1, float* dx2, float* ipart, int n, int Ci, int Co, int T, int V, int KT,
                      int stride, void* stream);

int dsgcn_tconv_wgrad_splits(int n, int Ci, int Co, int T, int V, int KT, int stride);
int dsgcn_tconv_wgrad(const float* x1, const float* s1, const float* h1, const float* x2, const float* s2,
                      const float* h2, int relu, const float* z, const float* gz, const float* A0, const float* B0,
                      float* dwp, float* dbp, int pstride, int n, int Ci, int Co, int T, int V, int KT, int stride,
                      void* stream);

int dsgcn_branch_act_fwd(const float* z, const float* zaug, const float* scale, const float* shift, int n_act,
                         float* h, int n, int C, int T, int V, void* stream);
int dsgcn_branch_act_bwd(const float* z, const float* zaug, const float* scale, const float* shift, int n_act,
                         const float* dh, float* dz, float* dzaug, float* part, int n, int C, int T, int V,
                         void* stream);
int dsgcn_tapconv_fwd(const float* h, float* o, int n, int Cin, int Cout, int T, int V1, int stride, int KT, int nbr,
                      const int* type, const int* ci0, const int* co0, const int* cin, const int* cout, const int* dil,
                      const float* const* w, const float* const* b, void* stream);
int dsgcn_tapconv_dgrad(const float* h, const float* go, float* dh, int n, int Cin, int Cout, int T, int V1, int stride,
                        int KT, int nbr, const int* type, const int* ci0, const int* co0, const int* cin,
                        const int* cout, const int* dil, const float* const* w, void* stream);
int dsgcn_tapconv_wgrad_splits(int n, int Cin, int Cout, int T, int V1, int stride, int KT, int nbr, const int* type,
                               const int* cin, const int* cout, const int* dil);
int dsgcn_tapconv_wgrad(const float* h, const float* go, int n, int Cin, int Cout, int T, int V1, int stride, int KT,
                        int nbr, const int* type, const int* ci0, const int* co0, const int* cin, const int* cout,
                        const int* dil, float* const* dwp, float* const* dbp, int splits, int pstride, void* stream);
int dsgcn_tms_combine_fwd(const float* o, const float* coeff, float* f, float* partial, int n, int C, int T, int V,
                          void* stream);
int dsgcn_tms_combine_bwd(const float* o, const float* coeff, const float* gf, const float* A0, const float* B0,
                          float* dout, float* pcoef, int n, int C, int T, int V, void* stream);
int dsgcn_pwconv_ipart_rows(int n, int Ci, int Co, int T, int V, int stride);

int dsgcn_pwconv_plan(int Tout, int V, int aug, int* TR, int* NPpad, int* nblk_per_sample);
int dsgcn_pwconv_partial_rows(int n, int Ci, int Co, int T, int V, int stride, int aug);
int dsgcn_pwconv_fwd(const float* x1, const float* s1, const float* h1, const float* x2, const float* s2,
                     const float* h2, int relu, const float* w, const float* bias, float* z, float* zaug,
                     float* partial, int n, int Ci, int Co, int T, int V, int stride, int aug, int stats,
                     void* stream);
int dsgcn_bn_finalize(const float* partial, int nblk, int C, double count, const float* gamma, const float* beta,
                      float eps, float* mean_out, float* var_out, float* scale_out, float* shift_out, int c_affine,
                      void* stream);
int dsgcn_colsum(const float* src, int R, int C, float* out, void* stream);
int dsgcn_colsum_t(const float* src, int R, int C, int inner, float* out, void* stream);
int dsgcn_colsum2(const float* src_a, int Ra, int Ca, int inner_a, float* out_a, const float* src_b, int Rb, int Cb,
                  int inner_b, float* out_b, void* stream);
int dsgcn_colsum_blocks(const float* src, int C);
int dsgcn_colsum_multi(const long* table, int njobs, int nblocks, void* stream);
int dsgcn_colsum_multi_host(const long* table, int njobs, void* stream);
int dsgcn_bn_bwd_coef(const float* g_scale, const float* g_shift, const float* mean, const float* var,
                      const float* gamma, float eps, double count, int C, int c_affine, float* dgamma, float* dbeta,
                      float* A0, float* B0, void* stream);
int dsgcn_bn_coef_rows(const float* part, int R, int C, int k, int i_ds, int i_dh, const float* mean, const float* var,
                       const float* gamma, float eps, double count, int c_affine, float* coef, int accumulate,
                       void* stream);
int dsgcn_bn_finalize_multi(const dsgcn_bn_fin_job* jobs, int njobs, void* stream);
int dsgcn_bn_coef_rows_multi(const dsgcn_bn_coef_job* jobs, int njobs, void* stream);
int dsgcn_dz_eff_aug(const float* gz, const float* z, const float* gzaug, const float* zaug, const float* A0,
                     const float* B0, float* out, int n, int C, int T, int V, void* stream);
int dsgcn_pwconv_dgrad(const float* x1, const float* s1, const float* h1, const float* x2, const float* s2,
                       const float* h2, int relu, const float* w, const float* z, const float* zaug,
                       const float* gz, const float* gzaug, const float* A0, const float* B0, float* dx1, float* dx2,
                       float* ipart, int n, int Ci, int Co, int T, int V, int stride, int aug, void* stream);
size_t dsgcn_pwconv_wsplit_bytes(int n, int Ci, int Co, int T, int V, int stride);
int dsgcn_pwconv_wsplit(const float* w, int Ci, int Co, void* ws, void* stream);
int dsgcn_pwconv_wsplit_multi(const float* const* w, void* const* ws, const int* Ci, const int* Co, int njobs,
                              void* stream);
int dsgcn_pwconv_fwd_ws(const float* x1, const float* s1, const float* h1, const float* x2, const float* s2,
                        const float* h2, int relu, const float* w, const float* bias, float* z, float* zaug,
                        float* partial, int n, int Ci, int Co, int T, int V, int stride, int aug, int stats,
                        const void* ws, void* stream);
int dsgcn_pwconv_dgrad_ws(const float* x1, const float* s1, const float* h1, const float* x2, const float* s2,
                          const float* h2, int relu, const float* w, const float* z, const float* zaug,
                          const float* gz, const float* gzaug, const float* A0, const float* B0, float* dx1, float* dx2,
                          float* ipart, int n, int Ci, int Co, int T, int V, int stride, int aug, const void* ws,
                          void* stream);
int dsgcn_pwconv_wgrad_splits(int n, int Ci, int Co, int T, int V, int stride);
int dsgcn_pwconv_bwd_rows(int n, int Ci, int Co, int T, int V, int stride);
int dsgcn_pwconv_bwd(const float* x1, const float* s1, const float* h1, const float* x2, const float* s2, const float* h2,
                     int relu, const float* w, const float* z, const float* gz, const float* A0, const float* B0,
                     float* dx1, float* dx2, float* ipart, float* dwp, float* dbp, int pstride, int n, int Ci, int Co,
                     int T, int V, void* stream);
int dsgcn_pwconv_wgrad(const float* x1, const float* s1, const float* h1, const float* x2, const float* s2,
                       const float* h2, int relu, const float* z, const float* zaug, const float* gz,
                       const float* gzaug, const float* A0, const float* B0, float* dwp, float* dbp, int pstride, int n,
                       int Ci, int Co, int T, int V, int stride, int aug, void* stream);
int dsgcn_pwconv_wgrad_jobs(const float* x1, const float* s1, const float* h1, const float* x2, const float* s2,
                            const float* h2, int relu, const float* z, const float* zaug, const float* gz,
                            const float* gzaug, const float* A0, const float* B0, float* dwp, float* dbp, int pstride, int n,
                            int Ci, int Co, int T, int V, int stride, int aug, const dsgcn_bn_coef_job* jobs, int njobs,
                            void* stream);
int dsgcn_pwconv_group_ok(int n, int Ci, int Co, int T, int V);
int dsgcn_pwconv_fwd_group(const float* const* x1, const float* const* s1, const float* const* h1, int relu,
                           const float* const* w, float* const* z, int ngroup, int n, int Ci, int Co, int T, int V,
                           void* stream);
int dsgcn_pwconv_dgrad_group(const float* const* x1, const float* const* s1, const float* const* h1, int relu,
                             const float* const* w, const float* const* gz, float* const* dx1, float* const* ipart,
                             int ngroup, int n, int Ci, int Co, int T, int V, void* stream);
int dsgcn_pwconv_wgrad_group(const float* const* x1, const float* const* s1, const float* const* h1, int relu,
                             const float* const* gz, float* const* dwp, float* const* dbp, int pstride, int ngroup, int n,
                             int Ci, int Co, int T, int V, void* stream);

int dsgcn_aggsum_partial_rows(int n, int T, int V);
int dsgcn_aggsum_bwd_piece_rows(int n, int K, int Co, int T, int V);
int dsgcn_aggsum_fwd(const float* p, const float* ahat, long a_ns, long a_ks, long a_cs, float* y, float* partial,
                     int n, int K, int Co, int T, int V, void* stream);
int dsgcn_aggsum_bwd(const float* p, const float* ahat, long a_ns, long a_ks, long a_cs, const float* gy,
                     const float* y, const float* A0, const float* B0, float* dp, float* dahat, long d_ns, long d_ks,
                     long d_cs, int n, int K, int Co, int T, int V, void* stream);

int dsgcn_tanhdiff_fwd(const float* proj, float* d, int n, int K, int R, int V, void* stream);
int dsgcn_tanhdiff_bwd(const float* d, const float* dd, float* dproj, int n, int K, int R, int V, void* stream);
int dsgcn_tanhdiff_bwd_k(const float* d, const float* const* dd, float* dproj, int n, int K, int R, int V, void* stream);
int dsgcn_tanhdiff_aug_fwd(const float* proj, const float* A, float* d, int n, int K, int R, int V, void* stream);
int dsgcn_tanhdiff_aug_bwd(const float* d, const float* const* dd, float* dproj, float* dAp, int n, int K, int R, int V,
                           void* stream);
int dsgcn_ctr_wprep(const float* const* w, const float* const* b, const float* alpha, float* wout, float* sh, int K,
                    int Co, int R, void* stream);
int dsgcn_ctr_wfin(const float* const* dwp, const float* const* ds, int ds_stride, float* const* out, float* dalpha, int K,
                   int Co, int R, void* stream);
int dsgcn_ctr_wprep_multi(const dsgcn_ctr_prep_job* jobs, int njobs, void* stream);
int dsgcn_ctr_wfin_multi(const dsgcn_ctr_fin_job* jobs, int njobs, void* stream);
int dsgcn_ctr_affine_fwd(const float* const* s, const float* alpha, int alpha_stride, const float* A, const float* beta,
                         const float* G, float* ahat, int n, int K, int Co, int V, void* stream);
int dsgcn_ctr_affine_bwd(const float* const* s, const float* alpha, int alpha_stride, const float* dahat,
                         float* const* ds, float* prow, int n, int K, int Co, int V, void* stream);
int dsgcn_edge_select_fwd(const float* in, const int* edge_type, float* out, int n, int R, int E, int V, void* stream);
int dsgcn_edge_select_bwd(const float* dout, const int* edge_type, float* din, int n, int R, int E, int V, void* stream);
int dsgcn_plane_stats(const float* x, float* partial, long planes, int L, void* stream);

int dsgcn_add3(const float* a, const float* b, const float* c, float* out, long n, void* stream);

int dsgcn_pack(const float* const* src_table, const long* dst_offsets, const int* numels, int count, float* dst,
               void* stream);
int dsgcn_pack_fill(const float* const* src_table, const long* dst_offsets, const long* numels, int count, float* dst,
                    void* stream);

int dsgcn_dwcausal_fwd(const float* h, const float* w, const float* b, const int* dil, float* y, int n, int C, int T,
                       int V, int stride, int KM, void* stream);
int dsgcn_dwcausal_bwd(const float* h, const float* w, const int* dil, const float* dy, float* dh, float* part, int n,
                       int C, int T, int V, int stride, int KM, void* stream);

int dsgcn_tms_rows(int which, int n, int C, int T, int V, int stride, int KT, int nbr, const int* type, const int* bc,
                   const int* dil, int aug);
int dsgcn_tms_fwd(const float* z, const float* zaug, const float* scale, const float* shift, int n_act,
                  const float* coeff, float* f, float* oaug, float* stats, int n, int C, int T, int V, int stride, int KT,
                  int nbr, const int* type, const int* c0, const int* bc, const int* dil, const float* const* w,
                  const float* const* b, void* stream);
int dsgcn_tms_dgrad(const float* z, const float* zaug, const float* scale, const float* shift, int n_act,
                    const float* coeff, const float* gf, const float* f, const float* A0, const float* B0,
                    const float* oaug, float* dz, float* dzaug, float* paff, float* pcoeff, int n, int C, int T, int V,
                    int stride, int KT, int nbr, const int* type, const int* c0, const int* bc, const int* dil,
                    const float* const* w, void* stream);
int dsgcn_tms_wgrad(const float* z, const float* zaug, const float* scale, const float* shift, int n_act,
                    const float* coeff, const float* gf, const float* f, const float* A0, const float* B0, int n, int C,
                    int T, int V, int stride, int KT, int nbr, const int* type, const int* c0, const int* bc,
                    const int* dil, float* const* dwp, float* const* dbp, int pstride, void* stream);

int dsgcn_tms_split_rows(int which, int n, int C, int T, int V, int stride, int KT, int nbr, const int* type,
                         const int* c0, const int* bc, const int* dil);
int dsgcn_tms_split_fwd(const float* z, const float* zaug, const float* scale, const float* shift, int n_act,
                        const float* coeff, float* f, float* oaug, float* stats, int n, int C, int T, int V, int stride,
                        int nbr, const int* type, const int* c0, const int* bc, const int* dil, const float* const* w,
                        const float* const* b, void* stream);
int dsgcn_tms_split_prep(const float* gf, const float* f, const float* oaug, const float* coeff, const float* A0,
                         const float* B0, float* ge, float* doaug, float* pcoef, int n, int C, int T, int V,
                         void* stream);
int dsgcn_tms_split_dgrad(const float* z, const float* zaug, const float* scale, const float* shift, int n_act,
                          const float* ge, const float* doaug, float* dz, float* dzaug, float* part, int n, int C, int T,
                          int V, int stride, int nbr, const int* type, const int* c0, const int* bc, const int* dil,
                          const float* const* w, void* stream);
int dsgcn_tms_split_wgrad(const float* z, const float* zaug, const float* scale, const float* shift, int n_act,
                          const float* ge, const float* doaug, int n, int C, int T, int V, int stride, int nbr,
                          const int* type, const int* c0, const int* bc, const int* dil, float* const* dwp, float* const* dbp,
                          int splits, int pstride, void* stream);
int dsgcn_tms_split_wgrad_jobs(const float* z, const float* zaug, const float* scale, const float* shift, int n_act,
                               const float* ge, const float* doaug, int n, int C, int T, int V, int stride, int nbr,
                               const int* type, const int* c0, const int* bc, const int* dil, float* const* dwp,
                               float* const* dbp, int splits, int pstride, const dsgcn_bn_coef_job* jobs, int njobs,
                               void* stream);

int dsgcn_gate_fwd(const float* y, const float* g, int mode, float* out, float* rout, int rmode, int n, int C, int T,
                   int V, void* stream);
int dsgcn_gate_bwd(const float* y, const float* g, int mode, const float* gout, const float* drout, int rmode, float* dy,
                   float* dgp, int n, int C, int T, int V, void* stream);

int dsgcn_skeleton_prep(const float* raw, const long* offset, const int* M, const int* T, const int* flags,
                        const int* f0, const int* f1, const float* center, const float* matrix, const int* parent,
                        float* out, int N, int clips, int Mout, int clip_len, int V, int C, int nfeat, int fmask,
                        int scored, int loop, void* stream);

int dsgcn_head_loss_fwd(const float* feat, const float* w, const float* b, const long long* label, int N, int M, int C,
                        int K, float loss_weight, float* pooled, float* score, float* prob, float* clip, float* loss,
                        double* acc, void* stream);
int dsgcn_head_loss_bwd(const float* prob, const float* pooled, const float* w, const long long* label, const float* gloss,
                        int N, int M, int C, int K, float loss_weight, float* dfeat, float* dw, float* db, void* stream);

int dsgcn_head_test_fwd(const float* feat, const float* w, const float* b, int N, int clips, int M, int C, int K, int mode,
                        float* clip_score, float* out, void* stream);

int dsgcn_bn_running_multi(float* const* running_mean, float* const* running_var, const float* const* mean,
                           const float* const* var, long long* const* num_batches_tracked, const int* C,
                           const float* unbias, const float* momentum, int njobs, void* stream);

int dsgcn_data_bn_fwd(const float* x, const float* gamma, const float* beta, float* running_mean, float* running_var,
                      long long* num_batches_tracked, float* y, float* save_mean, float* save_invstd, float* scratch,
                      int N, int M, int T, int V, int C, int mvc, int training, float eps, float momentum,
                      void* stream);
int dsgcn_data_bn_bwd(const float* x, const float* dy, const float* save_mean, const float* save_invstd, float* pg,
                      float* pb, int N, int M, int T, int V, int C, int mvc, void* stream);

int dsgcn_sgd_step(float* p, const float* g, float* buf, const float* lr, float momentum, float weight_decay,
                   int nesterov, long long n, void* stream);

int dsgcn_grad_norm_rows(long long n);
int dsgcn_grad_norm_partials(const float* g, long long n, int norm_type, double* partial, void* stream);
int dsgcn_sgd_step_clip(float* p, float* g, float* buf, const float* lr, const double* partial, int rows, int norm_type,
                        float max_norm, float* grad_norm_out, float momentum, float weight_decay, int nesterov,
                        long long n, void* stream);

#ifdef __cplusplus
}
#endif
#endif
```

Before: 5924 clips/s.

## Share one unscaled gradient buffer across residual inputs, folding BN scale into consumer

```diff
diff --git a/ds-gcn_amd/csrc/bwd64.hip b/ds-gcn_amd/csrc/bwd64.hip
--- a/ds-gcn_amd/csrc/bwd64.hip
+++ b/ds-gcn_amd/csrc/bwd64.hip
@@ -10,6 +10,7 @@
   const float* x2; const float* s2; const float* h2; int relu;
   const float* w;
   const float* z; const float* gz; const float* A0; const float* B0;
+  const float* gscale; int one;
   float* dx; float* dx2; float* dwp; float* dbp; float* ipart;
   int pstride, n, Ci, Co, L, cpn, total_chunks, cps;
 };
@@ -44,6 +45,7 @@
   float* Ws = lds + 192 * BF_LS;
   bf_f2* Cs = reinterpret_cast<bf_f2*>(Ws + 64 * 65);
   f32x4* Ps = reinterpret_cast<f32x4*>(Cs + 64);
+  float* Gs = reinterpret_cast<float*>(Ps + 64);
   const int tid = threadIdx.x, lane = tid & 63;
   const int wave = __builtin_amdgcn_readfirstlane(tid >> 6);
   const int half = lane >> 5, l31 = lane & 31;
@@ -57,6 +59,7 @@
   }
   if (tid < 64) {
     Cs[tid] = (HASC && tid < Co) ? bf_f2{a.A0[tid], a.B0[tid]} : bf_f2{0.f, 0.f};
+    Gs[tid] = (a.gscale && tid < Co) ? a.gscale[tid] : 1.f;
     f32x4 p = {1.f, 0.f, 1.f, 0.f};
     if (AFF && tid < Ci) {
       if (a.s1) { p.x = a.s1[tid]; p.y = a.h1[tid]; }
@@ -97,6 +100,11 @@
     for (int j = 0; j < BF_J; ++j) {
       const int row = row0 + 16 * j;
       f32x4 d = gr[j];
+      {
+        const float gs = Gs[row];
+#pragma unroll
+        for (int e = 0; e < 4; ++e) d[e] = __fmul_rn(d[e], gs);
+      }
       if constexpr (HASC) {
         const bf_f2 c = Cs[row];
 #pragma unroll
@@ -220,8 +228,11 @@
               }
             }
             const size_t go = ((size_t)n * Ci + row) * L + c0 + col;
-            __builtin_nontemporal_store(f32x4{dv.x * p.x, dv.y * p.x, dv.z * p.x, dv.w * p.x}, reinterpret_cast<f32x4*>(a.dx + go));
-            if constexpr (HAS2) __builtin_nontemporal_store(f32x4{dv.x * p.z, dv.y * p.z, dv.z * p.z, dv.w * p.z}, reinterpret_cast<f32x4*>(a.dx2 + go));
+            const float sx = (HAS2 && a.one) ? 1.f : p.x;
+            __builtin_nontemporal_store(f32x4{dv.x * sx, dv.y * sx, dv.z * sx, dv.w * sx}, reinterpret_cast<f32x4*>(a.dx + go));
+            if constexpr (HAS2) {
+              if (!a.one) __builtin_nontemporal_store(f32x4{dv.x * p.z, dv.y * p.z, dv.z * p.z, dv.w * p.z}, reinterpret_cast<f32x4*>(a.dx2 + go));
+            }
           }
         }
       }
@@ -287,6 +298,7 @@
   const int row = tid >> 2, q = tid & 3;
   const bool rd = row < Co, rx = row < Ci;
   const float A0v = (HASC && rd) ? a.A0[row] : 0.f, B0v = (HASC && rd) ? a.B0[row] : 0.f;
+  const float gsv = (a.gscale && rd) ? a.gscale[row] : 1.f;
   float s1v = 1.f, h1v = 0.f;
   if (AFF && rx && a.s1) { s1v = a.s1[row]; h1v = a.h1[row]; }
   const float lo = a.relu ? 0.f : -__builtin_inff();
@@ -329,7 +341,7 @@
       const bool in = c0 + 8 * q + 4 * h < L;
 #pragma unroll
       for (int e = 0; e < 4; ++e) {
-        float x = R.g[h][e];
+        float x = __fmul_rn(R.g[h][e], gsv);
         if constexpr (HASC) x += fmaf(B0v, R.z[h][e], A0v);
         d[4 * h + e] = (rd && in) ? x : 0.f;
         float t = R.x[h][e];
@@ -526,12 +538,13 @@
                                                        const float* s2, const float* h2, int relu, const float* w,
                                                        const float* z, const float* gz, const float* A0, const float* B0,
                                                        float* dx, float* dx2, float* dwp, float* dbp, int pstride,
-                                                       float* ipart, int n, int Ci, int Co, int L, hipStream_t st) {
+                                                       float* ipart, int n, int Ci, int Co, int L, hipStream_t st,
+                                                       const float* gscale) {
   BfPlan p;
   if (!bf_plan(n, Ci, Co, L, &p)) return 0;
   BfArgs a = {};
   a.x1 = x1; a.s1 = s1; a.h1 = h1; a.x2 = x2; a.s2 = s2; a.h2 = h2; a.relu = relu; a.w = w; a.z = z; a.gz = gz;
-  a.A0 = A0; a.B0 = B0; a.dx = dx; a.dx2 = dx2; a.dwp = dwp; a.dbp = dbp; a.ipart = ipart; a.pstride = pstride;
+  a.A0 = A0; a.B0 = B0; a.gscale = gscale; a.one = (x2 != nullptr && dx2 == nullptr) ? 1 : 0; a.dx = dx; a.dx2 = dx2; a.dwp = dwp; a.dbp = dbp; a.ipart = ipart; a.pstride = pstride;
   a.n = n; a.Ci = Ci; a.Co = Co; a.L = L; a.cpn = p.cpn; a.total_chunks = p.chunks; a.cps = p.cps;
   const bool b3 = g_bf_b3 && x2 == nullptr && Ci >= 16;
   if (b3) {
@@ -539,7 +552,7 @@
     a.total_chunks = n * a.cpn;
     a.cps = (a.total_chunks + p.splits - 1) / p.splits;
   }
-  const size_t lds = b3 ? (size_t)BB_LDS : (size_t)(192 * BF_LS + 64 * 65 + 2 * 64 + 4 * 64) * sizeof(float);
+  const size_t lds = b3 ? (size_t)BB_LDS : (size_t)(192 * BF_LS + 64 * 65 + 2 * 64 + 4 * 64 + 64) * sizeof(float);
   const dim3 grid((unsigned)p.splits), blk(BF_NT);
   const bool hasc = A0 != nullptr, has2 = x2 != nullptr, aff = s1 != nullptr || s2 != nullptr || relu != 0 || has2;
   if (b3) {
diff --git a/ds-gcn_amd/csrc/fuseout.hip b/ds-gcn_amd/csrc/fuseout.hip
--- a/ds-gcn_amd/csrc/fuseout.hip
+++ b/ds-gcn_amd/csrc/fuseout.hip
@@ -108,7 +108,7 @@
                                                      const float* __restrict__ dout2, const float* __restrict__ dout3,
                                                      const float* __restrict__ dxbar, float* __restrict__ dx1,
                                                      float* __restrict__ dx2, float* __restrict__ part, int C, int T,
-                                                     int V, int ld, int s3, DropArgs dr) {
+                                                     int V, int ld, int s3, DropArgs dr, int one) {
   __shared__ float dxb[32];
   const int lane = threadIdx.x;
   const long plane = blockIdx.x;
@@ -149,7 +149,7 @@
     g += dxb[v];
     if ((relu & 1) && !(pre > 0.f)) g = 0.f;
     const float g1 = (((relu & 2) && !(pre1 > 0.f)) ? 0.f : g) * dm;
-    o1[i] = g1 * a1;
+    o1[i] = one ? g : g1 * a1;
     if (o2) o2[i] = g * a2;
     u0 = fmaf(g1, xa, u0);
     u1 += g;
@@ -181,7 +181,7 @@
                                                       const float* __restrict__ dout2, const float* __restrict__ dout3,
                                                       const float* __restrict__ dxbar, float* __restrict__ dx1,
                                                       float* __restrict__ dx2, float* __restrict__ part, int C, int T,
-                                                      int V, int ld, DropArgs dr) {
+                                                      int V, int ld, DropArgs dr, int one) {
   __shared__ float dxb[32];
   const int lane = threadIdx.x;
   const long plane = blockIdx.x;
@@ -201,7 +201,7 @@
   const f32x4* __restrict__ pg3 = (NG >= 3 && !S3) ? reinterpret_cast<const f32x4*>(dout3 + (size_t)plane * L) : nullptr;
   const float* __restrict__ ps3 = S3 ? dout3 + (size_t)plane * (((T + 1) >> 1) * V) : nullptr;
   f32x4* __restrict__ o1 = reinterpret_cast<f32x4*>(dx1 + (size_t)plane * L);
-  f32x4* __restrict__ o2 = X2 ? reinterpret_cast<f32x4*>(dx2 + (size_t)plane * L) : nullptr;
+  f32x4* __restrict__ o2 = (X2 && !one) ? reinterpret_cast<f32x4*>(dx2 + (size_t)plane * L) : nullptr;
   const float invV = 1.f / (float)V;
   float u0 = 0.f, u1 = 0.f, u2 = 0.f, u3 = 0.f;
   for (int i = lane; i < L4; i += 64) {
@@ -231,7 +231,7 @@
       if constexpr (X2) pre += fmaf(xb[k], a2, b2);
       if ((relu & 1) && !(pre > 0.f)) gg = 0.f;
       const float g1 = (((relu & 2) && !(pre1 > 0.f)) ? 0.f : gg) * dm[k];
-      r1[k] = g1 * a1;
+      r1[k] = one ? gg : g1 * a1;
       r2[k] = gg * a2;
       u0 = fmaf(g1, xa[k], u0);
       u1 += gg;
@@ -240,7 +240,7 @@
       if (++v == V) { v = 0; ++t; }
     }
     o1[i] = r1;
-    if constexpr (X2) o2[i] = r2;
+    if constexpr (X2) { if (!one) o2[i] = r2; }
   }
   if (part) {
     u0 = wave_sum(u0);
@@ -319,11 +319,11 @@
   return dsgcn_fuse_out_fwd_drop(x1, s1, h1, x2, s2, h2, relu, nullptr, nullptr, nullptr, pmean, n, C, T, V, V, nullptr, stream);
 }
 
-int dsgcn_fuse_out_bwd_drop(const float* x1, const float* s1, const float* h1, const float* x2, const float* s2,
+static int fuse_out_bwd_any(const float* x1, const float* s1, const float* h1, const float* x2, const float* s2,
                             const float* h2, int relu, const float* dout, const float* dout2, const float* dout3,
                             int stride3, const float* dxbar, float* dx1, float* dx2, float* part, int n, int C, int T, int V,
-                            int xbar_ld, const dsgcn_dropout* d, void* stream) {
-  if (!x1 || !dx1 || n <= 0 || C <= 0 || T <= 0 || V <= 0 || V > 32 || (x2 && !dx2)) return DSGCN_EINVAL;
+                            int xbar_ld, const dsgcn_dropout* d, void* stream, int one) {
+  if (!x1 || !dx1 || n <= 0 || C <= 0 || T <= 0 || V <= 0 || V > 32 || (x2 && !dx2 && !one)) return DSGCN_EINVAL;
   if (dxbar && xbar_ld < V) return DSGCN_EINVAL;
   if ((dout2 || dout3) && !dout) return DSGCN_EINVAL;
   if (stride3 < 1 || stride3 > 3 || (stride3 == 3 && (!dout || dout2 || dout3 || dxbar))) return DSGCN_EINVAL;
@@ -335,13 +335,13 @@
     if ((T * V) % 4 == 0) {
       if (x2)
         hipLaunchKernelGGL((k_fuse_out_bwd4<0, false, true>), grid, blk, 0, st, x1, s1, h1, x2, s2, h2, relu, dout,
-                           (const float*)nullptr, (const float*)nullptr, (const float*)nullptr, dx1, dx2, part, C, T, V, V, dr);
+                           (const float*)nullptr, (const float*)nullptr, (const float*)nullptr, dx1, dx2, part, C, T, V, V, dr, one);
       else
         hipLaunchKernelGGL((k_fuse_out_bwd4<0, false, false>), grid, blk, 0, st, x1, s1, h1, x2, s2, h2, relu, dout,
-                           (const float*)nullptr, (const float*)nullptr, (const float*)nullptr, dx1, dx2, part, C, T, V, V, dr);
+                           (const float*)nullptr, (const float*)nullptr, (const float*)nullptr, dx1, dx2, part, C, T, V, V, dr, one);
     } else {
       hipLaunchKernelGGL(k_fuse_out_bwd, grid, blk, 0, st, x1, s1, h1, x2, s2, h2, relu, dout, (const float*)nullptr,
-                         (const float*)nullptr, (const float*)nullptr, dx1, dx2, part, C, T, V, V, 3, dr);
+                         (const float*)nullptr, (const float*)nullptr, dx1, dx2, part, C, T, V, V, 3, dr, one);
     }
     DSGCN_LAUNCH_CHECK();
     return 0;
@@ -350,7 +350,7 @@
     const int ng = dout3 && stride3 == 1 ? 3 : (dout2 ? 2 : 1);
     const bool s3 = dout3 && stride3 == 2;
 #define FO4(NGV, S3V, X2V) hipLaunchKernelGGL((k_fuse_out_bwd4<NGV, S3V, X2V>), grid, blk, 0, st, x1, s1, h1, x2, s2, h2, relu, \
-                                              dout, dout2, dout3, dxbar, dx1, dx2, part, C, T, V, xbar_ld, dr)
+                                              dout, dout2, dout3, dxbar, dx1, dx2, part, C, T, V, xbar_ld, dr, one)
     if (x2) {
       if (s3) { if (ng == 2) FO4(2, true, true); else FO4(1, true, true); }
       else if (ng == 3) FO4(3, false, true);
@@ -367,9 +367,26 @@
     return 0;
   }
   hipLaunchKernelGGL(k_fuse_out_bwd, grid, blk, 0, st, x1, s1, h1, x2, s2, h2, relu, dout, dout2, dout3, dxbar, dx1, dx2,
-                     part, C, T, V, xbar_ld, stride3, dr);
+                     part, C, T, V, xbar_ld, stride3, dr, one);
   DSGCN_LAUNCH_CHECK();
   return 0;
+}
+
+int dsgcn_fuse_out_bwd_drop(const float* x1, const float* s1, const float* h1, const float* x2, const float* s2,
+                            const float* h2, int relu, const float* dout, const float* dout2, const float* dout3,
+                            int stride3, const float* dxbar, float* dx1, float* dx2, float* part, int n, int C, int T, int V,
+                            int xbar_ld, const dsgcn_dropout* d, void* stream) {
+  return fuse_out_bwd_any(x1, s1, h1, x2, s2, h2, relu, dout, dout2, dout3, stride3, dxbar, dx1, dx2, part, n, C, T, V,
+                          xbar_ld, d, stream, 0);
+}
+
+int dsgcn_fuse_out_bwd_one(const float* x1, const float* s1, const float* h1, const float* x2, const float* s2,
+                           const float* h2, int relu, const float* dout, const float* dout2, const float* dout3,
+                           int stride3, const float* dxbar, float* dx, float* part, int n, int C, int T, int V, int xbar_ld,
+                           void* stream) {
+  if (!x2 || (relu & 2)) return DSGCN_EINVAL;
+  return fuse_out_bwd_any(x1, s1, h1, x2, s2, h2, relu, dout, dout2, dout3, stride3, dxbar, dx, nullptr, part, n, C, T, V,
+                          xbar_ld, nullptr, stream, 1);
 }
 
 int dsgcn_fuse_out_pool_bwd(const float* x1, const float* s1, const float* h1, const float* x2, const float* s2,
diff --git a/ds-gcn_amd/csrc/pwconv.hip b/ds-gcn_amd/csrc/pwconv.hip
--- a/ds-gcn_amd/csrc/pwconv.hip
+++ b/ds-gcn_amd/csrc/pwconv.hip
@@ -1096,7 +1096,8 @@
                                                        const float* s2, const float* h2, int relu, const float* w,
                                                        const float* z, const float* gz, const float* A0, const float* B0,
                                                        float* dx, float* dx2, float* dwp, float* dbp, int pstride,
-                                                       float* ipart, int n, int Ci, int Co, int L, hipStream_t st);
+                                                       float* ipart, int n, int Ci, int Co, int L, hipStream_t st,
+                                                       const float* gscale = nullptr);
 
 __attribute__((visibility("hidden"))) int dsgcn_wg2_splits(int n, int Ci, int Co, int L);
 __attribute__((visibility("hidden"))) int dsgcn_wg2(const float* x1, const float* s1, const float* h1, const float* x2,
@@ -1597,4 +1598,16 @@
   return rc == 0 ? DSGCN_EUNSUPPORTED : rc;
 }
 
-}
+int dsgcn_pwconv_bwd_gs(const float* x1, const float* s1, const float* h1, const float* x2, const float* s2,
+                        const float* h2, int relu, const float* w, const float* z, const float* gz, const float* gscale,
+                        const float* A0, const float* B0, float* dx1, float* dx2, float* ipart, float* dwp, float* dbp,
+                        int pstride, int n, int Ci, int Co, int T, int V, void* stream) {
+  if (!x1 || !w || !gz || !dx1 || !dwp || !dbp || n <= 0 || Ci <= 0 || Co <= 0 || T <= 0 || V <= 0) return DSGCN_EINVAL;
+  if ((A0 && (!B0 || !z)) || (s1 && !h1) || (s2 && !h2) || (dx2 && !x2) || pstride < Co * Ci) return DSGCN_EINVAL;
+  const int rc = dsgcn_bwd64(x1, s1, h1, x2, s2, h2, relu, w, z, gz, A0, B0, dx1, dx2, dwp, dbp, pstride, ipart, n, Ci, Co,
+                             T * V, (hipStream_t)stream, gscale);
+  if (rc == 1) return 0;
+  return rc == 0 ? DSGCN_EUNSUPPORTED : rc;
+}
+
+}
diff --git a/ds-gcn_amd/kernels.py b/ds-gcn_amd/kernels.py
--- a/ds-gcn_amd/kernels.py
+++ b/ds-gcn_amd/kernels.py
@@ -430,12 +430,17 @@
 
 
 class BNCtx:
-    __slots__ = ('mean', 'var', 'gamma', 'eps', 'count', 'C', 'n_affine', 'coef', 'host', 'queued')
+    __slots__ = ('mean', 'var', 'gamma', 'eps', 'count', 'C', 'n_affine', 'coef', 'host', 'queued', 'gs_ok', 'z_ptr', 'uses',
+                 'shared')
 
     def __init__(self):
         self.coef = None
         self.host = False
         self.queued = None
+        self.gs_ok = False
+        self.z_ptr = 0
+        self.uses = 0
+        self.shared = None
 
 
 def _bn_attach(scale, bn, mean, var, gamma, eps, count, n_affine):
@@ -447,7 +452,23 @@
 
 
 def _bn_of(scale):
-    return getattr(scale, '_dsgcn_bn', None) if (scale is not None and BN_FEED) else None
+    bn = getattr(scale, '_dsgcn_bn', None) if (scale is not None and BN_FEED) else None
+    if bn is not None:
+        bn.uses += 1
+    return bn
+
+
+SHARED_GRAD = _os.environ.get('DSGCN_SHARED_GRAD', '1') == '1'
+shared_grad_taken = {'fuse_out': 0, 'pwconv': 0}
+
+
+def _takes_unscaled(bn, x):
+    return bn is not None and bn.gs_ok and bn.uses == 1 and bn.z_ptr == x.data_ptr()
+
+
+def _share_ok(x1, s1, bn1, x2, s2, bn2):
+    return (SHARED_GRAD and x2 is not None and s1 is not None and _takes_unscaled(bn1, x1) and
+            (s2 is None or _takes_unscaled(bn2, x2)))
 
 
 BN_BATCH = _os.environ.get('DSGCN_BN_BATCH', '1') == '1'
@@ -851,6 +872,9 @@
             mean, var, scale, shift = stats[0], stats[1], stats[2], stats[3]
             bn_finalize(partial, partial.shape[0], Co, count, gamma, beta, eps, mean, var, scale, shift, n_affine)
             ctx.mark_non_differentiable(mean, var)
+            if bn is not None and bn.gs_ok:
+                bn.z_ptr = z.data_ptr()
+                ctx.stats = stats
         ctx.set_materialize_grads(False)
         ctx.save_for_backward(x1, s1, h1, x2, s2, h2, w2, z, zaug, gamma, mean, var, ws)
         ctx.cfg = (int(relu), stride, int(aug), float(eps), int(n_affine), bool(want_bn), count, tuple(weight.shape),
@@ -876,6 +900,13 @@
         if want_bn:
             dgamma, dbeta, A0, B0 = _bn_coef(ctx.bn, gscale, gshift, mean, var, gamma, eps, count, Co, n_affine)
         Tout = z.shape[2]
+        gsc = None
+        if ctx.bn is not None and ctx.bn.shared is not None:
+            sh, ctx.bn.shared = ctx.bn.shared, None
+            if gz is None or gz.data_ptr() != sh.data_ptr() or gz.shape != sh.shape or aug:
+                raise RuntimeError('dsgcn: a shared (unscaled) gradient did not reach its conv as handed on — '
+                                   'z has another consumer; run with DSGCN_SHARED_GRAD=0')
+            gsc = ctx.stats[2]
         if gz is None:
             gz = torch.zeros_like(z)
         if aug:
@@ -884,20 +915,36 @@
                                       Co, Tout, V, st)
             native.check(rc, 'dsgcn_dz_eff_aug')
             gz, gzaug, A0, B0, aug = dzeff, None, None, None, 0
-        dx1 = torch.empty_like(x1)
-        dx2 = torch.empty_like(x2) if x2 is not None else None
         pstride = Co * Ci + Co
         rows = lib.dsgcn_pwconv_bwd_rows(n, Ci, Co, T, V, stride) if (not aug and gz is not None) else 0
+        one = rows > 0 and _share_ok(x1, s1, ctx.bn1, x2, s2, ctx.bn2)
+        dx1 = torch.empty_like(x1)
+        dx2 = torch.empty_like(x2) if (x2 is not None and not one) else None
         if rows > 0:
             wpart = torch.empty((rows, pstride), device=dev, dtype=torch.float32)
             ipart = (torch.empty((rows, Ci, 3), device=dev, dtype=torch.float32)
                      if (s1 is not None or s2 is not None) else None)
-            rc = lib.dsgcn_pwconv_bwd(_ptr(x1), _ptr(s1), _ptr(h1), _ptr(x2), _ptr(s2), _ptr(h2), relu, _ptr(w2), _ptr(z),
-                                      _ptr(gz), _ptr(A0), _ptr(B0), _ptr(dx1), _ptr(dx2), _ptr(ipart), wpart.data_ptr(),
-                                      wpart.data_ptr() + 4 * Co * Ci, pstride, n, Ci, Co, T, V, st)
-            native.check(rc, 'dsgcn_pwconv_bwd')
+            if one or gsc is not None:
+                rc = lib.dsgcn_pwconv_bwd_gs(_ptr(x1), _ptr(s1), _ptr(h1), _ptr(x2), _ptr(s2), _ptr(h2), relu, _ptr(w2),
+                                             _ptr(z), _ptr(gz), _ptr(gsc), _ptr(A0), _ptr(B0), _ptr(dx1),
+                                             _ptr(dx2), _ptr(ipart), wpart.data_ptr(),
+                                             wpart.data_ptr() + 4 * Co * Ci, pstride, n, Ci, Co, T, V, st)
+                native.check(rc, 'dsgcn_pwconv_bwd_gs')
+                if one:
+                    dx2 = dx1
+                    ctx.bn1.shared = dx1
+                    if s2 is not None:
+                        ctx.bn2.shared = dx1
+                    shared_grad_taken['pwconv'] += 1
+            else:
+                rc = lib.dsgcn_pwconv_bwd(_ptr(x1), _ptr(s1), _ptr(h1), _ptr(x2), _ptr(s2), _ptr(h2), relu, _ptr(w2),
+                                          _ptr(z), _ptr(gz), _ptr(A0), _ptr(B0), _ptr(dx1), _ptr(dx2), _ptr(ipart),
+                                          wpart.data_ptr(), wpart.data_ptr() + 4 * Co * Ci, pstride, n, Ci, Co, T, V, st)
+                native.check(rc, 'dsgcn_pwconv_bwd')
             return _PwConv._finish(wpart, ipart, dx1, dx2, s1, s2, Co, Ci, wshape, has_bias, dgamma, dbeta, gamma,
                                    has_beta, n_affine, ctx.defer_ok, ctx.bn1, ctx.bn2, ctx.sink is not None and bool(ctx.sink))
+        if gsc is not None:
+            raise RuntimeError('dsgcn: a shared (unscaled) gradient reached a conv off the one-pass backward')
         ipart = None
         if s1 is not None or s2 is not None:
             rows = lib.dsgcn_pwconv_ipart_rows(n, Ci, Co, T, V, stride)
@@ -1071,6 +1118,9 @@
     if n_affine is None:
         n_affine = weight.shape[0] if gamma is not None else 0
     bn = BNCtx() if want_bn else None
+    if (bn is not None and SHARED_GRAD and BN_FEED and not aug and int(stride) == 1 and x1.is_cuda and
+            native.lib().dsgcn_pwconv_bwd_rows(x1.shape[0], x1.shape[1], weight.shape[0], x1.shape[2], x1.shape[3], 1) > 0):
+        bn.gs_ok = True
     out = _PwConv.apply(x1, s1, h1, x2, s2, h2, bool(relu), weight, bias, int(stride), bool(aug), gamma, beta,
                         float(eps), int(n_affine), bool(want_bn), bn, out)
     if want_bn:
@@ -2385,14 +2435,25 @@
             douts += [None] * (3 - len(douts))
         dxbar = _f32c(dxbar)
         dx1 = torch.empty_like(x1)
-        dx2 = torch.empty_like(x2) if x2 is not None else None
         need_part = s1 is not None or s2 is not None
         part = torch.empty((n, C, 4), device=x1.device, dtype=torch.float32) if need_part else None
-        rc = native.lib().dsgcn_fuse_out_bwd_drop(_ptr(x1), _ptr(s1), _ptr(h1), _ptr(x2), _ptr(s2), _ptr(h2), ctx.relu,
-                                                  _ptr(douts[0]), _ptr(douts[1]), _ptr(douts[2]), stride3, _ptr(dxbar),
-                                                  _ptr(dx1), _ptr(dx2), _ptr(part), n, C, T, V, ctx.xbar_ld or V,
-                                                  _ct.byref(ctx.drop[0]) if ctx.drop else None, _stream())
-        native.check(rc, 'dsgcn_fuse_out_bwd_drop')
+        if not (ctx.relu & 2) and not ctx.drop and _share_ok(x1, s1, ctx.bn1, x2, s2, ctx.bn2):
+            rc = native.lib().dsgcn_fuse_out_bwd_one(_ptr(x1), _ptr(s1), _ptr(h1), _ptr(x2), _ptr(s2), _ptr(h2), ctx.relu,
+                                                     _ptr(douts[0]), _ptr(douts[1]), _ptr(douts[2]), stride3, _ptr(dxbar),
+                                                     _ptr(dx1), _ptr(part), n, C, T, V, ctx.xbar_ld or V, _stream())
+            native.check(rc, 'dsgcn_fuse_out_bwd_one')
+            dx2 = dx1
+            ctx.bn1.shared = dx1
+            if s2 is not None:
+                ctx.bn2.shared = dx1
+            shared_grad_taken['fuse_out'] += 1
+        else:
+            dx2 = torch.empty_like(x2) if x2 is not None else None
+            rc = native.lib().dsgcn_fuse_out_bwd_drop(_ptr(x1), _ptr(s1), _ptr(h1), _ptr(x2), _ptr(s2), _ptr(h2), ctx.relu,
+                                                      _ptr(douts[0]), _ptr(douts[1]), _ptr(douts[2]), stride3, _ptr(dxbar),
+                                                      _ptr(dx1), _ptr(dx2), _ptr(part), n, C, T, V, ctx.xbar_ld or V,
+                                                      _ct.byref(ctx.drop[0]) if ctx.drop else None, _stream())
+            native.check(rc, 'dsgcn_fuse_out_bwd_drop')
         ds1 = dh1 = ds2 = dh2 = None
         if need_part and (s1 is None or ctx.bn1 is not None) and (s2 is None or ctx.bn2 is not None):
             _bn_feed_multi(([(ctx.bn1, part, 4, 0, 3)] if s1 is not None else []) +
diff --git a/ds-gcn_amd/native.py b/ds-gcn_amd/native.py
--- a/ds-gcn_amd/native.py
+++ b/ds-gcn_amd/native.py
@@ -55,6 +55,7 @@
     'dsgcn_pwconv_wgrad_splits': [c_int] * 6,
     'dsgcn_pwconv_bwd_rows': [c_int] * 6,
     'dsgcn_pwconv_bwd': [c_f] * 6 + [c_int] + [c_f] * 10 + [c_int] * 6 + [c_st],
+    'dsgcn_pwconv_bwd_gs': [c_f] * 6 + [c_int] + [c_f] * 11 + [c_int] * 6 + [c_st],
     'dsgcn_pwconv_wgrad': [c_f] * 6 + [c_int] + [c_f] * 8 + [c_int] * 8 + [c_st],
     'dsgcn_bn_bwd_coef': [c_f] * 5 + [ctypes.c_float, ctypes.c_double, c_int, c_int] + [c_f] * 4 + [c_st],
     'dsgcn_branch_act_fwd': [c_f] * 4 + [c_int] + [c_f] + [c_int] * 4 + [c_st],
@@ -118,6 +119,7 @@
     'dsgcn_pwconv_wgrad_jobs': [c_f] * 6 + [c_int] + [c_f] * 8 + [c_int] * 8 + [ctypes.c_void_p, c_int, c_st],
     'dsgcn_tms_split_wgrad_jobs': [c_f] * 4 + [c_int] + [c_f] * 2 + [c_int] * 6 + [c_i] * 4 + [ctypes.c_void_p, ctypes.c_void_p, c_int, c_int, ctypes.c_void_p, c_int, c_st],
     'dsgcn_fuse_out_fwd_drop': [c_f] * 6 + [c_int] + [c_f] * 4 + [c_int] * 5 + [ctypes.c_void_p, c_st],
+    'dsgcn_fuse_out_bwd_one': [c_f] * 6 + [c_int] + [c_f] * 3 + [c_int] + [c_f] * 3 + [c_int] * 5 + [c_st],
     'dsgcn_fuse_out_bwd_drop': [c_f] * 6 + [c_int] + [c_f] * 3 + [c_int] + [c_f] * 4 + [c_int] * 5 + [ctypes.c_void_p, c_st],
     'dsgcn_dropout_mask': [c_f, ctypes.c_long, ctypes.c_void_p, c_st],
     'dsgcn_bn_finalize_multi': [ctypes.c_void_p, c_int, c_st],
diff --git a/include/dsgcn.h b/include/dsgcn.h
--- a/include/dsgcn.h
+++ b/include/dsgcn.h
@@ -93,6 +93,10 @@
                             int stride3, const float* dxbar, float* dx1, float* dx2, float* part, int n, int C, int T, int V,
                             int xbar_ld, const dsgcn_dropout* d, void* stream);
 int dsgcn_dropout_mask(float* mask, long numel, const dsgcn_dropout* d, void* stream);
+int dsgcn_fuse_out_bwd_one(const float* x1, const float* s1, const float* h1, const float* x2, const float* s2,
+                           const float* h2, int relu, const float* dout, const float* dout2, const float* dout3,
+                           int stride3, const float* dxbar, float* dx, float* part, int n, int C, int T, int V, int xbar_ld,
+                           void* stream);
 
 size_t dsgcn_tconv_ws_bytes(int n, int Ci, int Co, int T, int V, int KT, int stride);
 int dsgcn_tconv_wsplit(const float* w, int Ci, int Co, int KT, void* ws, void* stream);
@@ -183,6 +187,10 @@
                      int relu, const float* w, const float* z, const float* gz, const float* A0, const float* B0,
                      float* dx1, float* dx2, float* ipart, float* dwp, float* dbp, int pstride, int n, int Ci, int Co,
                      int T, int V, void* stream);
+int dsgcn_pwconv_bwd_gs(const float* x1, const float* s1, const float* h1, const float* x2, const float* s2,
+                        const float* h2, int relu, const float* w, const float* z, const float* gz, const float* gscale,
+                        const float* A0, const float* B0, float* dx1, float* dx2, float* ipart, float* dwp, float* dbp,
+                        int pstride, int n, int Ci, int Co, int T, int V, void* stream);
 int dsgcn_pwconv_wgrad(const float* x1, const float* s1, const float* h1, const float* x2, const float* s2,
                        const float* h2, int relu, const float* z, const float* zaug, const float* gz,
                        const float* gzaug, const float* A0, const float* B0, float* dwp, float* dbp, int pstride, int n,
```

After: 5936 clips/s, median of 5. About the same (+0.2%).
